# Neos-codes/microbeast

Hardware: AMD Instinct MI355X
Metric: env frames/sec (whole node) on 16x16 microRTS (higher is better)
Workload: dtype bf16

## Files before the change

### microbeast_amd/_native.py

```python
from __future__ import annotations

import ctypes
import importlib.util
import os
import sys
import threading
from pathlib import Path

import torch

_LIB = Path(__file__).resolve().parent / "_lib"
_lock = threading.Lock()
_kern = None
_rt = None

c_void_p, c_int, c_int64, c_float = ctypes.c_void_p, ctypes.c_int, ctypes.c_int64, ctypes.c_float

_SIGS = {
    "mbk_multi_copy": [c_void_p, c_int, c_void_p],
    "mbk_comm_standin": [c_void_p, c_void_p, c_int64, c_int, c_int, c_void_p],
    "mbk_row_gather": [c_void_p, c_void_p, c_void_p, c_int, c_int64, c_void_p],
    "mbk_memset": [c_void_p, c_int, c_int64, c_void_p],
    "mbk_masked_cell_fwd": [c_void_p, c_int, c_void_p, c_void_p, c_void_p, c_int, c_int64,
                            c_void_p, c_void_p, c_void_p],
# ... 10 lines not shown
    "mbk_imgwgrad_parts": [],
    "mbk_cells_nchunk": [c_int],
    "mbk_cells_compact": [c_void_p, c_int, c_int, c_int, c_void_p, c_void_p, c_void_p, c_void_p,
                          c_void_p, c_void_p, c_void_p, c_void_p, c_void_p, c_void_p],
    "mbk_rows_colsum": [c_void_p, c_int, c_int, c_void_p, c_int, c_void_p, c_void_p],
    "mbk_masked_cell_rows_fwd": [c_void_p, c_int, c_void_p, c_void_p, c_int, c_void_p, c_void_p,
                                 c_void_p, c_int, c_void_p, c_void_p, c_void_p],
    "mbk_masked_cell_rows_bwd": [c_void_p, c_int, c_void_p, c_void_p, c_int, c_int, c_void_p,
                                 c_void_p, c_void_p, c_void_p, c_void_p, c_void_p],
    "mbk_pwgrad": [c_void_p, c_void_p],
    "mbk_pwgrad_all": [c_void_p, c_void_p],
    "mbk_pwgrad_all_parts": [c_int, c_int, c_int],
    "mbk_pwgrad_parts": [c_int, c_int, c_int, c_int],
    "mbk_reduce_map": [c_void_p, c_int, c_int64, c_void_p, c_int64, c_void_p, c_void_p],
    "mbk_reduce_inv": [c_void_p, c_int, c_int64, c_void_p, c_int64, c_void_p, c_void_p, c_int64,
                       c_void_p],
    "mbk_ppool_fwd": [c_void_p, c_int, c_int, c_int, c_int, c_void_p, c_void_p, c_void_p],
    "mbk_ppool_bwd": [c_void_p, c_int64, c_int, c_void_p, c_int64, c_int, c_void_p, c_void_p,
                      c_int, c_int, c_int, c_int, c_void_p, c_void_p],
    "mbk_rng_advance": [c_void_p, c_void_p],
    "mbk_vtrace": [c_void_p, c_void_p, c_void_p, c_void_p, c_void_p, c_void_p, c_int, c_int,
                   c_float, c_float, c_float, c_float, c_float, c_float, c_float, c_void_p,
                   c_void_p, c_void_p, c_void_p, c_void_p, c_void_p, c_void_p],
    "mbk_vtrace_upgo": [c_void_p, c_void_p, c_void_p, c_void_p, c_void_p, c_void_p, c_int, c_int,
                        c_float, c_float, c_float, c_float, c_float, c_float, c_float, c_float,
                        c_float, c_float, c_void_p, c_void_p, c_void_p, c_void_p, c_void_p,
                        c_void_p, c_void_p, c_void_p],
    "mbk_gae": [c_void_p, c_void_p, c_void_p, c_int, c_int, c_float, c_float, c_float, c_int,
                c_void_p, c_void_p, c_void_p, c_void_p, c_void_p],
    "mbk_vtrace_adv": [c_void_p, c_void_p, c_void_p, c_void_p, c_void_p, c_int, c_int, c_float,
                       c_float, c_float, c_float, c_float, c_int, c_void_p, c_void_p, c_void_p,
                       c_void_p, c_void_p, c_void_p],
    "mbk_ppo_loss": [c_void_p, c_void_p, c_void_p, c_void_p, c_void_p, c_void_p, c_void_p,
                     c_void_p, c_int, c_int, c_float, c_float, c_float, c_float, c_float, c_float,
                     c_void_p, c_void_p, c_void_p, c_void_p, c_void_p],
    "mbk_adv_stats_rows": [c_void_p, c_int, c_int, c_int, c_int, c_void_p, c_void_p, c_void_p],
    "mbk_ppo_loss_rows": [c_void_p, c_void_p, c_void_p, c_void_p, c_void_p, c_void_p, c_void_p,
                          c_void_p, c_int, c_int, c_int, c_float, c_float, c_float, c_float,
                          c_float, c_float, c_int, c_void_p, c_void_p, c_void_p, c_void_p,
                          c_void_p, c_void_p],
    "mbk_grad_clip_scale": [c_void_p, c_int64, c_float, c_float, c_void_p, c_void_p, c_void_p],
    "mbk_adam": [c_void_p, c_void_p, c_void_p, c_void_p, c_void_p, c_int64, c_float, c_float,
                 c_float, c_float, c_float, c_int64, c_void_p, c_float, c_void_p],
    "mbk_to_bf16": [c_void_p, c_int64, c_void_p, c_void_p],
    "mbk_from_bf16": [c_void_p, c_int64, c_void_p, c_void_p],
    "mbk_conv_fwd": [c_void_p, c_int, c_int, c_int, c_void_p, c_void_p, c_void_p, c_void_p,
                     c_void_p, c_void_p, c_void_p, c_int, c_int, c_int, c_int, c_int, c_void_p],
    "mbk_conv_fwd_fp8": [c_void_p, c_int, c_int, c_int, c_void_p, c_void_p, c_void_p, c_void_p,
                         c_void_p, c_int, c_int, c_int, c_int, c_int, c_void_p],
    "mbk_conv_fwd_imgs": [c_int, c_int, c_int, c_int, c_int, c_int, c_int],
    "mbk_conv_wgrad_imgs": [c_int, c_int, c_int, c_int, c_int, c_int],
    "mbk_res_bwd16_imgs": [c_int, c_int],
    "mbk_res_blk32_fwd_imgs": [c_int, c_int],
    "mbk_res_bwd32_imgs": [c_int, c_int],
    "mbk_res_fwd16_stage_ok": [c_int, c_int],
    "mbk_conv_pack_fp8": [c_void_p, c_int, c_void_p],
    "mbk_pool_bwd_idx": [c_void_p, c_void_p, c_int, c_int, c_int, c_int, c_void_p, c_void_p],
    "mbk_conv_wgrad": [c_void_p, c_int, c_int, c_int, c_void_p, c_void_p, c_void_p, c_void_p,
                       c_int, c_int, c_int, c_int, c_int, c_int, c_void_p],
    "mbk_conv_wgrad_parts": [c_int, c_int, c_int, c_int, c_int, c_int, c_int],
    "mbk_conv_wgrad0_sparse_parts": [c_int],
    "mbk_conv_wgrad0_sparse": [c_void_p, c_void_p, c_void_p, ctypes.c_uint, c_void_p, c_int, c_int,
                               c_void_p],
    "mbk_pool_conv_bwd_parts": [c_int, c_int, c_int, c_int, c_int],
    "mbk_pool_conv_bwd": [c_void_p, c_void_p, c_void_p, c_void_p, c_void_p, c_void_p, c_int,
                          c_int, c_int, c_int, c_int, c_int, c_void_p],
    "mbk_conv_set_grid_cap": [c_int],
    "mbk_set_learner_occupancy": [c_int, c_int],
    "mbk_set_work_queues": [c_int],
    "mbk_set_work_queue_site": [c_int, c_int],
    "mbk_conv0_row_set": [c_int],
    "mbk_fc_wgrad_parts": [c_int, c_int, c_int],
    "mbk_fc_wgrad": [c_void_p, c_void_p, c_int, c_int, c_int, c_void_p, c_int, c_void_p, c_int,
                     c_void_p],
    "mbk_fc_fwd": [c_void_p, c_int, c_void_p, c_void_p, c_void_p, c_void_p, c_int, c_int, c_int,
                   c_void_p, c_void_p, c_void_p],
    "mbk_gemm_nt": [c_void_p, c_void_p, c_void_p, c_void_p, c_int, c_int, c_int, c_int, c_int,
                    c_int, c_int, c_int, c_int, c_void_p],
    "mbk_wgrad_partial_floats": [c_int, c_int, c_int],
    "mbk_wgrad_reduce_batch": [c_void_p, c_int, c_void_p],
    "mbk_pool_bwd": [c_void_p, c_void_p, c_int, c_int, c_int, c_int, c_void_p, c_void_p],
    "mbk_conv_pack": [c_void_p, c_int, c_void_p],
    "mbk_head_compact": [c_void_p, c_int, c_int, c_void_p, c_void_p, c_void_p, c_void_p,
                         c_void_p, c_void_p, c_void_p, c_void_p, c_void_p, c_void_p, c_void_p,
                         c_void_p, c_void_p, c_int, c_void_p, c_void_p, c_void_p, c_void_p],
    "mbk_head_fwd": [c_void_p, c_void_p, c_void_p, c_void_p, c_void_p, c_void_p, c_int,
                     c_void_p, c_void_p, c_void_p, c_void_p, c_void_p, c_void_p, c_int, c_int,
                     c_void_p, c_void_p, c_int, c_void_p],
    "mbk_fc_wgrad_wide_parts": [c_int, c_int, c_int],
    "mbk_fc_wgrad_wide": [c_void_p, c_void_p, c_int, c_int, c_int, c_int, c_void_p, c_int,
                          c_void_p, c_void_p, c_void_p],
    "mbk_head_score": [c_void_p, c_void_p, c_void_p, c_void_p, c_void_p, c_void_p, c_void_p,
                       c_void_p, c_void_p, c_void_p, c_void_p, c_int, c_void_p, c_void_p,
                       c_void_p, c_void_p],
    "mbk_head_pair_rowsum": [c_void_p, c_void_p, c_int, c_int, c_void_p, c_void_p, c_void_p,
                             c_void_p, c_void_p],
    "mbk_head_bwd": [c_void_p, c_void_p, c_void_p, c_void_p, c_void_p, c_void_p, c_void_p,
                     c_void_p, c_void_p, c_void_p, c_void_p, c_void_p, c_void_p, c_void_p,
                     c_void_p, c_int, c_int, c_void_p, c_void_p, c_void_p, c_void_p,
                     c_void_p, c_void_p, c_void_p],
    "mbk_head_dx_gather": [c_void_p, c_void_p, c_void_p, c_int, c_int, c_void_p, c_void_p],
    "mbk_head_dx_value_parts": [c_int],
    "mbk_head_dx_value": [c_void_p, c_void_p, c_void_p, c_int, c_int, c_void_p, c_void_p,
                          c_void_p, c_int, c_void_p, c_void_p, c_int, c_void_p],
    "mbk_head_pack": [c_void_p, c_void_p, c_int, c_void_p, c_void_p, c_void_p, c_void_p],
    "mbk_decode_obs_mask": [c_void_p, c_void_p, c_int, c_int, c_int, c_void_p, c_void_p, c_void_p],
    "mbk_decode_obs_mask_bucket": [c_void_p, c_void_p, c_int, c_int, c_int, c_void_p, c_void_p,
                                   c_void_p, c_void_p, c_void_p, c_void_p, c_void_p],
    "mbk_head_units": [c_void_p, c_int, c_int, c_void_p, c_void_p, c_void_p, c_void_p, c_void_p,
                       c_void_p],
    "mbk_row_sum_rng": [c_void_p, c_int64, c_int, c_void_p, c_void_p, c_void_p],
    "mbk_row_sum_pack": [c_void_p, c_int64, c_int, c_void_p, c_void_p, c_void_p, c_void_p,
                         c_void_p, c_int, c_void_p],
    "mbk_head_fwd_counts": [c_void_p, c_void_p, c_void_p, c_void_p, c_void_p, c_void_p,
                            c_void_p, c_void_p, c_int, c_int, c_int, c_void_p, c_int, c_void_p],
    "mbk_trunk_tail": [c_void_p, c_void_p, c_void_p, c_int, c_int, c_int, c_void_p, c_void_p],
    "mbk_trunk_tail_fp8": [c_void_p, c_void_p, c_void_p, c_void_p, c_int, c_int, c_int, c_void_p,
                           c_void_p],
    "mbk_trunk_tail_fc": [c_void_p, c_void_p, c_void_p, c_int, c_int, c_int, c_void_p, c_void_p,
                          c_void_p, c_void_p, c_void_p, c_int, c_void_p, c_void_p, c_void_p],
    "mbk_pack_env_actions": [c_void_p, c_int64, c_void_p, c_void_p],
    "mbk_res_bwd16_parts": [c_int, c_int, c_int],
    "mbk_res_bwd32_parts": [c_int, c_int, c_int],
    "mbk_res_bwd32": [c_void_p, c_void_p, c_void_p, c_void_p, c_void_p, c_void_p, c_void_p, c_int,
                      c_int, c_int, c_int, c_void_p],
    "mbk_res_fwd16": [c_void_p, c_void_p, c_void_p, c_void_p, c_void_p, c_void_p, c_void_p, c_int,
                      c_int, c_int, c_void_p],
    "mbk_res_fwd16_stage": [c_void_p, c_void_p, c_void_p, c_void_p, c_void_p, c_void_p, c_void_p,
                            c_void_p, c_void_p, c_void_p, c_void_p, c_int, c_int, c_int, c_void_p],
    "mbk_res_blk32_fwd": [c_void_p, c_void_p, c_void_p, c_void_p, c_void_p, c_int, c_int, c_int,
                          c_void_p],
    "mbk_pool_conv_fwd4": [c_void_p, c_void_p, c_void_p, c_void_p, c_void_p, c_int, c_void_p],
    "mbk_res_blk32_fwd_wave": [c_void_p, c_void_p, c_void_p, c_void_p, c_void_p, c_int, c_int,
                               c_int, c_void_p],
    "mbk_res_bwd32_team_parts": [c_int, c_int, c_int],
    "mbk_res_bwd32_team": [c_void_p, c_void_p, c_void_p, c_void_p, c_void_p, c_void_p, c_void_p,
                           c_int, c_int, c_int, c_int, c_void_p],
    "mbk_res_bwd16": [c_void_p, c_void_p, c_void_p, c_void_p, c_void_p, c_void_p, c_void_p, c_int,
                      c_int, c_int, c_int, c_void_p],
    "mbk_bits_pad": [c_void_p, c_int, c_int, c_int, c_int, c_int, c_void_p, c_void_p],
    "mbk_colsum_parts": [c_int64],
    "mbk_colsum": [c_void_p, c_int, c_int, c_int, c_int, c_void_p, c_void_p, c_int, c_void_p,
                   c_void_p],
    "mbk_map_gather": [c_int, c_void_p, c_void_p, c_void_p, c_void_p, c_void_p, c_void_p],
    "mbk_value_bwd_parts": [c_int],
    "mbk_value_bwd": [c_void_p, c_void_p, c_void_p, c_int, c_int, c_void_p, c_void_p, c_void_p,
                      c_int, c_int, c_void_p],
    "mbk_fc_wgrad_ex": [c_void_p, c_void_p, c_int, c_int, c_int, c_void_p, c_int, c_void_p, c_int,
                        c_int, c_void_p],
    "mbk_act_step": [c_void_p, c_void_p, c_void_p],
    "mbk_act_trunk": [c_void_p, c_void_p, c_void_p],
    "mbk_act_head": [c_void_p, c_void_p, c_void_p],
    "mbk_act_set_stamps": [c_void_p],
    "mbk_rows_to_codes": [c_void_p, c_int, c_int, c_int, c_void_p, c_void_p, c_void_p],
    "mbk_codes_to_rows": [c_void_p, c_int, c_int, c_void_p, c_int, c_void_p],
    "mbk_gemm_nt_mask": [c_void_p, c_void_p, c_void_p, c_void_p, c_int, c_int, c_int, c_int, c_int,
                         c_int, c_int, c_int, c_void_p, c_void_p],
}
_RESTYPE = {"mbk_wgrad_partial_floats": c_int64}


def _ensure_built() -> None:
    kl = _LIB / "libmbk_kernels.so"
    rts = list(_LIB.glob("_mbrt*.so"))
    if kl.exists() and rts and os.environ.get("MBK_REBUILD", "0") != "1":
        return
    from .csrc import build as _b

    _b.build()


def kernels():
    global _kern
    if _kern is not None:
        return _kern
    with _lock:
        if _kern is None:
            _ensure_built()
            lib = ctypes.CDLL(str(_LIB / "libmbk_kernels.so"), mode=ctypes.RTLD_GLOBAL)
            for name, args in _SIGS.items():
                fn = getattr(lib, name)
                fn.argtypes = args
                fn.restype = _RESTYPE.get(name, c_int)
            _kern = _Checked(lib)
    return _kern


class _Checked:

    def __init__(self, lib):
        self._lib = lib

    def __getattr__(self, name):
        if name not in _SIGS:
            raise AttributeError(f"{name}: no ctypes signature declared in _native._SIGS")
        return getattr(self._lib, name)


def runtime():
    global _rt
    if _rt is not None:
        return _rt
    with _lock:
        if _rt is None:
            _ensure_built()
            kernels_path = _LIB / "libmbk_kernels.so"
            ctypes.CDLL(str(kernels_path), mode=ctypes.RTLD_GLOBAL)
            cands = sorted(_LIB.glob("_mbrt*.so"))
            if not cands:
                raise ImportError("microbeast_amd native runtime (_mbrt) not built")
            spec = importlib.util.spec_from_file_location("microbeast_amd._lib._mbrt", cands[0])
            mod = importlib.util.module_from_spec(spec)
            spec.loader.exec_module(mod)
            sys.modules["microbeast_amd._lib._mbrt"] = mod
            _rt = mod
    return _rt


def check(rc: int, what: str) -> None:
    if rc != 0:
        raise RuntimeError(f"{what} failed with hipError {rc}")


def stream_ptr(stream: torch.cuda.Stream | None = None) -> int:
    s = stream if stream is not None else torch.cuda.current_stream()
    return int(s.cuda_stream)


def ptr(t: torch.Tensor | None) -> int | None:
    return None if t is None else t.data_ptr()


def loaded_libraries() -> list[str]:
    out = []
    try:
        with open("/proc/self/maps") as f:
            for line in f:
                if str(_LIB) in line:
                    p = line.split()[-1]
                    if p not in out:
                        out.append(p)
    except OSError:
        pass
    return out
```

### microbeast_amd/csrc/include/mbk_api.h

```cpp
#pragma once
#include <hip/hip_runtime_api.h>
#include <stdint.h>

#ifdef __cplusplus
extern "C" {
#endif

#define MBK_MAX_COPY_SEGS 16
typedef struct {
  const void* src;
  void* dst;
  uint64_t bytes;
} MbkCopySeg;

int mbk_multi_copy(const MbkCopySeg* segs, int n, hipStream_t stream);

typedef struct {
  const float* w;
  void* fwd;
  void* bwd;
  int cin, cin_real, cout;
} MbkPackJob;

int mbk_conv_pack(const MbkPackJob* jobs, int n, hipStream_t stream);

typedef struct {
  const float* w;
  void* q;
  float* scale;
  int cin, cin_real, cout;
} MbkPackJob8;

int mbk_conv_pack_fp8(const MbkPackJob8* jobs, int n, hipStream_t stream);

typedef struct {
  const void* w0;
  const float* b0;
  const void* w[14];
  const float* b[14];
  const void* w5;
  const float* b5;
  const float* wc;
  const float* bc;
  const void* Wp;
  const float* bp;
  uint64_t* rng;
  void* feat;
  int* bucket_cnt;
  int* bucket;
  uint64_t* cellx;
  int* pending;
  int E, H, W;
} MbkActModel;

typedef struct {
  const uint16_t* codes;
  const int32_t* res;
  const uint32_t* code_list;
  uint32_t* obs;
  uint32_t* mask;
  uint32_t* obs2;
  uint32_t* mask2;
  uint8_t* action;
  float* logp;
  float* value;
  uint16_t* act16;
  uint32_t* act_list;
  int list_stride;
  const float* reward_src;
  const uint8_t* done_src;
  float* reward_dst;
  uint8_t* done_dst;
  uint64_t step;
  uint32_t* abits;
  uint32_t* abits2;
  int32_t greedy;
} MbkActStep;

int mbk_act_step(const MbkActModel* m, const MbkActStep* s, hipStream_t stream);
int mbk_rows_to_codes(const uint32_t* rows, int stride, int E, int S, void* codes, int32_t* res,
                      hipStream_t stream);
int mbk_codes_to_rows(const void* act16, int E, int S, uint32_t* rows, int stride,
                      hipStream_t stream);
int mbk_act_trunk(const MbkActModel* m, const MbkActStep* s, hipStream_t stream);
int mbk_act_head(const MbkActModel* m, const MbkActStep* s, hipStream_t stream);

int mbk_gae(const float* v_old, const float* reward, const uint8_t* done, int T, int B,
            float gamma, float lambda, float reward_clip, int norm_adv, float* adv, float* ret,
            float* partials, float* stats, hipStream_t stream);
int mbk_vtrace_adv(const float* logp_pi, const float* logp_mu, const float* v,
                   const float* reward, const uint8_t* done, int T, int B, float gamma,
                   float lambda, float rho_bar, float c_bar, float reward_clip, int norm_adv,
                   float* adv, float* ret, float* partials, float* stats, float* is_stats,
                   hipStream_t stream);
int mbk_ppo_loss(const float* logp_new, const float* logp_old, const float* values,
                 const float* v_old, const float* adv, const float* ret, const float* entropy,
                 const float* stats, int T, int B, float clip_lo, float clip_hi, float clip,
                 float value_clip, float baseline_cost, float entropy_cost, float* g_logp,
                 float* g_value, float* partials, float* losses, hipStream_t stream);
int mbk_adv_stats_rows(const float* adv, int T, int B, int K, int norm_adv, float* partials,
                       float* stats, hipStream_t stream);
int mbk_ppo_loss_rows(const float* logp_new, const float* logp_old, const float* values,
                      const float* v_old, const float* adv, const float* ret,
                      const float* entropy, const float* stats, int t0, int Tm, int B,
                      float clip_lo, float clip_hi, float clip, float value_clip,
                      float baseline_cost, float entropy_cost, int step, float* g_logp,
                      float* g_value, float* partials, float* losses, float* epoch_mean,
                      hipStream_t stream);

int mbk_vtrace_upgo(const float* logp_new, const float* logp_old, const float* values,
                    const float* reward, const uint8_t* done, const float* entropy, int T, int B,
                    float gamma, float lambda, float rho_bar, float c_bar, float pg_rho_bar,
                    float upgo_rho_bar, float baseline_cost, float entropy_cost, float upgo_cost,
                    float reward_clip, float* vs_out, float* adv_out, float* upgo_out,
                    float* g_logp, float* g_value, float* partials, float* losses,
                    hipStream_t stream);

#ifdef __cplusplus
}
#endif
```

### microbeast_amd/csrc/kernels/conv.hip

```cpp
#include "../include/mbk_api.h"
#include "common.h"
#include "launch.h"
#include "tile.h"

#include <algorithm>
#include <map>
#include <mutex>

using namespace mbk;

namespace {

constexpr int kThreads = 256;

template <int CIN>
struct Geo {
  static constexpr int NCH = CIN == 16 ? 5 : 9;
  static constexpr int PIXB = CIN * 2 + 16;
  static constexpr int PIXB8 = CIN + 8;
};

struct ConvFwdArgs {
  const void* x;
  const bf16* w;
  const float* bias;
  const bf16* add;
  const bf16* mask_src;
  bf16* y;
  bf16* y_full;
  uint8_t* pool_idx;
  int N, H, W, imgs, relu_in, pool;
  const float* wscale;
  int* queue = nullptr;
};

constexpr int kPF = 8;

__device__ __forceinline__ uint4 expand_bits8(uint32_t bits) {
  uint32_t w4[4];
#pragma unroll
  for (int j = 0; j < 4; ++j)
    w4[j] = (((bits >> (2 * j)) & 1u) ? 0x3F80u : 0u) |
            (((bits >> (2 * j + 1)) & 1u) ? 0x3F800000u : 0u);
  return make_uint4(w4[0], w4[1], w4[2], w4[3]);
}

__device__ __forceinline__ uint2 expand_bits8_fp8(uint32_t bits) {
  uint32_t w2[2] = {0u, 0u};
#pragma unroll
  for (int j = 0; j < 8; ++j)
    if ((bits >> j) & 1u) w2[j >> 2] |= 0x38u << (8 * (j & 3));
  return make_uint2(w2[0], w2[1]);
}

__device__ __forceinline__ uint32_t cvt_fp8x4(float a, float b, float c, float d) {
  auto sat = [](float v) { return fminf(fmaxf(v, -448.f), 448.f); };
  int w = __builtin_amdgcn_cvt_pk_fp8_f32(sat(a), sat(b), 0, false);
  w = __builtin_amdgcn_cvt_pk_fp8_f32(sat(c), sat(d), w, true);
  return (uint32_t)w;
}

__device__ __forceinline__ uint2 bf16x8_to_fp8(uint4 v) {
  const uint32_t w[4] = {v.x, v.y, v.z, v.w};
  float f[8];
#pragma unroll
  for (int j = 0; j < 4; ++j) {
    f[2 * j] = __uint_as_float(w[j] << 16);
    f[2 * j + 1] = __uint_as_float(w[j] & 0xFFFF0000u);
  }
  return make_uint2(cvt_fp8x4(f[0], f[1], f[2], f[3]), cvt_fp8x4(f[4], f[5], f[6], f[7]));
}

template <int CIN, bool BITS, bool F8>
__device__ __forceinline__ int fwd_lds_off(int e, int H, int W) {
  constexpr int PIXB = F8 ? Geo<CIN>::PIXB8 : Geo<CIN>::PIXB;
  const int Hp = H + 2, Wp = W + 2, HW = H * W;
  if (BITS) {
    const int im = e / HW, r = e - im * HW, y = r / W, x = r - y * W;
    return ((im * Hp + y + 1) * Wp + x + 1) * PIXB;
  } else {
    constexpr int CH16 = CIN / 8;
    const int q = e % CH16, p = e / CH16;
    const int im = p / HW, r = p - im * HW, y = r / W, x = r - y * W;
    return ((im * Hp + y + 1) * Wp + x + 1) * PIXB + q * (F8 ? 8 : 16);
  }
}


template <int CIN, int COUT, bool BITS, bool F8>
__global__ __launch_bounds__(kThreads) void conv_fwd_kernel(ConvFwdArgs a) {
  extern __shared__ __attribute__((aligned(16))) char smem[];
  constexpr int NCH = Geo<CIN>::NCH;
  constexpr int PIXB = F8 ? Geo<CIN>::PIXB8 : Geo<CIN>::PIXB;
  constexpr int NB = COUT / 16;
  constexpr int EPP = BITS ? 1 : CIN / 8;
  constexpr int OSTR = COUT + 4;
  const int H = a.H, W = a.W, HW = H * W, Hp = H + 2, Wp = W + 2;
  const PixSplit split{HW, W, 1.f / (float)HW, 1.f / (float)W};
  const int tid = threadIdx.x, lane = tid & 63, wave = tid >> 6;
  const int g = lane >> 4, li = lane & 15;
  char* tile = smem;
  const int tile_bytes = ((a.imgs * Hp * Wp * PIXB) + 15) & ~15;
  bf16* otile = (bf16*)(smem + tile_bytes);
  const int ngroups = (a.N + a.imgs - 1) / a.imgs;
  const int per_grp = a.imgs * HW * EPP;

  for (int e = tid; e < tile_bytes / 16; e += kThreads) ((uint4*)tile)[e] = make_uint4(0, 0, 0, 0);
  int loff[kPF];
#pragma unroll
  for (int k = 0; k < kPF; ++k) {
    const int e = tid + k * kThreads;
    loff[k] = e < per_grp ? fwd_lds_off<CIN, BITS, F8>(e, H, W) : 0;
  }
  Frag8 bw[NCH][NB];
  long bw8[NCH][NB];
#pragma unroll
  for (int nb = 0; nb < NB; ++nb) {
    if constexpr (F8) {
      const long* wp = (const long*)((const uint8_t*)a.w + (size_t)(nb * 16 + li) * NCH * 32 + g * 8);
#pragma unroll
      for (int c = 0; c < NCH; ++c) bw8[c][nb] = wp[c * 4];
    } else {
      const uint4* wp = (const uint4*)(a.w + (size_t)(nb * 16 + li) * NCH * 32 + g * 8);
#pragma unroll
      for (int c = 0; c < NCH; ++c) bw[c][nb].u = wp[c * 4];
    }
  }
  float bias_v[NB][4], wsc[NB][4];
#pragma unroll
  for (int nb = 0; nb < NB; ++nb)
#pragma unroll
    for (int i = 0; i < 4; ++i) {
      bias_v[nb][i] = a.bias ? a.bias[nb * 16 + 4 * g + i] : 0.f;
      wsc[nb][i] = F8 ? a.wscale[nb * 16 + 4 * g + i] : 1.f;
    }

  uint4 pv[kPF];
  uint32_t pw[kPF];
  auto prefetch = [&](int grp) {
    const size_t base = (size_t)grp * per_grp;
    const int lim = min(per_grp, (a.N - grp * a.imgs) * HW * EPP);
#pragma unroll
    for (int k = 0; k < kPF; ++k) {
      const int e = tid + k * kThreads;
      if (BITS) pw[k] = e < lim ? ((const uint32_t*)a.x)[base + e] : 0u;
      else pv[k] = e < lim ? ((const uint4*)a.x)[base + e] : make_uint4(0, 0, 0, 0);
    }
  };
  auto put = [&](int off, uint4 v) {
    if (a.relu_in) {
      v.x = relu2(v.x); v.y = relu2(v.y);
      v.z = relu2(v.z); v.w = relu2(v.w);
    }
    if constexpr (F8) *(uint2*)(tile + off) = bf16x8_to_fp8(v);
    else *(uint4*)(tile + off) = v;
// ... 1045 lines not shown
  red[pl][col] = s;
  __syncthreads();
  if (pl != 0 || e >= row) return;
  s = red[0][col] + red[1][col] + red[2][col] + red[3][col];
  if (stage) {
    stage[(size_t)split * row + e] = s;
    return;
  }
  if (e < cout * ktot) {
    const int co = e / ktot, r = e - co * ktot, t = r / cin, ci = r - t * cin;
    if (ci >= cin_real) return;
    float* d = dw + ((size_t)co * cin_real + ci) * 9 + t;
    *d = s;
  } else if (db) {
    const int co = e - cout * ktot;
    db[co] = s;
  }
}

struct MbkReduceJob {
  const float* partial;
  float* dw;
  float* db;
  int nparts, cin, cin_real, cout;
};
constexpr int kMaxReduceJobs = 32;
struct ReduceBatch {
  MbkReduceJob j[kMaxReduceJobs];
};

__global__ __launch_bounds__(256) void wgrad_reduce_batch_kernel(ReduceBatch b, int level) {
  __shared__ float red[4][64];
  const MbkReduceJob J = b.j[blockIdx.z];
  const int row = mbk::wgrad_row_floats(J.cin, J.cout);
  if ((int)blockIdx.x * 64 >= row) return;
  const bool two = J.nparts > 2 * kReducePps;
  const int splits = two ? mbk::wgrad_reduce_splits(J.nparts) : 1;
  float* stage = two ? (float*)J.partial + (size_t)J.nparts * row : nullptr;
  if (level == 0) {
    if ((int)blockIdx.y >= splits) return;
    wgrad_reduce_cols(J.partial, J.nparts, two ? kReducePps : J.nparts, blockIdx.y, blockIdx.x,
                      stage, J.cin, J.cin_real, J.cout, J.dw, J.db, red);
  } else {
    if (!two || blockIdx.y != 0) return;
    wgrad_reduce_cols(stage, splits, splits, 0, blockIdx.x, nullptr, J.cin, J.cin_real, J.cout,
                      J.dw, J.db, red);
  }
}

__global__ __launch_bounds__(256) void pool_bwd_kernel(const bf16* __restrict__ cfull,
                                                       const bf16* __restrict__ dp, int N, int H,
                                                       int W, int C, bf16* __restrict__ dc) {
  const int Ho = (H + 1) >> 1, Wo = (W + 1) >> 1;
  const size_t tot = (size_t)N * H * W * C;
  for (size_t e = (size_t)blockIdx.x * blockDim.x + threadIdx.x; e < tot;
       e += (size_t)gridDim.x * blockDim.x) {
    const int c = e % C;
    const size_t p = e / C;
    const int x = p % W, y = (p / W) % H;
    const size_t n = p / ((size_t)H * W);
    float g = 0.f;
    const int oy_lo = y / 2, oy_hi = min(Ho - 1, (y + 1) / 2);
    const int ox_lo = x / 2, ox_hi = min(Wo - 1, (x + 1) / 2);
    for (int oy = max(0, oy_lo - 1); oy <= oy_hi; ++oy) {
      if (y < 2 * oy - 1 || y > 2 * oy + 1) continue;
      for (int ox = max(0, ox_lo - 1); ox <= ox_hi; ++ox) {
        if (x < 2 * ox - 1 || x > 2 * ox + 1) continue;
        float mx = -INFINITY;
        int ay = -1, ax = -1;
        for (int ky = 0; ky < 3; ++ky) {
          const int yy = 2 * oy - 1 + ky;
          if (yy < 0 || yy >= H) continue;
          for (int kx = 0; kx < 3; ++kx) {
            const int xx = 2 * ox - 1 + kx;
            if (xx < 0 || xx >= W) continue;
            const float v = bf2f(cfull[((n * H + yy) * W + xx) * C + c]);
            if (v > mx || ay < 0) { mx = v; ay = yy; ax = xx; }
          }
        }
        if (ay == y && ax == x) g += bf2f(dp[((n * Ho + oy) * Wo + ox) * C + c]);
      }
    }
    dc[e] = f2bf(g);
  }
}

template <int C>
__global__ __launch_bounds__(256) void pool_bwd_idx_kernel(const uint8_t* __restrict__ pidx,
                                                           const bf16* __restrict__ dp, int N,
                                                           int H, int W,
                                                           bf16* __restrict__ dc) {
  constexpr int C8 = C / 8;
  const int Ho = (H + 1) >> 1, Wo = (W + 1) >> 1;
  const uint32_t tot = (uint32_t)N * Ho * Wo * C8;
  for (uint32_t e = blockIdx.x * blockDim.x + threadIdx.x; e < tot; e += gridDim.x * blockDim.x) {
    const int c8 = e % C8;
    uint32_t q = e / C8;
    const int k = q % Wo;
    q /= Wo;
    const int j = q % Ho;
    const uint32_t n = q / Ho;
    uint32_t ids[2][2][2];
    uint32_t dv[2][2][4];
#pragma unroll
    for (int dj = 0; dj < 2; ++dj)
#pragma unroll
      for (int dk = 0; dk < 2; ++dk) {
        const int oy = j + dj, ox = k + dk;
        if (oy < Ho && ox < Wo) {
          const uint32_t o = ((n * Ho + oy) * Wo + ox) * C + c8 * 8;
          const uint2 iv = *(const uint2*)(pidx + o);
          const uint4 d = *(const uint4*)(dp + o);
          ids[dj][dk][0] = iv.x; ids[dj][dk][1] = iv.y;
          dv[dj][dk][0] = d.x; dv[dj][dk][1] = d.y; dv[dj][dk][2] = d.z; dv[dj][dk][3] = d.w;
        } else {
          ids[dj][dk][0] = ids[dj][dk][1] = 0xFFFFFFFFu;
          dv[dj][dk][0] = dv[dj][dk][1] = dv[dj][dk][2] = dv[dj][dk][3] = 0u;
        }
      }
#pragma unroll
    for (int a = 0; a < 2; ++a)
#pragma unroll
      for (int b = 0; b < 2; ++b) {
        const int y = 2 * j + a, x = 2 * k + b;
        if (y >= H || x >= W) continue;
        float g[8] = {0, 0, 0, 0, 0, 0, 0, 0};
#pragma unroll
        for (int dj = 0; dj < 2; ++dj)
#pragma unroll
          for (int dk = 0; dk < 2; ++dk) {
            const int ky = a + 1 - 2 * dj, kx = b + 1 - 2 * dk;
            if (ky < 0 || kx < 0) continue;
            const uint32_t me = (uint32_t)(ky * 3 + kx);
#pragma unroll
            for (int t = 0; t < 8; ++t) {
              const uint32_t id = (ids[dj][dk][t >> 2] >> (8 * (t & 3))) & 0xFFu;
              const uint32_t hb = (dv[dj][dk][t >> 1] >> (16 * (t & 1))) & 0xFFFFu;
              if (id == me) g[t] += __uint_as_float(hb << 16);
            }
          }
        uint32_t o[4];
#pragma unroll
        for (int t = 0; t < 4; ++t) {
          const uint32_t lo = __bfloat16_as_ushort(f2bf(g[2 * t]));
          const uint32_t hi = __bfloat16_as_ushort(f2bf(g[2 * t + 1]));
          o[t] = lo | (hi << 16);
        }
        *(uint4*)(dc + ((size_t)(n * H + y) * W + x) * C + c8 * 8) =
            make_uint4(o[0], o[1], o[2], o[3]);
      }
  }
}

struct PackJob {
  const float* w;
  bf16* fwd;
  bf16* bwd;
  int cin, cin_real, cout;
};
struct PackJobs {
  PackJob j[16];
  int n;
};

__device__ __forceinline__ int nch_of(int c) { return c == 16 ? 5 : 9; }

__global__ __launch_bounds__(256) void conv_pack_kernel(PackJobs jobs) {
  const PackJob& J = jobs.j[blockIdx.y];
  if (blockIdx.y >= jobs.n) return;
  const int nf = J.cout * nch_of(J.cin) * 32;
  const int nb = J.bwd ? J.cin * nch_of(J.cout) * 32 : 0;
  for (int e = blockIdx.x * blockDim.x + threadIdx.x; e < nf + nb; e += gridDim.x * blockDim.x) {
    if (e < nf) {
      const int co = e / (nch_of(J.cin) * 32), r = e % (nch_of(J.cin) * 32);
      const int c = r / 32, k = r % 32;
      int tap, ci;
      if (J.cin == 16) { tap = 2 * c + k / 16; ci = k % 16; }
      else { tap = c; ci = k; }
      float v = 0.f;
      if (tap < 9 && ci < J.cin_real) v = J.w[((size_t)co * J.cin_real + ci) * 9 + tap];
      J.fwd[e] = f2bf(v);
    } else {
      const int f = e - nf;
      const int ci = f / (nch_of(J.cout) * 32), r = f % (nch_of(J.cout) * 32);
      const int c = r / 32, k = r % 32;
      int tap, co;
      if (J.cout == 16) { tap = 2 * c + k / 16; co = k % 16; }
      else { tap = c; co = k; }
      float v = 0.f;
      if (tap < 9 && ci < J.cin_real) v = J.w[((size_t)co * J.cin_real + ci) * 9 + (8 - tap)];
      J.bwd[f] = f2bf(v);
    }
  }
}

struct PackJob8 {
  const float* w;
  uint8_t* q;
  float* scale;
  int cin, cin_real, cout;
};
struct PackJobs8 {
  PackJob8 j[16];
  int n;
};

__global__ __launch_bounds__(256) void conv_pack_fp8_kernel(PackJobs8 jobs) {
  if ((int)blockIdx.y >= jobs.n) return;
  const PackJob8& J = jobs.j[blockIdx.y];
  const int co = blockIdx.x;
  if (co >= J.cout) return;
  __shared__ float red[256];
  const int nk = J.cin_real * 9;
  const float* wr = J.w + (size_t)co * nk;
  float m = 0.f;
  for (int e = threadIdx.x; e < nk; e += blockDim.x) m = fmaxf(m, fabsf(wr[e]));
  red[threadIdx.x] = m;
  __syncthreads();
  for (int st = 128; st > 0; st >>= 1) {
    if ((int)threadIdx.x < st) red[threadIdx.x] = fmaxf(red[threadIdx.x], red[threadIdx.x + st]);
    __syncthreads();
  }
  const float amax = red[0];
  int k = 0;
  if (amax > 0.f) {
    k = (int)floorf(log2f(224.f / amax));
    k = max(-30, min(30, k));
  }
  const float sc = ldexpf(1.f, k);
  const int nch = J.cin == 16 ? 5 : 9;
  for (int e = threadIdx.x; e < nch * 32; e += blockDim.x) {
    const int c = e / 32, kk = e % 32;
    int tap, ci;
    if (J.cin == 16) { tap = 2 * c + kk / 16; ci = kk % 16; }
    else { tap = c; ci = kk; }
    float v = 0.f;
    if (tap < 9 && ci < J.cin_real) v = wr[ci * 9 + tap] * sc;
    v = fminf(fmaxf(v, -448.f), 448.f);
    const int b = __builtin_amdgcn_cvt_pk_fp8_f32(v, 0.f, 0, false);
    J.q[(size_t)co * nch * 32 + e] = (uint8_t)(b & 0xFF);
  }
  if (threadIdx.x == 0) J.scale[co] = ldexpf(1.f, -k);
}

inline size_t fwd_smem(int cin, int imgs, int H, int W, int cout, bool pool, bool fp8 = false) {
  const int pixb = fp8 ? cin + 8 : cin * 2 + 16;
  size_t t = (((size_t)imgs * (H + 2) * (W + 2) * pixb) + 15) & ~(size_t)15;
  if (pool) t += (size_t)imgs * H * W * (cout + 4) * 2;
  return t;
}

constexpr int kFwdPix = 512;
constexpr size_t kFwdLds = 48 * 1024;
int fwd_imgs(int cin, int cout, int H, int W, bool bits, bool pool, bool fp8) {
  if (cin < 8 || H < 1 || W < 1) return 0;
  const int hw = H * W, epp = bits ? 1 : cin / 8;
  int imgs = std::max(1, kFwdPix / hw);
  while (imgs > 1 && (fwd_smem(cin, imgs, H, W, cout, pool, fp8) > kFwdLds ||
                      imgs * hw * epp > kPF * kThreads))
    imgs /= 2;
  return imgs;
}

int wgrad_imgs(int cin, int cout, int H, int W, bool bits, int unpool_imgs) {
  if (cin < 8 || cout < 8 || H < 1 || W < 1) return 0;
  const int hw = H * W, xepp = bits ? 1 : cin / 8, pf = kPFW * kThreads;
  int imgs = std::max(1, std::min(pf / (hw * xepp), pf / (hw * (cout / 8))));
  if (unpool_imgs > 0) imgs = std::min(imgs, unpool_imgs);
  const size_t lim = (cin > cout ? 72 : 64) * 1024;
  while (imgs > 1 && wg_tile_bytes(cin, cout, imgs, H, W, wg_band_w(H, W)) - 128 > lim) imgs /= 2;
  return imgs;
}

inline size_t wgrad_smem(int cin, int cout, int imgs, int H, int W) {
  size_t t = wg_tile_bytes(cin, cout, imgs, H, W, wg_band_w(H, W));
  t += 4096;
  t += 64;
  size_t red = (size_t)cout * 9 * cin * 4;
  return t > red ? t : red;
}

int g_grid_cap = 0;
int g_conv0_row = 1;

int capped_resident_blocks(const void* kfn, int threads, size_t sm, int (*occ)(int)) {
  const int r = resident_blocks(kfn, threads, sm, occ);
  return g_grid_cap > 0 && r > g_grid_cap ? g_grid_cap : r;
}

int fwd_grid(int ngroups, const void* kfn, size_t sm) {
  const long r = (long)capped_resident_blocks(kfn, kThreads, sm, mbk_occ_f);
  return (int)std::max(1L, std::min((long)ngroups, r));
}

}

static int conv_fwd_launch(const void* x, int in_bits, int cin, int cout, const void* w,
                           const float* wscale, const float* bias, const void* add,
                           const void* mask_src, void* y, void* y_full, void* pool_idx, int N,
                           int H, int W, int relu_in, int pool, bool fp8, hipStream_t stream) {
  if (N <= 0) return 0;
  if (fp8 && !wscale) return (int)hipErrorInvalidValue;
  const int imgs = fwd_imgs(cin, cout, H, W, in_bits != 0, pool != 0, fp8);
  if (!index_math_ok(imgs, H, W)) return (int)hipErrorInvalidValue;
  ConvFwdArgs a{x, (const bf16*)w, bias, (const bf16*)add, (const bf16*)mask_src, (bf16*)y,
                (bf16*)y_full, (uint8_t*)pool_idx, N, H, W, imgs, relu_in, pool, wscale};
  const size_t sm = fwd_smem(cin, imgs, H, W, cout, pool != 0, fp8);
  if (sm > 160 * 1024) return (int)hipErrorInvalidValue;
  const int ngroups = (N + imgs - 1) / imgs;
#define LAUNCH(CI, CO, B)                                                                   \
  do {                                                                                      \
    auto kfn = fp8 ? conv_fwd_kernel<CI, CO, B, true> : conv_fwd_kernel<CI, CO, B, false>;  \
    const int grid = fwd_grid(ngroups, (const void*)kfn, sm);   \
    hipLaunchKernelGGL(kfn, dim3(grid), dim3(kThreads), sm, stream, a);                     \
  } while (0)
  if (in_bits && cout == 16 && W > 16 && W <= 32 && !fp8 && g_conv0_row && !add && !mask_src &&
      !relu_in && kLutBytes + (size_t)kRowImgs * H * W * 16 * 2 <= 160 * 1024) {
    const size_t sm0 = kLutBytes + (pool ? (size_t)kRowImgs * H * W * 16 * 2 : 0);
    const auto kfn = conv0_row_kernel<0, 16, true>;
    const int grid = fwd_grid((N + kRowImgs - 1) / kRowImgs, (const void*)kfn, sm0);
    hipLaunchKernelGGL(kfn, dim3(grid), dim3(kThreads), sm0, stream, a);
    return (int)hipGetLastError();
  }
  if (in_bits && (cout == 16 || cout == 32) && W == 16 && !fp8 && g_conv0_row && !add &&
      !mask_src && !relu_in) {
    const size_t sm0 =
        kLutBytes + (pool ? (size_t)kRowImgs * H * 16 * conv0_ostr(cout, false) * 2 : 0);
    if (sm0 > 160 * 1024) return (int)hipErrorInvalidValue;
    const bool hb = H == 16;
    const auto kfn = cout == 16 ? (hb ? conv0_row16_kernel : conv0_row_kernel<0, 16>)
                                : (hb ? conv0_row_kernel<16, 32> : conv0_row_kernel<0, 32>);
    const int grid = fwd_grid((N + kRowImgs - 1) / kRowImgs, (const void*)kfn, sm0);
    if (hb) a.queue = mbk_work_queue(stream, kQueueConv0);
    hipLaunchKernelGGL(kfn, dim3(grid), dim3(kThreads), sm0, stream, a);
    return (int)hipGetLastError();
  }
  if (in_bits) {
    if (cout == 16) LAUNCH(32, 16, true);
    else if (cout == 32) LAUNCH(32, 32, true);
    else return (int)hipErrorInvalidValue;
  } else if (cin == 16 && cout == 16) LAUNCH(16, 16, false);
  else if (cin == 16 && cout == 32) LAUNCH(16, 32, false);
  else if (cin == 32 && cout == 16) LAUNCH(32, 16, false);
  else if (cin == 32 && cout == 32) LAUNCH(32, 32, false);
  else return (int)hipErrorInvalidValue;
#undef LAUNCH
// ... 277 lines not shown
```

### microbeast_amd/csrc/kernels/gridnet.hip

```cpp
#include "common.h"

#include <algorithm>
#include <climits>

namespace {

constexpr int kThreads = 256;

__device__ __forceinline__ float bf_lo(uint32_t u) { return __uint_as_float(u << 16); }
__device__ __forceinline__ float bf_hi(uint32_t u) { return __uint_as_float(u & 0xFFFF0000u); }
__device__ __forceinline__ uint32_t bf_bits(float v) {
  return (uint32_t)__bfloat16_as_ushort(__float2bfloat16(v));
}
__device__ __forceinline__ uint32_t pack2(float a, float b) { return bf_bits(a) | (bf_bits(b) << 16); }
__device__ __forceinline__ float to_f(float v) { return v; }
__device__ __forceinline__ float to_f(bf16 v) { return __bfloat162float(v); }

int grid_for(long work) {
  long g = (work + kThreads - 1) / kThreads;
  return (int)(g < 1 ? 1 : g > 65535 * 4 ? 65535 * 4 : g);
}

template <typename IDX>
__global__ __launch_bounds__(kThreads) void bits_pad_kernel(const uint32_t* __restrict__ bits,
                                                            int n, int h, int w, int ph, int pw,
                                                            uint32_t* __restrict__ out) {
  const IDX total = (IDX)n * ph * pw;
  for (IDX e = (IDX)blockIdx.x * kThreads + threadIdx.x; e < total; e += (IDX)gridDim.x * kThreads) {
    const int x = (int)(e % pw), t = (int)(e / pw);
    const int y = t % ph, b = t / ph;
    out[e] = (y < h && x < w) ? bits[(size_t)b * h * w + y * w + x] : 0u;
  }
}

template <typename T>
__global__ __launch_bounds__(kThreads) void colsum_part_kernel(const T* __restrict__ x, int R,
                                                               int C, int ld, int rpp,
                                                               float* __restrict__ partial) {
  __shared__ float red[4][64];
  const int lane = threadIdx.x & 63, wave = threadIdx.x >> 6;
  const int col = blockIdx.y * 64 + lane;
  const int r0 = blockIdx.x * rpp, r1 = min(R, r0 + rpp);
  float s = 0.f;
  if (col < C)
    for (int r = r0 + wave; r < r1; r += 4) s += to_f(x[(size_t)r * ld + col]);
  red[wave][lane] = s;
  __syncthreads();
  if (wave == 0 && col < C)
    partial[(size_t)blockIdx.x * C + col] = (red[0][lane] + red[1][lane]) + (red[2][lane] + red[3][lane]);
}

__global__ __launch_bounds__(kThreads) void colsum_part_vec_kernel(const bf16* __restrict__ x,
                                                                   int R, int C, int ld, int rpp,
                                                                   float* __restrict__ partial) {
  __shared__ float red[kThreads][8];
  const int CG = (C + 7) >> 3, slots = kThreads / CG;
  const int cg = threadIdx.x % CG, rs = threadIdx.x / CG;
  const int r0 = blockIdx.x * rpp, r1 = min(R, r0 + rpp);
  float acc[8];
#pragma unroll
  for (int j = 0; j < 8; ++j) acc[j] = 0.f;
  if (rs < slots)
    for (int r = r0 + rs; r < r1; r += slots) {
      const uint4 u = *(const uint4*)(x + (size_t)r * ld + 8 * cg);
      const uint32_t uu[4] = {u.x, u.y, u.z, u.w};
#pragma unroll
      for (int j = 0; j < 8; ++j) acc[j] += (j & 1) ? bf_hi(uu[j >> 1]) : bf_lo(uu[j >> 1]);
    }
#pragma unroll
  for (int j = 0; j < 8; ++j) red[threadIdx.x][j] = acc[j];
  __syncthreads();
  if (threadIdx.x < CG) {
    float s[8];
#pragma unroll
    for (int j = 0; j < 8; ++j) s[j] = 0.f;
    for (int q = 0; q < slots; ++q)
#pragma unroll
      for (int j = 0; j < 8; ++j) s[j] += red[q * CG + threadIdx.x][j];
#pragma unroll
    for (int j = 0; j < 8; ++j) {
      const int c = 8 * threadIdx.x + j;
      if (c < C) partial[(size_t)blockIdx.x * C + c] = s[j];
    }
  }
}

__global__ __launch_bounds__(kThreads) void colsum_fin_kernel(const float* __restrict__ partial,
                                                              int P, int C, float* out0, int c0,
                                                              float* out1) {
  __shared__ float red[kThreads];
  const int c = blockIdx.x;
  float s = 0.f;
  for (int p = threadIdx.x; p < P; p += kThreads) s += partial[(size_t)p * C + c];
  red[threadIdx.x] = s;
  __syncthreads();
  for (int o = kThreads / 2; o > 0; o >>= 1) {
    if ((int)threadIdx.x < o) red[threadIdx.x] += red[threadIdx.x + o];
    __syncthreads();
  }
  if (threadIdx.x == 0) {
    if (c < c0) out0[c] = red[0];
    else out1[c - c0] = red[0];
  }
}

constexpr int kMaxSeg = 24;
struct MapSeg {
  const float* src;
  void* dst;
  const int* map;
  int n, dst_bf16;
};
struct MapSegs {
  MapSeg s[kMaxSeg];
};

__global__ __launch_bounds__(kThreads) void map_gather_kernel(MapSegs a) {
  const MapSeg sg = a.s[blockIdx.y];
  for (int i = blockIdx.x * kThreads + threadIdx.x; i < sg.n; i += gridDim.x * kThreads) {
    const int m = sg.map[i];
    const float v = m >= 0 ? sg.src[m] : 0.f;
    if (sg.dst_bf16) ((bf16*)sg.dst)[i] = __float2bfloat16(v);
    else ((float*)sg.dst)[i] = v;
  }
}

__global__ __launch_bounds__(kThreads) void value_bwd_kernel(const float* __restrict__ dv,
                                                             const bf16* __restrict__ h,
                                                             const float* __restrict__ w2, int R,
                                                             int K, int rpp, bf16* __restrict__ dh,
                                                             float* __restrict__ partial,
                                                             const void* __restrict__ gadd,
                                                             int gadd_rows, int gadd_f32) {
  __shared__ float red[kThreads][9];
  const int G = K >> 3, rows = kThreads / G;
  const int cg = threadIdx.x % G, rs = threadIdx.x / G;
  float w[8], sw[8], sb = 0.f;
#pragma unroll
  for (int j = 0; j < 8; ++j) { w[j] = w2[8 * cg + j]; sw[j] = 0.f; }
  const int r0 = blockIdx.x * rpp, r1 = min(R, r0 + rpp);
  if (rs < rows)
    for (int r = r0 + rs; r < r1; r += rows) {
      const float d = dv[r];
      const uint4 u = *(const uint4*)(h + (size_t)r * K + 8 * cg);
      const uint32_t uu[4] = {u.x, u.y, u.z, u.w};
      float ga[8];
#pragma unroll
      for (int j = 0; j < 8; ++j) ga[j] = 0.f;
      if (r < gadd_rows) {
        if (gadd_f32) {
          const float4* gp = (const float4*)((const float*)gadd + (size_t)r * K + 8 * cg);
          const float4 a = gp[0], b = gp[1];
          ga[0] = a.x, ga[1] = a.y, ga[2] = a.z, ga[3] = a.w;
          ga[4] = b.x, ga[5] = b.y, ga[6] = b.z, ga[7] = b.w;
        } else {
          const uint4 gv = *(const uint4*)((const bf16*)gadd + (size_t)r * K + 8 * cg);
          const uint32_t gg[4] = {gv.x, gv.y, gv.z, gv.w};
#pragma unroll
          for (int j = 0; j < 8; ++j) ga[j] = (j & 1) ? bf_hi(gg[j >> 1]) : bf_lo(gg[j >> 1]);
        }
      }
      float o[8];
#pragma unroll
      for (int j = 0; j < 8; ++j) {
        const float hj = (j & 1) ? bf_hi(uu[j >> 1]) : bf_lo(uu[j >> 1]);
        o[j] = hj > 0.f ? d * w[j] + ga[j] : 0.f;
        sw[j] += d * hj;
      }
      sb += d;
      *(uint4*)(dh + (size_t)r * K + 8 * cg) =
          make_uint4(pack2(o[0], o[1]), pack2(o[2], o[3]), pack2(o[4], o[5]), pack2(o[6], o[7]));
    }
#pragma unroll
  for (int j = 0; j < 8; ++j) red[threadIdx.x][j] = sw[j];
  red[threadIdx.x][8] = sb;
  __syncthreads();
  if (threadIdx.x < G) {
    float acc[9];
#pragma unroll
    for (int j = 0; j < 9; ++j) acc[j] = 0.f;
    for (int s = 0; s < rows; ++s)
#pragma unroll
      for (int j = 0; j < 9; ++j) acc[j] += red[s * G + threadIdx.x][j];
    float* out = partial + (size_t)blockIdx.x * (K + 1);
#pragma unroll
    for (int j = 0; j < 8; ++j) out[8 * threadIdx.x + j] = acc[j];
    if (threadIdx.x == 0) out[K] = acc[8];
  }
}

bool fits(long v) { return v >= 0 && v < INT_MAX; }
#define MBK_LAUNCH_IDX(kern, total, ...)                                                  \
  do {                                                                                   \
    if (fits(total))                                                                     \
      hipLaunchKernelGGL(kern<int>, dim3(grid_for(total)), dim3(kThreads), 0, __VA_ARGS__); \
    else                                                                                 \
      hipLaunchKernelGGL(kern<int64_t>, dim3(grid_for(total)), dim3(kThreads), 0,          \
                         __VA_ARGS__);                                                   \
  } while (0)

}

extern "C" int mbk_bits_pad(const void* bits, int n, int h, int w, int ph, int pw, void* out,
                            hipStream_t stream) {
  if (n <= 0) return 0;
  if (ph < h || pw < w) return (int)hipErrorInvalidValue;
  const long total = (long)n * ph * pw;
  MBK_LAUNCH_IDX(bits_pad_kernel, total, stream, (const uint32_t*)bits, n, h, w, ph, pw,
                 (uint32_t*)out);
  return (int)hipGetLastError();
}

int colsum_parts(long R) { return (int)std::max(1L, std::min(2048L, (R + 1023) / 1024)); }

extern "C" int mbk_colsum(const void* x, int x_f32, int R, int C, int ld, float* partial,
                          float* out0, int c0, float* out1, hipStream_t stream) {
  if (C <= 0) return 0;
  if (R < 0 || ld < C) return (int)hipErrorInvalidValue;
  const int P = colsum_parts(R);
  const int rpp = std::max(1, (R + P - 1) / P);
  const dim3 g1(P, (C + 63) / 64);
  if (!x_f32 && ld % 8 == 0 && C <= 256 && ((uintptr_t)x & 15) == 0)
    hipLaunchKernelGGL(colsum_part_vec_kernel, dim3(P), dim3(kThreads), 0, stream, (const bf16*)x,
                       R, C, ld, rpp, partial);
  else if (x_f32)
    hipLaunchKernelGGL(colsum_part_kernel<float>, g1, dim3(kThreads), 0, stream, (const float*)x,
                       R, C, ld, rpp, partial);
  else
    hipLaunchKernelGGL(colsum_part_kernel<bf16>, g1, dim3(kThreads), 0, stream, (const bf16*)x, R,
                       C, ld, rpp, partial);
  hipLaunchKernelGGL(colsum_fin_kernel, dim3(C), dim3(kThreads), 0, stream, (const float*)partial,
                     P, C, out0, c0, out1);
  return (int)hipGetLastError();
}

extern "C" int mbk_colsum_parts(long R) { return colsum_parts(R); }

extern "C" int mbk_map_gather(int nseg, const void* const* src, void* const* dst,
                              const void* const* map, const int* n, const int* dst_bf16,
                              hipStream_t stream) {
  if (nseg <= 0) return 0;
  if (nseg > kMaxSeg) return (int)hipErrorInvalidValue;
  MapSegs a{};
  int mx = 0;
  for (int s = 0; s < nseg; ++s) {
    a.s[s] = MapSeg{(const float*)src[s], dst[s], (const int*)map[s], n[s], dst_bf16[s]};
    mx = std::max(mx, n[s]);
  }
  if (mx == 0) return 0;
  hipLaunchKernelGGL(map_gather_kernel, dim3(std::min(grid_for(mx), 1024), nseg), dim3(kThreads),
                     0, stream, a);
  return (int)hipGetLastError();
}

int value_parts(int R) { return std::max(1, std::min(256, (R + 1023) / 1024)); }
extern "C" int mbk_value_bwd_parts(int R) { return value_parts(R); }

extern "C" int mbk_value_bwd(const float* dv, const void* h, const float* w2, int R, int K,
                             void* dh, float* partial, const void* gadd, int gadd_rows,
                             int gadd_f32, hipStream_t stream) {
  if (R <= 0) return 0;
  if (K % 8 || K > 8 * kThreads || gadd_rows > R) return (int)hipErrorInvalidValue;
  const int P = value_parts(R);
  const int rpp = (R + P - 1) / P;
  hipLaunchKernelGGL(value_bwd_kernel, dim3(P), dim3(kThreads), 0, stream, dv, (const bf16*)h, w2,
                     R, K, rpp, (bf16*)dh, partial, gadd, gadd ? gadd_rows : 0, gadd_f32);
  return (int)hipGetLastError();
}
```

### microbeast_amd/csrc/kernels/head.hip

```cpp
#include <cstdio>
#include <vector>

#include "../include/mbk_api.h"
#include "../include/microrts_rules.h"
#include "common.h"
#include "launch.h"
#include "tile.h"

#ifndef MBK_HA_MB
#define MBK_HA_MB 4
#endif

using namespace mbk;

namespace {

constexpr int KD = 256;
constexpr int NP = 80;
constexpr int NPT = 96;

__device__ __forceinline__ bool active3(const uint32_t* m) { return (m[0] | m[1] | m[2]) != 0u; }

__device__ __forceinline__ int abits_words(int S) { return (S + 31) >> 5; }

__global__ __launch_bounds__(256) void head_count_kernel(const uint32_t* __restrict__ mask,
                                                         int F, int S, int FB,
                                                         int* __restrict__ cnt,
                                                         uint32_t* __restrict__ abits) {
  const int b = blockIdx.x, nfb = gridDim.x;
  const int lane = threadIdx.x & 63;
  const int c = blockIdx.y * 256 + threadIdx.x, c0 = c - lane;
  if (c0 >= S) return;
  const bool in = c < S;
  const int SW = abits_words(S), w0 = c0 >> 5;
  const bool two = c0 + 32 < S;
  const int f0 = b * FB, f1 = min(F, f0 + FB);
  int n = 0;
#pragma unroll 8
  for (int f = f0; f < f1; ++f) {
    const bool a = in && active3(mask + ((size_t)f * S + c) * 3);
    n += a;
    const uint64_t bal = __ballot(a);
    if (lane == 0) abits[(size_t)f * SW + w0] = (uint32_t)bal;
    if (lane == 1 && two) abits[(size_t)f * SW + w0 + 1] = (uint32_t)(bal >> 32);
  }
  if (in) cnt[c * nfb + b] = n;
}

constexpr int CHUNK = 512;
constexpr int MAX_S = 1024;

__global__ __launch_bounds__(256) void head_cell_scan_kernel(const int* __restrict__ cnt, int nfb,
                                                             int* __restrict__ off,
                                                             int* __restrict__ tot) {
  __shared__ int ws[4];
  const int c = blockIdx.x, tid = threadIdx.x, lane = tid & 63, wave = tid >> 6;
  int carry = 0;
  for (int b0 = 0; b0 < nfb; b0 += 256) {
    const int b = b0 + tid;
    const int x = b < nfb ? cnt[c * nfb + b] : 0;
    int incl = x;
#pragma unroll
    for (int o = 1; o < 64; o <<= 1) {
      const int y = __shfl_up(incl, o, 64);
      if (lane >= o) incl += y;
    }
    if (lane == 63) ws[wave] = incl;
    __syncthreads();
    int wbase = 0;
    for (int w = 0; w < wave; ++w) wbase += ws[w];
    const int total = ws[0] + ws[1] + ws[2] + ws[3];
    if (b < nfb) off[c * nfb + b] = carry + wbase + incl - x;
    carry += total;
    __syncthreads();
  }
  if (tid == 0) tot[c] = carry;
}

__global__ __launch_bounds__(1024) void head_scan_kernel(const int* __restrict__ cell_tot, int S,
                                                         int* __restrict__ grp_start,
                                                         int* __restrict__ grp_count,
                                                         int* __restrict__ unit_cell,
                                                         int* __restrict__ unit_row,
                                                         int* __restrict__ chunk_cell,
                                                         int* __restrict__ chunk_row,
                                                         int* __restrict__ chunk_start,
                                                         int* __restrict__ totals ) {
  __shared__ int ust[MAX_S], cst[MAX_S], gst[MAX_S];
  __shared__ int sv[1024], su[1024], sq[1024];
  const int tid = threadIdx.x, lane = tid & 63, wave = tid >> 6, nw = blockDim.x >> 6;
  int v = 0, u = 0, q = 0;
  if (tid < S) {
    v = cell_tot[tid];
    u = (v + 15) / 16;
    q = (v + CHUNK - 1) / CHUNK;
  }
  sv[tid] = v; su[tid] = u; sq[tid] = q;
  __syncthreads();
  for (int o = 1; o < 1024; o <<= 1) {
    const int a = tid >= o ? sv[tid - o] : 0, b = tid >= o ? su[tid - o] : 0,
              d = tid >= o ? sq[tid - o] : 0;
    __syncthreads();
    sv[tid] += a; su[tid] += b; sq[tid] += d;
    __syncthreads();
  }
  if (tid < S) {
    const int gs = sv[tid] - v;
    grp_start[tid] = gs;
    grp_count[tid] = v;
    chunk_start[tid] = sq[tid] - q;
    gst[tid] = gs;
    ust[tid] = su[tid] - u;
    cst[tid] = sq[tid] - q;
  }
  if (tid == 1023) {
    totals[0] = sv[1023];
    totals[1] = su[1023];
    totals[2] = sq[1023];
  }
  __syncthreads();
  for (int c = wave; c < S; c += nw) {
    const int gs = gst[c], n = sv[c] - gs;
    for (int r = lane * 16; r < n; r += 64 * 16) {
      const int k = ust[c] + r / 16;
      unit_cell[k] = c;
      unit_row[k] = gs + r;
    }
    for (int r = lane * CHUNK; r < n; r += 64 * CHUNK) {
      const int k = cst[c] + r / CHUNK;
      chunk_cell[k] = c;
      chunk_row[k] = gs + r;
    }
  }
}

__global__ __launch_bounds__(256) void head_count_bits_kernel(const uint32_t* __restrict__ abits,
                                                              int F, int S, int FB,
                                                              int* __restrict__ cnt) {
  const int b = blockIdx.x, nfb = gridDim.x;
  const int c = blockIdx.y * 256 + threadIdx.x;
  if (c >= S) return;
  const int SW = abits_words(S), w = c >> 5, bit = c & 31;
  const int f0 = b * FB, f1 = min(F, f0 + FB);
  int n = 0;
#pragma unroll 8
  for (int f = f0; f < f1; ++f) n += (abits[(size_t)f * SW + w] >> bit) & 1u;
  cnt[c * nfb + b] = n;
}

__global__ __launch_bounds__(256) void head_scatter_kernel(
    const uint32_t* __restrict__ abits, int F, int S, int FB, const int* __restrict__ off,
    const int* __restrict__ grp_start,
    int* __restrict__ pairs, int* __restrict__ pidx, uint8_t* __restrict__ action_zero,
    float* __restrict__ cell_lp, float* __restrict__ cell_ent) {
  const int b = blockIdx.x, nfb = gridDim.x;
  const int c = blockIdx.y * 256 + threadIdx.x;
  if (c >= S) return;
  const int f0 = b * FB, f1 = min(F, f0 + FB);
  const int SW = abits_words(S), w = c >> 5, bit = c & 31;
// ... 1013 lines not shown
    float s = 0.f;
    for (int q = 0; q < nch; ++q)
      if (hb_run_end(c0 + q, c0 + nch, nchunks, bwd_grid))
        s += dWp[(size_t)(c0 + q) * kCell * KD + e];
    dW[(size_t)c * kCell * KD + e] = s;
  } else if (e < kCell * KD + kCell) {
    const int n = e - kCell * KD;
    float s = 0.f;
    for (int q = 0; q < nch; ++q)
      if (hb_run_end(c0 + q, c0 + nch, nchunks, bwd_grid)) s += dbp[(size_t)(c0 + q) * kCell + n];
    db[c * kCell + n] = s;
  }
}

__device__ __forceinline__ bool abit(const uint32_t* ab, int c, int S) {
  return c < S && ((ab[c >> 5] >> (c & 31)) & 1u);
}

__global__ __launch_bounds__(256) void head_dx_gather_kernel(const bf16* __restrict__ dXp,
                                                             const int* __restrict__ pidx,
                                                             const uint32_t* __restrict__ abits,
                                                             int F, int S,
                                                             float* __restrict__ dX) {
  const int lane = threadIdx.x & 63;
  const int f = blockIdx.x * 4 + (threadIdx.x >> 6);
  if (f >= F) return;
  float4 acc = make_float4(0.f, 0.f, 0.f, 0.f);
  const int* pr = pidx + (size_t)f * S;
  const uint32_t* ab = abits + (size_t)f * abits_words(S);
  for (int c0 = 0; c0 < S; c0 += 64) {
    const int p = abit(ab, c0 + lane, S) ? pr[c0 + lane] : -1;
    uint64_t m = __ballot(p >= 0);
    while (m) {
      const int b = __builtin_ctzll(m);
      m &= m - 1;
      const int pp = __shfl(p, b);
      const uint2 v = ((const uint2*)(dXp + (size_t)pp * KD))[lane];
      acc.x += __uint_as_float(v.x << 16); acc.y += __uint_as_float(v.x & 0xFFFF0000u);
      acc.z += __uint_as_float(v.y << 16); acc.w += __uint_as_float(v.y & 0xFFFF0000u);
    }
  }
  ((float4*)(dX + (size_t)f * KD))[lane] = acc;
}

__global__ __launch_bounds__(256) void head_dx_value_kernel(const bf16* __restrict__ dXp,
                                                            const int* __restrict__ pidx,
                                                            const uint32_t* __restrict__ abits,
                                                            int F,
                                                            int S, const float* __restrict__ dv,
                                                            const bf16* __restrict__ h,
                                                            const float* __restrict__ wc, int R,
                                                            bf16* __restrict__ dh,
                                                            float* __restrict__ partial) {
  __shared__ float red[4][KD + 4];
  const int lane = threadIdx.x & 63, wave = __builtin_amdgcn_readfirstlane(threadIdx.x >> 6);
  const float4 w = ((const float4*)wc)[lane];
  float sw[4] = {0.f, 0.f, 0.f, 0.f}, sb = 0.f;
  constexpr int kMaxCh = MAX_S / 64;
  const int nch = (S + 63) / 64;
  const int stride = gridDim.x * 4;
  float dn = 0.f;
  uint2 hn = make_uint2(0, 0);
  int pn[kMaxCh];
  uint32_t wn[kMaxCh];
  auto fetch_bits = [&](int r) {
    const uint32_t* ab = abits + (size_t)r * abits_words(S);
#pragma unroll
    for (int q = 0; q < kMaxCh; ++q)
      wn[q] = (r < F && q < nch && q * 64 + lane < S) ? ab[(q * 64 + lane) >> 5] : 0u;
  };
  auto fetch = [&](int r) {
    dn = dv[r];
    hn = ((const uint2*)(h + (size_t)r * KD))[lane];
    const int* pr = pidx + (size_t)r * S;
#pragma unroll
    for (int q = 0; q < kMaxCh; ++q)
      pn[q] = ((wn[q] >> (lane & 31)) & 1u) ? pr[q * 64 + lane] : -1;
  };
  const int rfirst = blockIdx.x * 4 + wave;
  if (rfirst < R) {
    fetch_bits(rfirst);
    fetch(rfirst);
    if (rfirst + stride < R) fetch_bits(rfirst + stride);
  }
  for (int r = rfirst; r < R; r += stride) {
    const float d = dn;
    const uint2 hv = hn;
    int pc[kMaxCh];
#pragma unroll
    for (int q = 0; q < kMaxCh; ++q) pc[q] = pn[q];
    if (r + stride < R) {
      fetch(r + stride);
      if (r + 2 * stride < R) fetch_bits(r + 2 * stride);
    }
    float4 acc = make_float4(0.f, 0.f, 0.f, 0.f);
#pragma unroll
    for (int q = 0; q < kMaxCh; ++q) {
      if (q >= nch) break;
      const int p = pc[q];
      uint64_t m = __ballot(p >= 0);
      while (m) {
        int pp[4];
#pragma unroll
        for (int j = 0; j < 4; ++j) {
          pp[j] = -1;
          if (m) {
            const int b = __builtin_ctzll(m);
            m &= m - 1;
            pp[j] = __shfl(p, b);
          }
        }
        uint2 v[4];
#pragma unroll
        for (int j = 0; j < 4; ++j)
          v[j] = pp[j] >= 0 ? ((const uint2*)(dXp + (size_t)pp[j] * KD))[lane]
                            : make_uint2(0u, 0u);
#pragma unroll
        for (int j = 0; j < 4; ++j) {
          if (pp[j] < 0) break;
          acc.x += __uint_as_float(v[j].x << 16); acc.y += __uint_as_float(v[j].x & 0xFFFF0000u);
          acc.z += __uint_as_float(v[j].y << 16); acc.w += __uint_as_float(v[j].y & 0xFFFF0000u);
        }
      }
    }
    const float hj[4] = {__uint_as_float(hv.x << 16), __uint_as_float(hv.x & 0xFFFF0000u),
                         __uint_as_float(hv.y << 16), __uint_as_float(hv.y & 0xFFFF0000u)};
    const float wj[4] = {w.x, w.y, w.z, w.w}, gj[4] = {acc.x, acc.y, acc.z, acc.w};
    float o[4];
#pragma unroll
    for (int i = 0; i < 4; ++i) {
      o[i] = hj[i] > 0.f ? d * wj[i] + gj[i] : 0.f;
      sw[i] += d * hj[i];
    }
    sb += d;
    const uint32_t o0 = (uint32_t)__bfloat16_as_ushort(f2bf(o[0])) |
                        ((uint32_t)__bfloat16_as_ushort(f2bf(o[1])) << 16);
    const uint32_t o1 = (uint32_t)__bfloat16_as_ushort(f2bf(o[2])) |
                        ((uint32_t)__bfloat16_as_ushort(f2bf(o[3])) << 16);
    ((uint2*)(dh + (size_t)r * KD))[lane] = make_uint2(o0, o1);
  }
#pragma unroll
  for (int i = 0; i < 4; ++i) red[wave][4 * lane + i] = sw[i];
  if (lane == 0) red[wave][KD] = sb;
  __syncthreads();
  for (int e = threadIdx.x; e < KD + 1; e += 256)
    partial[(size_t)blockIdx.x * (KD + 1) + e] = red[0][e] + red[1][e] + red[2][e] + red[3][e];
}

__global__ __launch_bounds__(256) void head_pack_kernel(const float* __restrict__ W,
                                                        const float* __restrict__ b, int S,
                                                        bf16* __restrict__ Wp,
                                                        float* __restrict__ bp,
                                                        bf16* __restrict__ WpT) {
  const size_t nWp = (size_t)S * NP * KD;
  const size_t nWt = WpT ? (size_t)S * KD * NPT : 0;
  const size_t nb = (size_t)S * NP;
  for (size_t e = (size_t)blockIdx.x * blockDim.x + threadIdx.x; e < nWp + nWt + nb;
       e += (size_t)gridDim.x * blockDim.x) {
    if (e < nWp) {
      const size_t c = e / (NP * KD), r = e % (NP * KD), n = r / KD, k = r % KD;
      Wp[e] = f2bf(n < (size_t)kCell ? W[(c * kCell + n) * KD + k] : 0.f);
    } else if (e < nWp + nWt) {
      const size_t q = e - nWp, c = q / (KD * NPT), r = q % (KD * NPT), d = r / NPT, n = r % NPT;
      WpT[q] = f2bf(n < (size_t)kCell ? W[(c * kCell + n) * KD + d] : 0.f);
    } else {
      const size_t q = e - nWp - nWt, c = q / NP, n = q % NP;
      bp[q] = n < (size_t)kCell ? b[c * kCell + n] : 0.f;
    }
  }
}

}

extern "C" int mbk_head_fb(int F) {
  int fb = F / 64;
  if (fb < 8) fb = 8;
  if (fb > 256) fb = 256;
  return fb;
}

extern "C" int mbk_head_compact(const uint32_t* mask, int F, int S, int* cnt, int* off,
                                int* grp_start, int* grp_count, int* unit_cell, int* unit_row,
                                int* chunk_cell, int* chunk_row, int* chunk_start,
                                int* totals, int* pairs, int* pidx, uint32_t* abits,
                                int abits_given, uint8_t* action_zero, float* cell_lp,
                                float* cell_ent, hipStream_t stream) {
  if (S > MAX_S) return (int)hipErrorInvalidValue;
  const int FB = mbk_head_fb(F);
  const int nfb = (F + FB - 1) / FB;
  dim3 g1(nfb, (S + 255) / 256);
  if (!abits) return (int)hipErrorInvalidValue;
  if (abits_given)
    hipLaunchKernelGGL(head_count_bits_kernel, g1, dim3(256), 0, stream, abits, F, S, FB, cnt);
  else
    hipLaunchKernelGGL(head_count_kernel, g1, dim3(256), 0, stream, mask, F, S, FB, cnt, abits);
  hipLaunchKernelGGL(head_cell_scan_kernel, dim3(S), dim3(256), 0, stream, cnt, nfb, off,
                     grp_count);
  hipLaunchKernelGGL(head_scan_kernel, dim3(1), dim3(1024), 0, stream, grp_count, S, grp_start,
                     grp_count, unit_cell, unit_row, chunk_cell, chunk_row, chunk_start, totals);
  hipLaunchKernelGGL(head_scatter_kernel, g1, dim3(256), 0, stream, abits, F, S, FB, off,
                     grp_start, pairs, pidx, action_zero, cell_lp, cell_ent);
  return (int)hipGetLastError();
}

extern "C" int mbk_head_units(int* bucket_cnt, int S, int E, int* grp_start, int* grp_count,
                              int* unit_cell, int* unit_row, int* totals, hipStream_t stream) {
  if (S > MAX_S) return (int)hipErrorInvalidValue;
  hipLaunchKernelGGL(head_units_kernel, dim3(1), dim3(1024), 0, stream, bucket_cnt, S, E,
                     grp_start, grp_count, unit_cell, unit_row, totals);
  return (int)hipGetLastError();
}

extern "C" int mbk_head_fwd(const void* X, const void* Wp, const float* bp, const uint32_t* mask,
                            uint8_t* action, const uint64_t* rng, int sample, const int* pairs,
                            const int* unit_cell, const int* unit_row, const int* grp_start,
                            const int* grp_count, const int* totals, int S, int grid,
                            float* cell_lp, float* cell_ent, int pair_out, hipStream_t stream) {
  if (sample < 0 || sample > 2) return (int)hipErrorInvalidValue;
  if (sample == 2)
    hipLaunchKernelGGL(head_fwd_kernel<true>, dim3(grid), dim3(256), 0, stream, (const bf16*)X,
                       (const bf16*)Wp, bp, mask, action, rng, sample, pairs, unit_cell, unit_row,
                       grp_start, grp_count, totals, S, cell_lp, cell_ent, pair_out,
                       (const int*)nullptr, 0);
  else
    hipLaunchKernelGGL(head_fwd_kernel<false>, dim3(grid), dim3(256), 0, stream, (const bf16*)X,
                       (const bf16*)Wp, bp, mask, action, rng, sample, pairs, unit_cell, unit_row,
                       grp_start, grp_count, totals, S, cell_lp, cell_ent, pair_out,
                       (const int*)nullptr, 0);
  return (int)hipGetLastError();
}

extern "C" int mbk_head_fwd_counts(const void* X, const void* Wp, const float* bp,
                                   const uint32_t* mask, uint8_t* action, const uint64_t* rng,
                                   const int* bucket, const int* cnt, int E, int S, int grid,
                                   float* cell_lp, int greedy, hipStream_t stream) {
  if (S < 1 || S > kMaxUnitCells - 1 || !cnt) return (int)hipErrorInvalidValue;
  if (greedy)
    hipLaunchKernelGGL(head_fwd_kernel<true>, dim3(grid), dim3(256), 0, stream, (const bf16*)X,
                       (const bf16*)Wp, bp, mask, action, rng, 2, bucket, (const int*)nullptr,
                       (const int*)nullptr, (const int*)nullptr, (const int*)nullptr,
                       (const int*)nullptr, S, cell_lp, (float*)nullptr, 0, cnt, E);
  else
    hipLaunchKernelGGL(head_fwd_kernel<false>, dim3(grid), dim3(256), 0, stream, (const bf16*)X,
                       (const bf16*)Wp, bp, mask, action, rng, 1, bucket, (const int*)nullptr,
                       (const int*)nullptr, (const int*)nullptr, (const int*)nullptr,
                       (const int*)nullptr, S, cell_lp, (float*)nullptr, 0, cnt, E);
  return (int)hipGetLastError();
}

extern "C" int mbk_head_pair_rowsum(const int* pidx, const uint32_t* abits, int F, int S,
                                    const float* plp, const float* pent, float* logp, float* ent,
                                    hipStream_t stream) {
  if (F <= 0) return 0;
  hipLaunchKernelGGL(head_pair_rowsum_kernel, dim3((F + 255) / 256), dim3(256), 0, stream, pidx,
                     abits, F, S, plp, pent, logp, ent);
  return (int)hipGetLastError();
}

extern "C" int mbk_head_bwd(const void* X, const void* Wp, const void* WpT, const float* bp,
                            const uint32_t* mask, const uint8_t* action, const int* pairs,
                            const int* grp_start, const int* grp_count, const int* chunk_cell,
                            const int* chunk_row, const int* chunk_start, const int* totals,
                            const float* g_logp, const float* g_ent, int S, int grid, void* dXp,
                            float* dWp, float* dbp, float* dW, float* db, const float* stats,
                            hipStream_t stream) {
  int bwd_grid = 1;
  {
    const int cus = mbk::cu_count();
    static uint64_t* hb_stamps = nullptr;
    static bool init = false;
    if (!init) {
      init = true;
      hipFuncSetAttribute((const void*)head_bwd2_kernel<false>,
                          hipFuncAttributeMaxDynamicSharedMemorySize, HB_LDS);
      hipFuncSetAttribute((const void*)head_bwd2_kernel<true>,
                          hipFuncAttributeMaxDynamicSharedMemorySize, HB_LDS);
      if (getenv("MBK_HB_STAMPS")) {
        hipMalloc(&hb_stamps, (size_t)cus * 64 * 8);
        hipMemset(hb_stamps, 0, (size_t)cus * 64 * 8);
      }
    }
    const int g2 = std::max(1, std::min(grid, cus));
    bwd_grid = g2;
    hipLaunchKernelGGL(stats ? head_bwd2_kernel<true> : head_bwd2_kernel<false>, dim3(g2),
                       dim3(64 * HB_NW), HB_LDS, stream, (const bf16*)X, (const bf16*)Wp, bp,
                       mask, action, pairs, grp_start, grp_count, chunk_cell, chunk_row, totals,
                       g_logp, g_ent, S, (bf16*)dXp, dWp, dbp, hb_stamps, stats);
    if (hb_stamps) {
      std::vector<uint64_t> h((size_t)g2 * 64);
      hipMemcpyAsync(h.data(), hb_stamps, h.size() * 8, hipMemcpyDeviceToHost, stream);
      hipStreamSynchronize(stream);
      double acc[8] = {0};
      int n = 0;
      for (int b = 0; b < g2; ++b)
        for (int t = 1; t < 8; ++t) {
          const uint64_t* r = &h[((size_t)b * 8 + t) * 8];
          if (!r[0] || !r[7]) continue;
          for (int k = 0; k < 7; ++k) acc[k] += (double)(r[k + 1] - r[k]) * 0.01;
          ++n;
        }
      fprintf(stderr, "head_bwd2 phases (us, %d tiles): store+W %.2f | loads+Z %.2f | dZ %.2f | "
              "B2 %.2f | dX %.2f | dW %.2f | end %.2f\n", n, acc[0] / n, acc[1] / n, acc[2] / n,
              acc[3] / n, acc[4] / n, acc[5] / n, acc[6] / n);
      hipMemsetAsync(hb_stamps, 0, h.size() * 8, stream);
    }
  }
  dim3 g2((kCell * KD + kCell + 255) / 256, S);
  hipLaunchKernelGGL(head_dw_reduce_kernel, g2, dim3(256), 0, stream, dWp, dbp, chunk_start,
                     grp_count, totals, bwd_grid, S, dW, db);
  return (int)hipGetLastError();
}

extern "C" int mbk_head_score(const void* X, const void* Wp, const float* bp,
                              const uint32_t* mask, const uint8_t* action, const int* pairs,
                              const int* grp_start, const int* grp_count, const int* chunk_cell,
                              const int* chunk_row, const int* totals, int S, float* plp,
                              float* pent, float* stats, hipStream_t stream) {
  const int cus = mbk::cu_count();
  static bool init = false;
  if (!init) {
    init = true;
    hipFuncSetAttribute((const void*)head_score_kernel,
                        hipFuncAttributeMaxDynamicSharedMemorySize, HS_LDS);
  }
  hipLaunchKernelGGL(head_score_kernel, dim3(cus), dim3(64 * HS_NW), HS_LDS, stream,
                     (const bf16*)X, (const bf16*)Wp, bp, mask, action, pairs, grp_start,
                     grp_count, chunk_cell, chunk_row, totals, S, plp, pent, stats);
  return (int)hipGetLastError();
}

extern "C" int mbk_head_dx_gather(const void* dXp, const int* pidx, const uint32_t* abits, int F,
                                  int S, float* dX, hipStream_t stream) {
  hipLaunchKernelGGL(head_dx_gather_kernel, dim3((F + 3) / 4), dim3(256), 0, stream,
                     (const bf16*)dXp, pidx, abits, F, S, dX);
  return (int)hipGetLastError();
}

extern "C" int mbk_head_dx_value_parts(int R) {
  const int cus = mbk::cu_count();
  const int need = (R + 3) / 4;
  return need < 1 ? 1 : (need < cus * 4 ? need : cus * 4);
}

extern "C" int mbk_head_dx_value(const void* dXp, const int* pidx, const uint32_t* abits, int F,
                                 int S, const float* dv, const void* h, const float* wc, int R,
                                 void* dh, float* partial, int parts, hipStream_t stream) {
  if (R <= 0) return 0;
  if (F > R || parts < 1) return (int)hipErrorInvalidValue;
  hipLaunchKernelGGL(head_dx_value_kernel, dim3(parts), dim3(256), 0, stream, (const bf16*)dXp,
                     pidx, abits, F, S, dv, (const bf16*)h, wc, R, (bf16*)dh, partial);
  return (int)hipGetLastError();
}

extern "C" int mbk_head_pack(const float* W, const float* b, int S, void* Wp, float* bp, void* WpT,
                             hipStream_t stream) {
  size_t tot = (size_t)S * (NP * KD + (WpT ? KD * NPT : 0) + NP);
  size_t blocks = (tot + 255) / 256;
  if (blocks > 4096) blocks = 4096;
  hipLaunchKernelGGL(head_pack_kernel, dim3((unsigned)blocks), dim3(256), 0, stream, W, b, S,
                     (bf16*)Wp, bp, (bf16*)WpT);
  return (int)hipGetLastError();
}

extern "C" int mbk_act_head(const MbkActModel* m, const MbkActStep* s, hipStream_t stream) {
  if (!m || !s || m->E <= 0) return (int)hipErrorInvalidValue;
  const int S = m->H * m->W;
  if (S < 1 || S > kMaxUnitCells - 1 || (S & 3)) return (int)hipErrorInvalidValue;
  if (!m->feat || !m->Wp || !m->bp || !m->rng || !m->bucket || !m->bucket_cnt || !m->cellx ||
      !m->pending || !s->mask || !s->action || (!s->act16 && !s->act_list) ||
      !s->logp)
    return (int)hipErrorInvalidValue;
  if ((uintptr_t)m->cellx & 7) return (int)hipErrorInvalidValue;
  HeadActArgs a{};
  a.X = (const bf16*)m->feat;
  a.Wp = (const bf16*)m->Wp;
  a.bp = m->bp;
  a.mask = s->mask;
  a.action = s->action;
  a.rng = m->rng;
  a.bucket = m->bucket;
  a.cnt = m->bucket_cnt + (s->step & 1) * S;
  a.cellx = m->cellx;
  a.act16 = s->act16;
  a.act_list = s->act_list;
  a.list_stride = s->list_stride;
  a.logp = s->logp;
  a.pending = m->pending;
  a.step = s->step;
  a.S = S;
  a.E = m->E;
  const int cus = mbk::cu_count();
  hipLaunchKernelGGL(s->greedy ? head_act_greedy_kernel : head_act_kernel,
                     dim3(std::max(1, cus * 6 / HA_NW)), dim3(64 * HA_NW), 0, stream, a);
  return (int)hipGetLastError();
}

extern "C" int mbk_act_trunk(const MbkActModel* m, const MbkActStep* s, hipStream_t stream);

extern "C" int mbk_act_step(const MbkActModel* m, const MbkActStep* s, hipStream_t stream) {
  const int rc = mbk_act_trunk(m, s, stream);
  if (rc) return rc;
  return mbk_act_head(m, s, stream);
}
```

### microbeast_amd/csrc/runtime/bindings.cpp

```cpp
#include <cstring>
#include <pybind11/pybind11.h>
#include <pybind11/stl.h>

#include <memory>

#include <hip/hip_runtime_api.h>

#include "engine.h"
#include "shm_ring.h"
#include "vec_env.h"

namespace py = pybind11;
using namespace mb;

namespace {

template <typename T>
T* P(uintptr_t a) { return reinterpret_cast<T*>(a); }

struct PyVecEnv {
  std::unique_ptr<VecEnv> env;
  EpisodeLog log;
  PyVecEnv(int size, int n, int max_steps, uint64_t seed, std::vector<int> bots,
           std::vector<float> rw, int base)
// ... 45 lines not shown
                               P<float>(ep_ret), P<int32_t>(ep_step), &e.log);
           },
           py::arg("actions"), py::arg("obs"), py::arg("mask"), py::arg("reward"),
           py::arg("done"), py::arg("ep_return") = 0, py::arg("ep_step") = 0)
      .def("dense_obs", [](PyVecEnv& e, uintptr_t out) { e.env->dense_obs(P<float>(out)); })
      .def("dense_mask", [](PyVecEnv& e, uintptr_t out) { e.env->dense_mask(P<uint8_t>(out)); })
      .def("drain_episodes", [](PyVecEnv& e) { return records_to_list(e.log.drain()); })
      .def("set_bot", [](PyVecEnv& e, int i, int bot) { e.env->sim(i).set_bot(bot); })
      .def("bot", [](PyVecEnv& e, int i) { return e.env->sim(i).bot(); })
      .def("preroll",
           [](PyVecEnv& e, int max_pre, uint64_t seed, int n_threads) {
             py::gil_scoped_release g;
             return e.env->preroll(max_pre, seed, n_threads);
           },
           py::arg("max_pre"), py::arg("seed"), py::arg("n_threads") = 1)
      .def("set_external_opponent",
           [](PyVecEnv& e, bool on) {
             for (int i = 0; i < e.env->num_envs(); ++i) e.env->sim(i).set_external_opponent(on);
           })
      .def("obs_p1",
           [](PyVecEnv& e, uintptr_t out) {
             const size_t S = (size_t)e.env->size() * e.env->size();
             for (int i = 0; i < e.env->num_envs(); ++i)
               e.env->sim(i).write_obs_p1(P<uint32_t>(out) + i * S);
           })
      .def("mask_p1",
           [](PyVecEnv& e, uintptr_t out) {
             const size_t S = (size_t)e.env->size() * e.env->size();
             for (int i = 0; i < e.env->num_envs(); ++i)
               e.env->sim(i).write_mask_p1(P<uint32_t>(out) + i * S * kMaskWords);
           })
      .def("set_opponent_actions",
           [](PyVecEnv& e, uintptr_t act) {
             const size_t S = (size_t)e.env->size() * e.env->size();
             for (int i = 0; i < e.env->num_envs(); ++i)
               e.env->sim(i).set_opponent_actions(P<uint8_t>(act) + i * S * kActComps);
           })
      .def("ticks", [](PyVecEnv& e, int i) { return e.env->sim(i).ticks(); })
      .def("set_validate", [](PyVecEnv& e, bool on) { e.env->set_validate(on); })
      .def("obs_codes",
           [](PyVecEnv& e, uintptr_t codes, uintptr_t res) {
             const size_t S = (size_t)e.env->size() * e.env->size();
             for (int i = 0; i < e.env->num_envs(); ++i) {
               e.env->sim(i).write_obs_codes(P<uint16_t>(codes) + i * S);
               P<int32_t>(res)[i] = e.env->sim(i).resources(0);
             }
           })
      .def("set_external_opponent_range",
           [](PyVecEnv& e, int e0, int e1, bool on) { e.env->set_external_opponent(e0, e1, on); })
      .def("obs_codes_p1",
           [](PyVecEnv& e, uintptr_t codes, uintptr_t res) {
             const size_t S = (size_t)e.env->size() * e.env->size();
             for (int i = 0; i < e.env->num_envs(); ++i) {
               e.env->sim(i).write_obs_codes_as(1, P<uint16_t>(codes) + i * S);
               P<int32_t>(res)[i] = e.env->sim(i).resources(1);
             }
           })
      .def("step_codes_sp",
           [](PyVecEnv& e, uintptr_t act16, uintptr_t opp16, uintptr_t codes, uintptr_t res,
              uintptr_t codes_p1, uintptr_t res_p1, uintptr_t rew, uintptr_t done, int opponent) {
             py::gil_scoped_release g;
             e.env->step_range_codes_sp(0, e.env->num_envs(), P<uint16_t>(act16),
                                        P<uint16_t>(opp16), P<uint16_t>(codes), P<int32_t>(res),
                                        P<uint16_t>(codes_p1), P<int32_t>(res_p1), P<float>(rew),
                                        P<uint8_t>(done), &e.log, opponent);
           })
      .def("step_codes",
           [](PyVecEnv& e, uintptr_t act16, uintptr_t codes, uintptr_t res, uintptr_t rew,
              uintptr_t done) {
             py::gil_scoped_release g;
             e.env->step_range_codes(0, e.env->num_envs(), P<uint16_t>(act16), P<uint16_t>(codes),
                                     P<int32_t>(res), P<float>(rew), P<uint8_t>(done), &e.log);
           })
      .def("code_lists",
           [](PyVecEnv& e, uintptr_t lists, int stride, int player) {
             e.env->write_code_lists(P<uint32_t>(lists), stride, player);
           },
           py::arg("lists"), py::arg("stride"), py::arg("player") = 0)
      .def("step_lists_sp",
           [](PyVecEnv& e, uintptr_t acts, uintptr_t opp_acts, uintptr_t lists,
              uintptr_t lists_p1, int stride, uintptr_t rew, uintptr_t done, int opponent) {
             py::gil_scoped_release g;
             return e.env->step_range_lists_sp(0, e.env->num_envs(), P<uint32_t>(acts),
                                               P<uint32_t>(opp_acts), P<uint32_t>(lists),
                                               P<uint32_t>(lists_p1), stride, P<float>(rew),
                                               P<uint8_t>(done), &e.log, opponent);
           });

  py::class_<IndexRing>(m, "IndexRing")
      .def(py::init([](uintptr_t addr, size_t cap, bool init) {
             return new IndexRing(P<void>(addr), cap, init);
           }),
           py::arg("addr"), py::arg("capacity"), py::arg("init"))
      .def_static("bytes_needed", &IndexRing::bytes_needed)
      .def("try_push", &IndexRing::try_push)
      .def("try_pop",
           [](IndexRing& r) -> py::object {
             int64_t v;
             if (r.try_pop(&v)) return py::int_(v);
             return py::none();
           })
      .def("push",
           [](IndexRing& r, int64_t v, double timeout) {
             py::gil_scoped_release g;
             return r.push(v, timeout);
           },
           py::arg("value"), py::arg("timeout") = -1.0)
      .def("pop",
           [](IndexRing& r, double timeout) -> py::object {
             int64_t v;
             bool ok;
             {
               py::gil_scoped_release g;
               ok = r.pop(&v, timeout);
             }
             if (ok) return py::int_(v);
             return py::none();
           },
           py::arg("timeout") = -1.0)
      .def("size", &IndexRing::size)
      .def("capacity", &IndexRing::capacity)
      .def("close", &IndexRing::close)
      .def("closed", &IndexRing::closed);

  m.def("seqlock_write_begin",
        [](uintptr_t ver) { return seqlock_write_begin(P<std::atomic<uint64_t>>(ver)); });
  m.def("seqlock_write_end", [](uintptr_t ver) { seqlock_write_end(P<std::atomic<uint64_t>>(ver)); });
  m.def("seqlock_write",
        [](uintptr_t ver, uintptr_t src, uintptr_t dst, size_t n) {
          py::gil_scoped_release g;
          seqlock_write(P<std::atomic<uint64_t>>(ver), P<const void>(src), P<void>(dst), n);
        },
        py::arg("ver"), py::arg("src"), py::arg("dst"), py::arg("nbytes"));
  m.def("seqlock_read",
        [](uintptr_t ver, uintptr_t src, uintptr_t dst, size_t n, int tries) {
          py::gil_scoped_release g;
          return seqlock_read(P<const std::atomic<uint64_t>>(ver), P<const void>(src), P<void>(dst),
                              n, tries);
        },
        py::arg("ver"), py::arg("src"), py::arg("dst"), py::arg("nbytes"),
        py::arg("max_tries") = 1000);

  m.def("host_register", [](uintptr_t addr, size_t nbytes) -> int {
    return (int)hipHostRegister(P<void>(addr), nbytes, hipHostRegisterDefault);
  });
  m.def("host_unregister", [](uintptr_t addr) -> int {
    return (int)hipHostUnregister(P<void>(addr));
  });
  m.def("memcpy2d_async", [](uintptr_t dst, size_t dpitch, uintptr_t src, size_t spitch,
                             size_t width, size_t height, uintptr_t stream) -> int {
    return (int)hipMemcpy2DAsync(P<void>(dst), dpitch, P<const void>(src), spitch, width, height,
                                 hipMemcpyDefault, (hipStream_t)stream);
  });

  py::class_<GpuEngine>(m, "GpuEngine")
      .def(py::init([](py::dict c, py::dict b) {
        EngineConfig cfg;
        cfg.size = c["size"].cast<int>();
        cfg.n_groups = c["n_groups"].cast<int>();
        cfg.envs_per_group = c["envs_per_group"].cast<int>();
        cfg.unroll = c["unroll"].cast<int>();
        cfg.n_slots = c["n_slots"].cast<int>();
        cfg.n_threads = c["n_threads"].cast<int>();
        cfg.max_steps = c["max_steps"].cast<int>();
        cfg.seed = c["seed"].cast<uint64_t>();
        cfg.bots = c["bots"].cast<std::vector<int>>();
        cfg.reward_weight = c["reward_weight"].cast<std::vector<float>>();
        cfg.env_index_base = c["env_index_base"].cast<int>();
        cfg.device = c["device"].cast<int>();
        if (c.contains("selfplay_groups")) cfg.selfplay_groups = c["selfplay_groups"].cast<int>();
        if (c.contains("n_lanes")) cfg.n_lanes = c["n_lanes"].cast<int>();
        if (c.contains("preroll")) cfg.preroll = c["preroll"].cast<int>();
        EngineBuffers buf;
        buf.obs = b["obs"].cast<uintptr_t>();
        buf.mask = b["mask"].cast<uintptr_t>();
        buf.action = b["action"].cast<uintptr_t>();
        buf.logp = b["logp"].cast<uintptr_t>();
        buf.value = b["value"].cast<uintptr_t>();
        buf.reward = b["reward"].cast<uintptr_t>();
        buf.done = b["done"].cast<uintptr_t>();
        auto opt = [&](const char* k) {
          return b.contains(k) ? b[k].cast<uintptr_t>() : (uintptr_t)0;
        };
        buf.ep_return = opt("ep_return");
        buf.ep_step = opt("ep_step");
        buf.last_action0 = opt("last_action0");
        buf.logits = opt("policy_logits");
        buf.abits = opt("abits");
        auto get = [](py::dict d, const char* k) {
          return d.contains(k) ? d[k].cast<uintptr_t>() : (uintptr_t)0;
        };
        for (auto item : b["lanes"].cast<py::list>()) {
          py::dict d = item.cast<py::dict>();
          LaneIO io;
          io.in_obs = get(d, "in_obs");
          io.in_mask = get(d, "in_mask");
          io.out_action = get(d, "out_action");
          io.out_logp = get(d, "out_logp");
          io.out_value = get(d, "out_value");
          io.in_codes = get(d, "in_codes");
          io.in_res = get(d, "in_res");
          io.out_act16 = get(d, "out_act16");
          io.in_codes_p1 = get(d, "in_codes_p1");
          io.in_res_p1 = get(d, "in_res_p1");
          io.out_act16_p1 = get(d, "out_act16_p1");
          io.out_logits = get(d, "out_logits");
          buf.lanes.push_back(io);
        }
        return new GpuEngine(cfg, buf);
      }))
      .def("start",
           [](GpuEngine& e, std::vector<std::vector<uintptr_t>> graphs) {
             std::vector<LaneGraphs> lg;
             for (const auto& t : graphs) {
               if (t.size() != 4)
                 throw std::runtime_error("start: need 4 graph handles per lane");
               lg.push_back(LaneGraphs{t[0], t[1], t[2], t[3]});
             }
             e.start(lg);
           })
      .def("stop", [](GpuEngine& e) { py::gil_scoped_release g; e.stop(); })
      .def("get_full",
           [](GpuEngine& e, int n, double timeout) {
             py::gil_scoped_release g;
             return e.get_full(n, timeout);
           },
           py::arg("n"), py::arg("timeout") = -1.0)
      .def("stream_wait_full", &GpuEngine::stream_wait_full)
      .def("release", &GpuEngine::release)
      .def("publish", &GpuEngine::publish, py::arg("src"), py::arg("dsts"), py::arg("nbytes"),
           py::arg("stream"), py::arg("version") = -1)
      .def("slot_version", &GpuEngine::slot_version)
      .def("set_policy_version", &GpuEngine::set_policy_version)
      .def("publish_opponent", &GpuEngine::publish_opponent)
      .def("set_initial_opponent", &GpuEngine::set_initial_opponent)
      .def("drain_episodes", [](GpuEngine& e) { return records_to_list(e.drain_episodes()); })
      .def("stream", &GpuEngine::stream, py::arg("lane") = 0)
      .def("failed", &GpuEngine::failed)
      .def("host_codes", &GpuEngine::host_codes)
      .def("host_res", &GpuEngine::host_res)
      .def("host_act16", &GpuEngine::host_act16)
      .def("set_act_models",
           [](GpuEngine& e, std::vector<py::bytes> blocks, std::vector<py::bytes> opp_blocks) {
             auto unpack = [](const std::vector<py::bytes>& bs) {
               std::vector<MbkActModel> ms;
               for (const py::bytes& b : bs) {
                 const std::string raw = b;
                 if (raw.size() != sizeof(MbkActModel))
                   throw std::runtime_error("set_act_models: block size " +
                                            std::to_string(raw.size()) +
                                            " != sizeof(MbkActModel) " +
                                            std::to_string(sizeof(MbkActModel)));
                 MbkActModel m;
                 std::memcpy(&m, raw.data(), sizeof(m));
                 ms.push_back(m);
               }
               return ms;
             };
             e.set_act_models(unpack(blocks), unpack(opp_blocks));
           },
           py::arg("blocks"),
           py::arg("opp_blocks") = std::vector<py::bytes>{})
      .def("act_mode", &GpuEngine::act_mode)
      .def("set_sparse_io", &GpuEngine::set_sparse_io)
      .def("set_greedy", &GpuEngine::set_greedy)
      .def("greedy", &GpuEngine::greedy)
      .def("sparse_io", &GpuEngine::sparse_io)
      .def_static("act_model_size", [] { return (int)sizeof(MbkActModel); })
      .def("inject_fault", &GpuEngine::inject_fault)
      .def("code_rows", [](GpuEngine& e) {
        return py::make_tuple((uintptr_t)e.host_code_list(), e.list_stride());
      })
      .def("error", &GpuEngine::error)
      .def("stats", [](GpuEngine& e) {
        EngineStats s = e.stats();
        py::dict d;
        d["frames"] = s.frames;
        d["gpu_steps"] = s.gpu_steps;
        d["slots_full"] = s.slots_full;
        d["full_depth"] = s.full_depth;
        d["driver_idle_s"] = s.driver_idle_s;
        d["gpu_phase_s"] = s.gpu_phase_s;
        d["step_h2d_s"] = s.step_h2d_s;
        d["step_graph_s"] = s.step_graph_s;
        d["step_out_s"] = s.step_out_s;
        d["timed_steps"] = s.timed_steps;
        d["env_phase_s"] = s.env_phase_s;
        d["enqueue_s"] = s.enqueue_s;
        d["graph_launch_s"] = s.graph_launch_s;
        d["act_steps"] = s.act_steps;
        d["act_active_cells"] = s.act_active_cells;
        d["slot_wait_s"] = s.slot_wait_s;
        d["env_s"] = s.env_s;
        d["publishes"] = s.publishes;
        d["opp_publishes"] = s.opp_publishes;
        d["opp_version"] = s.opp_version;
        d["preroll_steps"] = s.preroll_steps;
        return d;
      });
}
```

### microbeast_amd/csrc/runtime/engine.cpp

```cpp
#include "engine.h"


#include <chrono>
#include <cstdlib>

#include <pthread.h>
#include <sched.h>
#include <cstring>
#include <stdexcept>
#include <string>

#include "../include/mbk_api.h"

namespace mb {

#define ENG_CHECK(expr)                                                              \
  do {                                                                               \
    hipError_t _e = (expr);                                                          \
    if (_e != hipSuccess) {                                                          \
      fail(std::string(#expr) + " failed: " + hipGetErrorString(_e));                \
      return false;                                                                  \
    }                                                                                \
  } while (0)

#define CTOR_CHECK(expr)                                                             \
  do {                                                                               \
    hipError_t _e = (expr);                                                          \
    if (_e != hipSuccess)                                                            \
      throw std::runtime_error(std::string(#expr) + " failed: " + hipGetErrorString(_e)); \
  } while (0)

GpuEngine::GpuEngine(const EngineConfig& cfg, const EngineBuffers& buf) : cfg_(cfg), buf_(buf) {
  if (cfg_.n_groups < 1 || cfg_.envs_per_group < 1 || cfg_.unroll < 1)
    throw std::runtime_error("GpuEngine: bad config");
  if (cfg_.n_slots < cfg_.n_groups + 1)
    throw std::runtime_error("GpuEngine: need n_slots >= n_groups + 1");
  S_ = cfg_.size * cfg_.size;
  const size_t E = cfg_.envs_per_group, T1 = cfg_.unroll + 1;
  slot_stride_obs_ = T1 * E * S_ * 4;
  slot_stride_mask_ = T1 * E * S_ * 4 * kMaskWords;
  slot_stride_act_ = T1 * E * S_ * kActComps;
  slot_stride_scalar_ = T1 * E;
  const int total = cfg_.n_groups * cfg_.envs_per_group;
  env_.reset(new VecEnv(cfg_.size, total, cfg_.max_steps, cfg_.seed, cfg_.bots,
                        cfg_.reward_weight.empty() ? nullptr : cfg_.reward_weight.data(),
                        cfg_.env_index_base));
  CTOR_CHECK(hipSetDevice(cfg_.device));
  if (cfg_.n_lanes < 1 || (int)buf_.lanes.size() != cfg_.n_lanes)
    throw std::runtime_error("GpuEngine: need one LaneIO per lane");
  int prio_least = 0, prio_greatest = 0;
  CTOR_CHECK(hipDeviceGetStreamPriorityRange(&prio_least, &prio_greatest));
  lanes_.resize(cfg_.n_lanes);
  for (int l = 0; l < cfg_.n_lanes; ++l) {
    Lane& L = lanes_[l];
    L.io = buf_.lanes[l];
    if (!L.io.in_codes || !L.io.in_res || !L.io.out_act16)
      throw std::runtime_error("GpuEngine: in_codes / in_res / out_act16 buffers required");
    CTOR_CHECK(hipStreamCreateWithPriority(&L.stream, hipStreamNonBlocking, prio_greatest));
  }
  CTOR_CHECK(hipHostMalloc((void**)&h_codes_, (size_t)total * S_ * 2, hipHostMallocDefault));
  CTOR_CHECK(hipHostMalloc((void**)&h_res_, (size_t)total * 4, hipHostMallocDefault));
  CTOR_CHECK(hipHostMalloc((void**)&h_act16_, (size_t)total * S_ * 2, hipHostMallocDefault));
  CTOR_CHECK(hipHostMalloc((void**)&h_reward_, (size_t)total * 4, hipHostMallocDefault));
  CTOR_CHECK(hipHostMalloc((void**)&h_done_, (size_t)total, hipHostMallocDefault));
  std::memset(h_reward_, 0, (size_t)total * 4);
  std::memset(h_done_, 0, (size_t)total);
  if (buf_.ep_return || buf_.ep_step) {
    CTOR_CHECK(hipHostMalloc((void**)&h_ep_return_, (size_t)total * 4, hipHostMallocDefault));
    CTOR_CHECK(hipHostMalloc((void**)&h_ep_step_, (size_t)total * 4, hipHostMallocDefault));
    std::memset(h_ep_return_, 0, (size_t)total * 4);
    std::memset(h_ep_step_, 0, (size_t)total * 4);
  }
  if (cfg_.selfplay_groups < 0 || cfg_.selfplay_groups > cfg_.n_groups)
    throw std::runtime_error("GpuEngine: bad selfplay_groups");
  const int sp0 = cfg_.n_groups - cfg_.selfplay_groups;
  if (cfg_.selfplay_groups > 0) {
    for (const Lane& L : lanes_)
      if (!L.io.in_codes_p1 || !L.io.in_res_p1 || !L.io.out_act16_p1)
        throw std::runtime_error(
            "GpuEngine: self-play needs in_codes_p1 / in_res_p1 / out_act16_p1");
    CTOR_CHECK(hipHostMalloc((void**)&h_codes_p1_, (size_t)total * S_ * 2, hipHostMallocDefault));
    CTOR_CHECK(hipHostMalloc((void**)&h_res_p1_, (size_t)total * 4, hipHostMallocDefault));
    CTOR_CHECK(hipHostMalloc((void**)&h_act16_p1_, (size_t)total * S_ * 2, hipHostMallocDefault));
    std::memset(h_act16_p1_, 0, (size_t)total * S_ * 2);
    env_->set_external_opponent(sp0 * cfg_.envs_per_group, total, true);
  }
  if (cfg_.preroll > 1) {
    env_->reset_codes(nullptr, nullptr);
    preroll_steps_ = env_->preroll(cfg_.preroll, cfg_.seed, std::max(1, cfg_.n_threads));
    env_->set_validate(false);
    env_->write_codes(h_codes_, h_res_);
  } else {
    env_->set_validate(false);
    env_->reset_codes(h_codes_, h_res_);
  }
  if (cfg_.selfplay_groups > 0) env_->reset_codes_p1(h_codes_p1_, h_res_p1_);
  {
    const char* st = std::getenv("MBK_STEP_TIMING");
    step_timing_ = st && st[0] == '1';
  }
  for (int g = 0; g < cfg_.n_groups; ++g) {
    groups_.emplace_back(new Group());
    CTOR_CHECK(hipEventCreateWithFlags(&groups_[g]->ev, hipEventDisableTiming));
    if (step_timing_)
      for (auto& e : groups_[g]->tev) CTOR_CHECK(hipEventCreate(&e));
    groups_[g]->selfplay = g >= sp0;
    groups_[g]->lane = g % cfg_.n_lanes;
    groups_[g]->phase.store(READY);
  }
  full_ev_.resize(cfg_.n_slots);
  release_ev_.resize(cfg_.n_slots);
  release_pending_.assign(cfg_.n_slots, 0);
  slot_version_.assign(cfg_.n_slots, 0);
  for (int s = 0; s < cfg_.n_slots; ++s) {
    CTOR_CHECK(hipEventCreateWithFlags(&full_ev_[s], hipEventDisableTiming));
    CTOR_CHECK(hipEventCreateWithFlags(&release_ev_[s], hipEventDisableTiming));
    free_slots_.push_back(s);
  }
  for (PubChan& c : pub_) {
    CTOR_CHECK(hipEventCreateWithFlags(&c.ready, hipEventDisableTiming));
    c.pending.assign(cfg_.n_lanes, false);
    c.dst.assign(cfg_.n_lanes, 0);
    c.consumed.assign(cfg_.n_lanes, nullptr);
    for (auto& ev : c.consumed) CTOR_CHECK(hipEventCreateWithFlags(&ev, hipEventDisableTiming));
  }
  chunk_ = std::max(1, std::min(16, cfg_.envs_per_group / std::max(1, 2 * cfg_.n_threads)));
}

GpuEngine::~GpuEngine() {
  stop();
  for (Lane& L : lanes_)
    if (L.stream) hipStreamSynchronize(L.stream);
  for (auto& g : groups_) {
    if (g->ev) hipEventDestroy(g->ev);
    for (auto e : g->tev)
      if (e) hipEventDestroy(e);
  }
  for (auto e : full_ev_) hipEventDestroy(e);
  for (auto e : release_ev_) hipEventDestroy(e);
  for (PubChan& c : pub_) {
    if (c.ready) hipEventDestroy(c.ready);
    for (auto ev : c.consumed)
      if (ev) hipEventDestroy(ev);
    if (c.staging) hipFree(c.staging);
  }
  if (h_codes_p1_) hipHostFree(h_codes_p1_);
  if (h_res_p1_) hipHostFree(h_res_p1_);
  if (h_act16_p1_) hipHostFree(h_act16_p1_);
  if (h_codes_) hipHostFree(h_codes_);
  if (h_res_) hipHostFree(h_res_);
  if (h_act16_) hipHostFree(h_act16_);
  if (h_reward_) hipHostFree(h_reward_);
  if (h_ep_return_) hipHostFree(h_ep_return_);
  if (h_ep_step_) hipHostFree(h_ep_step_);
  if (h_done_) hipHostFree(h_done_);
  if (h_code_list_) hipHostFree(h_code_list_);
  if (h_act_list_) hipHostFree(h_act_list_);
  if (h_code_list_p1_) hipHostFree(h_code_list_p1_);
  if (h_act_list_p1_) hipHostFree(h_act_list_p1_);
  for (Lane& L : lanes_) {
    if (L.opp_scratch) hipFree(L.opp_scratch);
    if (L.stream) hipStreamDestroy(L.stream);
  }
}

void GpuEngine::fail(const std::string& msg) {
  {
    std::lock_guard<std::mutex> g(err_m_);
    if (err_.empty()) err_ = msg;
  }
  failed_.store(true);
  running_.store(false);
  work_cv_.notify_all();
  full_cv_.notify_all();
}

std::string GpuEngine::error() const {
  std::lock_guard<std::mutex> g(err_m_);
  return err_;
}

void GpuEngine::start(const std::vector<LaneGraphs>& graphs) {
  if (running_.load()) return;
  if ((int)graphs.size() != cfg_.n_lanes)
    throw std::runtime_error("GpuEngine::start: need one LaneGraphs per lane");
  for (int l = 0; l < cfg_.n_lanes; ++l) {
    const LaneGraphs& g = graphs[l];
    if (!g.policy) throw std::runtime_error("GpuEngine::start: missing policy graph");
    if (cfg_.selfplay_groups > 0 && !g.opp)
      throw std::runtime_error("GpuEngine::start: self-play groups need the opponent graph");
    Lane& L = lanes_[l];
    L.graph = (hipGraphExec_t)g.policy;
    L.opp_graph = (hipGraphExec_t)g.opp;
    L.pack_graph[0] = (hipGraphExec_t)g.pack;
    L.pack_graph[1] = (hipGraphExec_t)g.opp_pack;
  }
  started_ = true;
  running_.store(true);
  for (int w = 0; w < cfg_.n_threads; ++w) workers_.emplace_back(&GpuEngine::worker_loop, this, w);
  driver_ = std::thread(&GpuEngine::driver_loop, this);
}

void GpuEngine::alloc_rows() {
  if (h_code_list_) return;
  const size_t total = (size_t)cfg_.n_groups * cfg_.envs_per_group;
  list_stride_ = (S_ + 1 + 3) & ~3;
  const size_t bytes = total * list_stride_ * 4;
  if (hipHostMalloc((void**)&h_code_list_, bytes, hipHostMallocDefault) != hipSuccess ||
      hipHostMalloc((void**)&h_act_list_, bytes, hipHostMallocDefault) != hipSuccess)
    throw std::runtime_error("GpuEngine: hipHostMalloc of the sparse rows failed");
  std::memset(h_act_list_, 0, bytes);
  env_->write_code_lists(h_code_list_, list_stride_);
  if (cfg_.selfplay_groups > 0) {
    if (hipHostMalloc((void**)&h_code_list_p1_, bytes, hipHostMallocDefault) != hipSuccess ||
        hipHostMalloc((void**)&h_act_list_p1_, bytes, hipHostMallocDefault) != hipSuccess)
      throw std::runtime_error("GpuEngine: hipHostMalloc of the opponent rows failed");
    std::memset(h_act_list_p1_, 0, bytes);
    std::memset(h_code_list_p1_, 0, bytes);
    env_->write_code_lists(h_code_list_p1_, list_stride_, 1);
  }
}

void GpuEngine::set_greedy(bool on) {
  if (started_ || running_.load()) throw std::runtime_error("set_greedy: engine already started");
  greedy_ = on;
}

void GpuEngine::set_sparse_io(bool on) {
  if (running_.load()) throw std::runtime_error("set_sparse_io: engine running");
  if (!on) { sparse_ = false; return; }
  if (act_mode()) return;
  if (buf_.ep_return || buf_.ep_step)
    throw std::runtime_error("set_sparse_io: not with the reference buffer keys");
  alloc_rows();
  sparse_ = true;
}

void GpuEngine::set_act_models(const std::vector<MbkActModel>& models,
                               const std::vector<MbkActModel>& opp_models) {
  if (running_.load()) throw std::runtime_error("set_act_models: engine running");
  if (!models.empty() && (int)models.size() != cfg_.n_lanes)
    throw std::runtime_error("set_act_models: need one model per lane");
  if (!models.empty() && (buf_.ep_return || buf_.ep_step || buf_.last_action0 || buf_.logits))
    throw std::runtime_error("set_act_models: not with reference buffer keys");
  const bool sp_needed = !models.empty() && cfg_.selfplay_groups > 0;
  if (sp_needed && (int)opp_models.size() != cfg_.n_lanes)
    throw std::runtime_error("set_act_models: self-play needs one opponent block per lane");
  if (!sp_needed && !opp_models.empty())
    throw std::runtime_error("set_act_models: opponent blocks without self-play groups");
  for (const std::vector<MbkActModel>* v : {&models, &opp_models})
    for (const MbkActModel& m : *v)
      if (m.E != cfg_.envs_per_group || m.H != cfg_.size || m.W != cfg_.size)
        throw std::runtime_error("set_act_models: model block shape mismatch");
  act_models_ = models;
  opp_act_models_ = opp_models;
  sparse_ = !models.empty();
  if (sparse_) alloc_rows();
  if (sp_needed) {
    const size_t E = cfg_.envs_per_group, sc = E * S_ * (4 + 12 + 8) + 2 * E * 4 + 256;
    for (Lane& L : lanes_)
      if (!L.opp_scratch && hipMalloc((void**)&L.opp_scratch, sc) != hipSuccess)
        throw std::runtime_error("set_act_models: hipMalloc of the opponent scratch failed");
  }
}

void GpuEngine::stop() {
  running_.store(false);
  work_cv_.notify_all();
  full_cv_.notify_all();
  if (driver_.joinable()) driver_.join();
  for (auto& t : workers_) if (t.joinable()) t.join();
  workers_.clear();
  for (Lane& L : lanes_)
    if (L.stream) hipStreamSynchronize(L.stream);
}

void GpuEngine::dispatch_env(int g) {
  Group& G = *groups_[g];
  const auto now = std::chrono::steady_clock::now();
  gpu_phase_ns_.fetch_add(
      std::chrono::duration_cast<std::chrono::nanoseconds>(now - G.t_phase).count(),
      std::memory_order_relaxed);
  G.t_phase = now;
  if (G.timed) {
    float ms[3] = {0.f, 0.f, 0.f};
    bool ok = true;
    for (int i = 0; i < 3; ++i)
      ok = ok && hipEventElapsedTime(&ms[i], G.tev[i], G.tev[i + 1]) == hipSuccess;
    if (ok) {
      step_h2d_ns_.fetch_add((int64_t)(ms[0] * 1e6), std::memory_order_relaxed);
      step_graph_ns_.fetch_add((int64_t)(ms[1] * 1e6), std::memory_order_relaxed);
      step_out_ns_.fetch_add((int64_t)(ms[2] * 1e6), std::memory_order_relaxed);
      timed_steps_.fetch_add(1, std::memory_order_relaxed);
    }
    G.timed = false;
  }
  G.idle.store(0, std::memory_order_relaxed);
  G.phase.store(ENV_BUSY, std::memory_order_release);
  G.remaining.store(cfg_.envs_per_group, std::memory_order_release);
  G.next_env.store(0, std::memory_order_release);
  {
    std::lock_guard<std::mutex> l(work_m_);
    work_epoch_.fetch_add(1);
  }
  work_cv_.notify_all();
}

void GpuEngine::worker_loop(int wid) {
  const int E = cfg_.envs_per_group, NG = cfg_.n_groups;
  while (running_.load(std::memory_order_relaxed)) {
    const uint64_t epoch = work_epoch_.load();
    bool did = false;
    for (int k = 0; k < NG; ++k) {
      const int g = (wid + k) % NG;
      Group& G = *groups_[g];
      if (G.phase.load(std::memory_order_acquire) != ENV_BUSY) continue;
      for (;;) {
        int e = G.next_env.fetch_add(chunk_);
        if (e >= E) break;
        int e1 = std::min(e + chunk_, E);
        const int a0 = g * E;
        auto t0 = std::chrono::steady_clock::now();
        try {
          if (inject_fault_.exchange(0) != 0)
            throw std::runtime_error("injected env-worker fault (--fault_inject_every)");
          if (sparse_ && G.selfplay)
            G.idle.fetch_add(env_->step_range_lists_sp(a0 + e, a0 + e1, h_act_list_,
                                                       h_act_list_p1_, h_code_list_,
                                                       h_code_list_p1_, list_stride_, h_reward_,
                                                       h_done_, &log_, G.opp_version),
                             std::memory_order_relaxed);
          else if (sparse_)
            G.idle.fetch_add(env_->step_range_lists(a0 + e, a0 + e1, h_act_list_, h_code_list_,
                                                    list_stride_, h_reward_, h_done_, &log_),
                             std::memory_order_relaxed);
          else if (G.selfplay)
            env_->step_range_codes_sp(a0 + e, a0 + e1, h_act16_, h_act16_p1_, h_codes_, h_res_,
                                      h_codes_p1_, h_res_p1_, h_reward_, h_done_, &log_,
                                      G.opp_version, h_ep_return_, h_ep_step_);
          else
            env_->step_range_codes(a0 + e, a0 + e1, h_act16_, h_codes_, h_res_, h_reward_,
                                   h_done_, &log_, h_ep_return_, h_ep_step_);
        } catch (const std::exception& ex) {
          fail("env worker " + std::to_string(wid) + ": " + ex.what());
          return;
        }
        env_ns_.fetch_add(std::chrono::duration_cast<std::chrono::nanoseconds>(
                              std::chrono::steady_clock::now() - t0).count(),
                          std::memory_order_relaxed);
        frames_.fetch_add(e1 - e, std::memory_order_relaxed);
        did = true;
        if (G.remaining.fetch_sub(e1 - e) == e1 - e) {
          G.t_ready_ns.store(std::chrono::duration_cast<std::chrono::nanoseconds>(
                                 std::chrono::steady_clock::now().time_since_epoch()).count(),
                             std::memory_order_relaxed);
          G.phase.store(READY, std::memory_order_release);
        }
      }
    }
    if (!did) {
      std::unique_lock<std::mutex> l(work_m_);
      work_cv_.wait_for(l, std::chrono::milliseconds(2),
                        [&] { return work_epoch_.load() != epoch || !running_.load(); });
    }
  }
}

bool GpuEngine::enqueue_gpu(int g) {
  const auto t_enq = std::chrono::steady_clock::now();
  struct Timer {
    std::atomic<int64_t>& acc;
    std::chrono::steady_clock::time_point t0;
    ~Timer() {
      acc.fetch_add(std::chrono::duration_cast<std::chrono::nanoseconds>(
                        std::chrono::steady_clock::now() - t0).count(),
                    std::memory_order_relaxed);
    }
  } timer{enqueue_ns_, t_enq};
  Group& G = *groups_[g];
  Lane& L = lanes_[G.lane];
  hipStream_t st = L.stream;
  const LaneIO& io = L.io;
  const size_t E = cfg_.envs_per_group, T = cfg_.unroll;
  {
    std::lock_guard<std::mutex> l(pub_m_);
    const int ln = G.lane;
    for (int c = 0; c < 2; ++c) {
      PubChan& P = pub_[c];
      if (!P.pending[ln]) continue;
      if (hipEventQuery(P.ready) == hipErrorNotReady) continue;
      ENG_CHECK(hipStreamWaitEvent(st, P.ready, 0));
      ENG_CHECK(hipMemcpyAsync((void*)P.dst[ln], P.staging, P.n, hipMemcpyDeviceToDevice,
                               st));
      ENG_CHECK(hipEventRecord(P.consumed[ln], st));
      if (L.pack_graph[c]) ENG_CHECK(hipGraphLaunch(L.pack_graph[c], st));
      P.pending[ln] = false;
      if (c == 1) L.opp_version = P.version;
      else if (P.version >= 0) L.policy_version = P.version;
      bool all = true;
      for (bool pl : P.pending) all = all && !pl;
      if (all) {
        if (c == 0) publishes_.fetch_add(1);
        else {
          opp_version_pub_.store(P.version);
          opp_publishes_.fetch_add(1);
        }
      }
    }
  }
  if (G.t == 0) {
    auto waiting = [&] {
      for (int w : slot_wait_q_) if (w == g) return true;
      return false;
    };
    if (!slot_wait_q_.empty() && slot_wait_q_.front() != g) {
      if (!waiting()) slot_wait_q_.push_back(g);
      return false;
    }
    int slot = -1;
    bool pending = false;
    {
      std::lock_guard<std::mutex> l(slot_m_);
      for (auto it = free_slots_.begin(); it != free_slots_.end(); ++it) {
        const int s = *it;
        if (release_pending_[s]) {
          const hipError_t q = hipEventQuery(release_ev_[s]);
          if (q == hipErrorNotReady) continue;
          if (q == hipSuccess) release_pending_[s] = 0;
        }
        slot = s;
        pending = release_pending_[s] != 0;
        free_slots_.erase(it);
        break;
      }
    }
    if (slot < 0) {
      if (!waiting()) slot_wait_q_.push_back(g);
      return false;
    }
    if (!slot_wait_q_.empty() && slot_wait_q_.front() == g) slot_wait_q_.pop_front();
    if (pending) ENG_CHECK(hipStreamWaitEvent(st, release_ev_[slot], 0));
    G.cur = slot;
    slot_version_[slot] = L.policy_version;
  }
  const size_t e0 = (size_t)g * E;
  G.timed = step_timing_;
  const size_t t = G.t;
  auto obs_at = [&](int slot, size_t i) {
    return (char*)buf_.obs + slot * slot_stride_obs_ + i * E * S_ * 4;
  };
  auto mask_at = [&](int slot, size_t i) {
    return (char*)buf_.mask + slot * slot_stride_mask_ + i * E * S_ * 4 * kMaskWords;
  };
  auto act_at = [&](int slot, size_t i) {
    return (char*)buf_.action + slot * slot_stride_act_ + i * E * S_ * kActComps;
  };
  auto f32_at = [&](uintptr_t base, int slot, size_t i) {
    return (char*)base + (slot * slot_stride_scalar_ + i * E) * 4;
  };
  auto u8_at = [&](uintptr_t base, int slot, size_t i) {
    return (char*)base + (slot * slot_stride_scalar_ + i * E);
  };
  const bool close_prev = (t == 0 && G.prev >= 0);
  const int rs = t > 0 ? G.cur : G.prev;
  const size_t ri = t > 0 ? t - 1 : T - 1;
  if (act_mode()) {
    const MbkActModel& M = act_models_[G.lane];
    if (G.timed) ENG_CHECK(hipEventRecord(G.tev[0], st));
    if (G.timed) ENG_CHECK(hipEventRecord(G.tev[1], st));
    MbkActStep a{};
    a.code_list = h_code_list_ + e0 * list_stride_;
    a.act_list = h_act_list_ + e0 * list_stride_;
    a.list_stride = list_stride_;
    a.obs = (uint32_t*)obs_at(G.cur, t);
    a.mask = (uint32_t*)mask_at(G.cur, t);
    if (close_prev) {
      a.obs2 = (uint32_t*)obs_at(G.prev, T);
      a.mask2 = (uint32_t*)mask_at(G.prev, T);
    }
    a.action = (uint8_t*)act_at(G.cur, t);
    if (buf_.abits) {
      const size_t sw = (size_t)(S_ + 31) / 32;
      auto ab_at = [&](int slot, size_t i) {
        return (uint32_t*)buf_.abits + (slot * slot_stride_scalar_ + i * E) * sw;
      };
      a.abits = ab_at(G.cur, t);
      if (close_prev) a.abits2 = ab_at(G.prev, T);
    }
    a.logp = (float*)f32_at(buf_.logp, G.cur, t);
    a.value = (float*)f32_at(buf_.value, G.cur, t);
    if (!G.first) {
      a.reward_src = h_reward_ + e0;
      a.done_src = h_done_ + e0;
      a.reward_dst = (float*)f32_at(buf_.reward, rs, ri);
      a.done_dst = (uint8_t*)u8_at(buf_.done, rs, ri);
    }
    a.step = L.act_step++;
    a.greedy = greedy_ ? 1 : 0;
    act_active_cells_.fetch_add(G.idle.load(std::memory_order_relaxed), std::memory_order_relaxed);
    act_steps_.fetch_add(1, std::memory_order_relaxed);
    {
      const auto t0 = std::chrono::steady_clock::now();
      ENG_CHECK((hipError_t)mbk_act_step(&M, &a, st));
      if (G.selfplay) {
        const size_t ES = E * S_;
        uint8_t* sc = L.opp_scratch;
        MbkActStep o{};
        o.code_list = h_code_list_p1_ + e0 * list_stride_;
        o.act_list = h_act_list_p1_ + e0 * list_stride_;
        o.list_stride = list_stride_;
        o.obs = (uint32_t*)sc;
        o.mask = (uint32_t*)(sc + ES * 4);
        o.action = sc + ES * 16;
        o.logp = (float*)(sc + ES * 24);
        o.value = (float*)(sc + ES * 24 + E * 4);
        o.step = L.opp_act_step++;
        ENG_CHECK((hipError_t)mbk_act_step(&opp_act_models_[G.lane], &o, st));
        G.opp_version = L.opp_version;
      }
      launch_ns_.fetch_add(std::chrono::duration_cast<std::chrono::nanoseconds>(
                               std::chrono::steady_clock::now() - t0).count(),
                           std::memory_order_relaxed);
    }
    if (G.timed) ENG_CHECK(hipEventRecord(G.tev[2], st));
    if (close_prev) {
      ENG_CHECK(hipEventRecord(full_ev_[G.prev], st));
      {
        std::lock_guard<std::mutex> l(slot_m_);
        full_slots_.push_back(G.prev);
      }
      slots_full_.fetch_add(1);
      full_cv_.notify_all();
      G.prev = -1;
    }
    if (G.timed) ENG_CHECK(hipEventRecord(G.tev[3], st));
    ENG_CHECK(hipEventRecord(G.ev, st));
  } else {
    const uintptr_t in_codes = io.in_codes, in_res = io.in_res, out_act16 = io.out_act16;
    if (G.timed) ENG_CHECK(hipEventRecord(G.tev[0], st));
    if (sparse_) {
      ENG_CHECK((hipError_t)mbk_rows_to_codes(h_code_list_ + e0 * list_stride_, list_stride_,
                                              (int)E, S_, (void*)in_codes, (int32_t*)in_res,
                                              st));
    } else {
      ENG_CHECK(hipMemcpyAsync((void*)in_codes, h_codes_ + e0 * S_, E * S_ * 2,
                               hipMemcpyHostToDevice, st));
      ENG_CHECK(hipMemcpyAsync((void*)in_res, h_res_ + e0, E * 4, hipMemcpyHostToDevice, st));
    }
    if (G.timed) ENG_CHECK(hipEventRecord(G.tev[1], st));
    {
      const auto t0 = std::chrono::steady_clock::now();
      ENG_CHECK(hipGraphLaunch(L.graph, st));
      launch_ns_.fetch_add(std::chrono::duration_cast<std::chrono::nanoseconds>(
                               std::chrono::steady_clock::now() - t0).count(),
                           std::memory_order_relaxed);
    }
    if (G.selfplay) {
// ... 23 lines not shown
      seg[n++] = {(const void*)(h_reward_ + e0), f32_at(buf_.reward, rs, ri), E * 4};
      seg[n++] = {(const void*)(h_done_ + e0), u8_at(buf_.done, rs, ri), E};
      if (buf_.ep_return)
        seg[n++] = {(const void*)(h_ep_return_ + e0), f32_at(buf_.ep_return, rs, ri), E * 4};
      if (buf_.ep_step)
        seg[n++] = {(const void*)(h_ep_step_ + e0), f32_at(buf_.ep_step, rs, ri), E * 4};
    }
    if (buf_.logits && io.out_logits)
      seg[n++] = {(const void*)io.out_logits,
                  (char*)buf_.logits + (G.cur * slot_stride_scalar_ + t * E) * (size_t)S_ * 78 * 4,
                  E * (size_t)S_ * 78 * 4};
    if (close_prev && buf_.last_action0)
      seg[n++] = {(const void*)act_at(G.prev, T - 1),
                  (char*)buf_.last_action0 + (size_t)G.cur * E * S_ * kActComps,
                  E * S_ * kActComps};
    if (close_prev) {
      seg[n++] = {(const void*)io.in_obs, obs_at(G.prev, T), E * S_ * 4};
      seg[n++] = {(const void*)io.in_mask, mask_at(G.prev, T), E * S_ * 4 * kMaskWords};
    }
    ENG_CHECK((hipError_t)mbk_multi_copy(seg, n, st));
    if (close_prev) {
      ENG_CHECK(hipEventRecord(full_ev_[G.prev], st));
      {
        std::lock_guard<std::mutex> l(slot_m_);
        full_slots_.push_back(G.prev);
      }
      slots_full_.fetch_add(1);
      full_cv_.notify_all();
      G.prev = -1;
    }
    if (sparse_) {
      ENG_CHECK((hipError_t)mbk_codes_to_rows((const void*)out_act16, (int)E, S_,
                                              h_act_list_ + e0 * list_stride_, list_stride_,
                                              st));
      if (G.selfplay)
        ENG_CHECK((hipError_t)mbk_codes_to_rows((const void*)io.out_act16_p1, (int)E, S_,
                                                h_act_list_p1_ + e0 * list_stride_,
                                                list_stride_, st));
    } else {
      ENG_CHECK(hipMemcpyAsync(h_act16_ + e0 * S_, (const void*)out_act16, E * S_ * 2,
                               hipMemcpyDeviceToHost, st));
      if (G.selfplay)
        ENG_CHECK(hipMemcpyAsync(h_act16_p1_ + e0 * S_, (const void*)io.out_act16_p1,
                                 E * S_ * 2, hipMemcpyDeviceToHost, st));
    }
    if (G.timed) ENG_CHECK(hipEventRecord(G.tev[3], st));
    ENG_CHECK(hipEventRecord(G.ev, st));
  }
  gpu_steps_.fetch_add(1);
  G.t += 1;
  if (G.t == (int)T) {
    G.t = 0;
    G.prev = G.cur;
    G.cur = -1;
  }
  G.first = false;
  {
    const auto now = std::chrono::steady_clock::now();
    const int64_t rdy = G.t_ready_ns.exchange(0, std::memory_order_relaxed);
    if (rdy > 0)
      env_phase_ns_.fetch_add(
          rdy - std::chrono::duration_cast<std::chrono::nanoseconds>(
                    G.t_phase.time_since_epoch()).count(),
          std::memory_order_relaxed);
    G.t_phase = now;
  }
  G.phase.store(ON_GPU, std::memory_order_release);
  return true;
}

void GpuEngine::driver_loop() {
  hipSetDevice(cfg_.device);
  const int NG = cfg_.n_groups;
  int idle_spins = 0;
  auto idle_t0 = std::chrono::steady_clock::now();
  bool idle = false;
  double stall_s = 0.0;
  while (running_.load(std::memory_order_relaxed)) {
    bool progressed = false, stalled = false;
    for (int g = 0; g < NG && running_.load(std::memory_order_relaxed); ++g) {
      Group& G = *groups_[g];
      int ph = G.phase.load(std::memory_order_acquire);
      if (ph == READY) {
        if (enqueue_gpu(g)) progressed = true;
        else if (failed_.load()) return;
        else stalled = true;
      } else if (ph == ON_GPU) {
        hipError_t q = hipEventQuery(G.ev);
        if (q == hipSuccess) {
          dispatch_env(g);
          progressed = true;
        } else if (q != hipErrorNotReady) {
          fail(std::string("hipEventQuery: ") + hipGetErrorString(q));
          return;
        }
      }
    }
    if (progressed) {
      if (idle) {
        double dt = std::chrono::duration<double>(std::chrono::steady_clock::now() - idle_t0).count();
        std::lock_guard<std::mutex> l(stats_m_);
        driver_idle_s_ += dt;
        if (stall_s > 0) slot_wait_s_ += dt;
      }
      idle = false;
      idle_spins = 0;
      stall_s = 0.0;
    } else {
      if (!idle) { idle = true; idle_t0 = std::chrono::steady_clock::now(); }
      if (stalled) stall_s = 1.0;
      if (++idle_spins < 256) {
        __builtin_ia32_pause();
      } else if (idle_spins < 2048) {
        std::this_thread::yield();
      } else {
        std::this_thread::sleep_for(std::chrono::microseconds(20));
      }
    }
  }
}

std::vector<int> GpuEngine::get_full(int n, double timeout_s) {
  std::unique_lock<std::mutex> l(slot_m_);
  auto pred = [&] { return (int)full_slots_.size() >= n || !running_.load() || failed_.load(); };
  if (timeout_s < 0) full_cv_.wait(l, pred);
  else full_cv_.wait_for(l, std::chrono::duration<double>(timeout_s), pred);
  std::vector<int> out;
  if ((int)full_slots_.size() < n) return out;
  for (int i = 0; i < n; ++i) { out.push_back(full_slots_.front()); full_slots_.pop_front(); }
  return out;
}

void GpuEngine::stream_wait_full(uintptr_t stream, int slot) {
  hipError_t e = hipStreamWaitEvent((hipStream_t)stream, full_ev_[slot], 0);
  if (e != hipSuccess) throw std::runtime_error(std::string("stream_wait_full: ") + hipGetErrorString(e));
}

void GpuEngine::release(const std::vector<int>& slots, uintptr_t stream) {
  for (int s : slots) {
    hipError_t e = hipEventRecord(release_ev_[s], (hipStream_t)stream);
    if (e != hipSuccess) throw std::runtime_error(std::string("release: ") + hipGetErrorString(e));
  }
  std::lock_guard<std::mutex> l(slot_m_);
  for (int s : slots) {
    release_pending_[s] = 1;
    free_slots_.push_back(s);
  }
}

bool GpuEngine::publish_chan(int chan, uintptr_t src, const std::vector<uintptr_t>& dsts,
                             size_t nbytes, uintptr_t stream, int version) {
  std::lock_guard<std::mutex> l(pub_m_);
  PubChan& P = pub_[chan];
  if ((int)dsts.size() != cfg_.n_lanes)
    throw std::runtime_error("publish: need one destination per lane");
  for (bool pl : P.pending)
    if (pl) return false;
  hipStream_t s = (hipStream_t)stream;
  if (nbytes > P.staging_n) {
    if (P.staging) {
      for (Lane& L : lanes_) hipStreamSynchronize(L.stream);
      hipFree(P.staging);
    }
    if (hipMalloc((void**)&P.staging, nbytes) != hipSuccess)
      throw std::runtime_error("publish: hipMalloc staging failed");
    P.staging_n = nbytes;
  }
  for (hipEvent_t ev : P.consumed) hipStreamWaitEvent(s, ev, 0);
  hipMemcpyAsync(P.staging, (const void*)src, nbytes, hipMemcpyDeviceToDevice, s);
  hipEventRecord(P.ready, s);
  P.dst = dsts;
  P.n = nbytes;
  P.version = version;
  P.pending.assign(cfg_.n_lanes, true);
  return true;
}

EngineStats GpuEngine::stats() const {
  EngineStats s;
  s.frames = frames_.load();
  s.gpu_steps = gpu_steps_.load();
  s.slots_full = slots_full_.load();
  s.env_s = env_ns_.load() * 1e-9;
  s.gpu_phase_s = gpu_phase_ns_.load() * 1e-9;
  s.step_h2d_s = step_h2d_ns_.load() * 1e-9;
  s.step_graph_s = step_graph_ns_.load() * 1e-9;
  s.step_out_s = step_out_ns_.load() * 1e-9;
  s.timed_steps = timed_steps_.load();
  s.preroll_steps = preroll_steps_;
  s.env_phase_s = env_phase_ns_.load() * 1e-9;
  s.enqueue_s = enqueue_ns_.load() * 1e-9;
  s.graph_launch_s = launch_ns_.load() * 1e-9;
  s.publishes = publishes_.load();
  s.opp_publishes = opp_publishes_.load();
  s.opp_version = opp_version_pub_.load();
  s.act_steps = act_steps_.load();
  s.act_active_cells = act_active_cells_.load();
  {
    std::lock_guard<std::mutex> q(slot_m_);
    s.full_depth = (int)full_slots_.size();
  }
  std::lock_guard<std::mutex> l(stats_m_);
  s.driver_idle_s = driver_idle_s_;
  s.slot_wait_s = slot_wait_s_;
  return s;
}

}
```

### microbeast_amd/csrc/runtime/engine.h

```cpp
#pragma once
#include <hip/hip_runtime_api.h>

#include <atomic>
#include <chrono>
#include <condition_variable>
#include <cstdint>
#include <cstdlib>
#include <deque>
#include <memory>
#include <mutex>
#include <thread>
#include <vector>

#include "vec_env.h"
#include "../include/mbk_api.h"

namespace mb {

struct EngineConfig {
  int size = 16;
  int n_groups = 2;
  int envs_per_group = 256;
  int unroll = 64;
  int n_slots = 8;
  int n_threads = 8;
  int max_steps = 2000;
  uint64_t seed = 1;
  std::vector<int> bots;
  std::vector<float> reward_weight;
  int env_index_base = 0;
  int device = 0;
  int selfplay_groups = 0;
  int n_lanes = 1;
  int preroll = 0;
};

struct LaneIO {
  uintptr_t in_obs = 0, in_mask = 0, out_action = 0, out_logp = 0, out_value = 0;
  uintptr_t in_codes = 0, in_res = 0, out_act16 = 0;
  uintptr_t in_codes_p1 = 0, in_res_p1 = 0, out_act16_p1 = 0;
  uintptr_t out_logits = 0;
};

struct LaneGraphs {
  uintptr_t policy = 0, opp = 0, pack = 0, opp_pack = 0;
};

struct EngineBuffers {
  uintptr_t obs = 0;
  uintptr_t mask = 0;
  uintptr_t action = 0;
  uintptr_t logp = 0;
  uintptr_t value = 0;
  uintptr_t reward = 0;
  uintptr_t done = 0;
  uintptr_t ep_return = 0;
  uintptr_t ep_step = 0;
  uintptr_t last_action0 = 0;
  uintptr_t logits = 0;
  uintptr_t abits = 0;
  std::vector<LaneIO> lanes;
};

struct EngineStats {
  int64_t frames = 0;
  int64_t gpu_steps = 0;
  int64_t slots_full = 0;
  int full_depth = 0;
  double driver_idle_s = 0.0;
  double slot_wait_s = 0.0;
  double env_s = 0.0;
  double gpu_phase_s = 0.0;
  double env_phase_s = 0.0;
  double enqueue_s = 0.0;
  double graph_launch_s = 0.0;
  double step_h2d_s = 0.0, step_graph_s = 0.0, step_out_s = 0.0;
  int64_t timed_steps = 0;
  int64_t publishes = 0;
  int64_t opp_publishes = 0;
  int opp_version = -1;
  int64_t act_steps = 0, act_active_cells = 0;
  int64_t preroll_steps = 0;
};

class GpuEngine {
 public:
  GpuEngine(const EngineConfig& cfg, const EngineBuffers& buf);
  ~GpuEngine();
  void start(const std::vector<LaneGraphs>& graphs);
  void stop();
  std::vector<int> get_full(int n, double timeout_s);
  void stream_wait_full(uintptr_t stream, int slot);
  void release(const std::vector<int>& slots, uintptr_t stream);
  bool publish(uintptr_t src, const std::vector<uintptr_t>& dsts, size_t nbytes,
               uintptr_t stream, int version = -1) {
    return publish_chan(0, src, dsts, nbytes, stream, version);
  }
  int slot_version(int slot) const { return slot_version_.at(slot); }
  void set_policy_version(int version) {
    for (auto& L : lanes_) L.policy_version = version;
  }
  void set_initial_opponent(int version) {
    for (auto& L : lanes_) L.opp_version = version;
    opp_version_pub_.store(version);
  }
  bool publish_opponent(uintptr_t src, const std::vector<uintptr_t>& dsts, size_t nbytes,
                        uintptr_t stream, int version) {
    return publish_chan(1, src, dsts, nbytes, stream, version);
  }
  std::vector<EpisodeRecord> drain_episodes() { return log_.drain(); }
  EngineStats stats() const;
  uintptr_t stream(int lane = 0) const { return (uintptr_t)lanes_.at(lane).stream; }
  uintptr_t host_codes() const { return (uintptr_t)h_codes_; }
  uintptr_t host_res() const { return (uintptr_t)h_res_; }
  uintptr_t host_act16() const { return (uintptr_t)h_act16_; }
  uintptr_t host_code_list() const { return (uintptr_t)h_code_list_; }
  uintptr_t host_act_list() const { return (uintptr_t)h_act_list_; }
  int list_stride() const { return list_stride_; }
  void set_act_models(const std::vector<MbkActModel>& models,
                      const std::vector<MbkActModel>& opp_models = {});
  bool act_mode() const { return !act_models_.empty(); }
  void set_sparse_io(bool on);
  bool sparse_io() const { return sparse_; }
  void set_greedy(bool on);
  bool greedy() const { return greedy_; }
  const EngineConfig& config() const { return cfg_; }
  VecEnv& env() { return *env_; }
  bool failed() const { return failed_.load(); }
  void inject_fault() { inject_fault_.store(1); }
  std::string error() const;

 private:
  enum Phase : int { ENV_BUSY = 0, READY = 1, ON_GPU = 2 };
  struct Group {
    std::atomic<int> phase{ENV_BUSY};
    std::atomic<int> next_env{0};
    std::atomic<int> remaining{0};
    std::atomic<int> idle{0};
    int cur = -1, prev = -1, t = 0;
    bool first = true;
    bool selfplay = false;
    int opp_version = -1;
    int lane = 0;
    hipEvent_t ev = nullptr;
    hipEvent_t tev[4] = {nullptr, nullptr, nullptr, nullptr};
    bool timed = false;
    std::chrono::steady_clock::time_point t_phase;
    std::atomic<int64_t> t_ready_ns{0};
  };
  struct PubChan {
    std::vector<bool> pending;
    std::vector<uintptr_t> dst;
    size_t n = 0;
    int version = -1;
    hipEvent_t ready = nullptr;
    std::vector<hipEvent_t> consumed;
    uint8_t* staging = nullptr;
    size_t staging_n = 0;
  };
  struct Lane {
    hipStream_t stream = nullptr;
    hipGraphExec_t graph = nullptr, opp_graph = nullptr;
    hipGraphExec_t pack_graph[2] = {nullptr, nullptr};
    LaneIO io;
    int opp_version = -1;
    int policy_version = 0;
    uint64_t act_step = 0;
    uint8_t* opp_scratch = nullptr;
    uint64_t opp_act_step = 0;
  };

  EngineConfig cfg_;
  EngineBuffers buf_;
  int S_;
  size_t slot_stride_obs_, slot_stride_mask_, slot_stride_act_, slot_stride_scalar_;
  std::unique_ptr<VecEnv> env_;
  EpisodeLog log_;
  std::vector<Lane> lanes_;
  std::vector<std::unique_ptr<Group>> groups_;
  uint16_t* h_codes_ = nullptr;
  int32_t* h_res_ = nullptr;
  float* h_reward_ = nullptr;
  uint8_t* h_done_ = nullptr;
  uint16_t* h_act16_ = nullptr;
  uint16_t* h_codes_p1_ = nullptr;
  int32_t* h_res_p1_ = nullptr;
  uint16_t* h_act16_p1_ = nullptr;
  float* h_ep_return_ = nullptr;
  int32_t* h_ep_step_ = nullptr;

  mutable std::mutex slot_m_;
  std::condition_variable full_cv_;
  std::deque<int> free_slots_, full_slots_;
  std::vector<hipEvent_t> full_ev_, release_ev_;
  int64_t preroll_steps_ = 0;
  std::vector<uint8_t> release_pending_;
  std::vector<int> slot_version_;
  std::deque<int> slot_wait_q_;

  std::mutex pub_m_;
  PubChan pub_[2];
  bool publish_chan(int chan, uintptr_t src, const std::vector<uintptr_t>& dsts, size_t nbytes,
                    uintptr_t stream, int version);

  std::vector<std::thread> workers_;
  std::thread driver_;
  std::mutex work_m_;
  std::condition_variable work_cv_;
  std::atomic<uint64_t> work_epoch_{0};
  std::atomic<bool> running_{false};
  bool started_ = false;
  bool greedy_ = false;
  std::atomic<bool> failed_{false};
  std::atomic<int> inject_fault_{0};
  mutable std::mutex err_m_;
  std::string err_;

  std::atomic<int64_t> frames_{0}, gpu_steps_{0}, slots_full_{0}, publishes_{0}, opp_publishes_{0};
  std::atomic<int> opp_version_pub_{-1};
  std::atomic<int64_t> env_ns_{0};
  std::atomic<int64_t> gpu_phase_ns_{0}, env_phase_ns_{0}, enqueue_ns_{0}, launch_ns_{0};
  bool step_timing_ = false;
  std::atomic<int64_t> step_h2d_ns_{0}, step_graph_ns_{0}, step_out_ns_{0}, timed_steps_{0};
  std::atomic<int64_t> act_steps_{0}, act_active_cells_{0};
  double driver_idle_s_ = 0.0, slot_wait_s_ = 0.0;
  mutable std::mutex stats_m_;

  void worker_loop(int wid);
  void driver_loop();
  bool enqueue_gpu(int g);
  void dispatch_env(int g);
  void fail(const std::string& msg);
  void alloc_rows();
  int chunk_;
  std::vector<MbkActModel> act_models_;
  std::vector<MbkActModel> opp_act_models_;
  bool sparse_ = false;
  int list_stride_ = 0;
  uint32_t* h_code_list_ = nullptr;
  uint32_t* h_act_list_ = nullptr;
  uint32_t* h_code_list_p1_ = nullptr;
  uint32_t* h_act_list_p1_ = nullptr;
};

}
```

### microbeast_amd/runtime/gpu_actors.py

```python
from __future__ import annotations

import os

import torch

from .. import _native as N
from ..ops import act as act_ops
from ..ops.pixconv import pbc_to_cell_major
from ..ops import cell_head
from ..ops.copy import zeros
from ..ops.optim import FlatParams

BOT_IDS = {"coac": 0, "random_biased": 1, "light_rush": 2, "worker_rush": 3, "passive": 4,
           "random": 5}
DEFAULT_BOTS = ("coac", "coac", "coac", "random_biased", "light_rush", "worker_rush")


def available_cpus() -> int:
    try:
        n = len(os.sched_getaffinity(0))
    except AttributeError:
        n = os.cpu_count() or 1
    try:
        with open("/sys/fs/cgroup/cpu.max") as f:
            q, p = f.read().split()
            if q != "max":
                n = min(n, max(1, int(int(q) / int(p))))
    except (OSError, ValueError):
        pass
    return n


class EngineFailure(RuntimeError):
    """The native engine stopped (an env worker raised, or a HIP call failed); the learner
    process is intact and may rebuild the actor side (train.py)."""


def graph_policy_step(io: dict, m, rng: torch.Tensor, E: int, size: int, device,
                      greedy: bool = False) -> None:
    k = N.kernels()
    st = N.stream_ptr()
    hip = hasattr(m, "_head") and m._use_hip(io["in_obs"])
    packed = False
    if hip:
        head = m._head(device)
        head.ensure_buckets(E)
        N.check(k.mbk_decode_obs_mask_bucket(
            io["in_codes"].data_ptr(), io["in_res"].data_ptr(), E, size, size,
            io["in_obs"].data_ptr(), io["in_mask"].data_ptr(), head.bucket_cnt.data_ptr(),
            head.bucket.data_ptr(), head.cell_lp.data_ptr(), io["out_action"].data_ptr(),
            st), "decode_obs_mask_bucket")
        _, _, value = m.act(io["in_obs"], io["in_mask"], rng, action_out=io["out_action"],
                            logp_out=io["out_logp"], bucketed=True,
                            logits_out=io.get("out_logits"), value_out=io["out_value"],
                            act16_out=io["out_act16"], greedy=greedy)
        packed = True
    else:
        N.check(k.mbk_decode_obs_mask(io["in_codes"].data_ptr(), io["in_res"].data_ptr(),
                                      E, size, size, io["in_obs"].data_ptr(),
                                      io["in_mask"].data_ptr(), st), "decode_obs_mask")
        if hasattr(m, "policy_value_pbc") and m._use_hip(io["in_obs"]):
            if "out_logits" in io:
                logits, value = m.policy_value_pbc(io["in_obs"])
                io["out_logits"].copy_(pbc_to_cell_major(logits).reshape(io["out_logits"].shape))
                cell_head.sample_pbc(logits, io["in_mask"], rng, action_out=io["out_action"],
                                     cell_logp=io["cell_logp"], logp_out=io["out_logp"],
                                     greedy=greedy)
            else:
                _, _, value = m.act(io["in_obs"], io["in_mask"], rng, action_out=io["out_action"],
                                    cell_logp=io["cell_logp"], logp_out=io["out_logp"],
                                    greedy=greedy)
        else:
            logits, value = m.policy_value(io["in_obs"])
            if "out_logits" in io:
                io["out_logits"].copy_(logits.reshape(io["out_logits"].shape))
            cell_head.sample_gpu(logits, io["in_mask"], rng, action_out=io["out_action"],
                                 cell_logp=io["cell_logp"], logp_out=io["out_logp"],
                                 greedy=greedy)
    if value.data_ptr() != io["out_value"].data_ptr():
        io["out_value"].copy_(value.view(-1))
    if not packed:
        N.check(k.mbk_pack_env_actions(io["out_action"].data_ptr(), E * size * size,
                                       io["out_act16"].data_ptr(), N.stream_ptr()),
                "pack_env_actions")


def make_io(E: int, S: int, device, logits: bool = False) -> dict:
    return {
        "in_codes": zeros(E, S, dtype=torch.int16, device=device),
        "in_res": zeros(E, dtype=torch.int32, device=device),
        "out_act16": zeros(E, S, dtype=torch.int16, device=device),
        "in_obs": zeros(E, S, dtype=torch.int32, device=device),
        "in_mask": zeros(E, S, 3, dtype=torch.int32, device=device),
        "out_action": zeros(E, S, 7, dtype=torch.uint8, device=device),
        "out_logp": zeros(E, dtype=torch.float32, device=device),
        "out_value": zeros(E, dtype=torch.float32, device=device),
        "cell_logp": zeros(E * S, dtype=torch.float32, device=device),
    } | ({"out_logits": zeros(E, S * 78, dtype=torch.float32, device=device)} if logits else {})


class GpuActorRuntime:
    def __init__(self, make_model, size: int, n_groups: int, envs_per_group: int, unroll: int,
                 batch_slots: int, device: torch.device, n_threads: int | None = None,
                 n_slots: int | None = None, max_steps: int = 2000, seed: int = 1,
                 bots=DEFAULT_BOTS, reward_weight=(10.0, 1.0, 1.0, 0.2, 1.0, 4.0),
                 env_index_base: int = 0, selfplay_groups: int = 0, fp8_policy: bool = False,
                 n_lanes: int | None = None,
                 reference_keys: bool = False, policy_logits: bool = False,
                 preroll: int = 0, fused_act: bool | None = None, greedy: bool = False):
        rt = N.runtime()
        self.device = device
        self.size, self.S = size, size * size
        self.G, self.E, self.T = n_groups, envs_per_group, unroll
        self.batch_slots = batch_slots
        self.n_slots = n_slots or (2 * n_groups + batch_slots + 1)
        S, E, T1, NS = self.S, self.E, self.T + 1, self.n_slots
        dev = device
        self.rb = {
            "obs": zeros(NS, T1, E, S, dtype=torch.int32, device=dev),
            "mask": zeros(NS, T1, E, S, 3, dtype=torch.int32, device=dev),
            "action": zeros(NS, T1, E, S, 7, dtype=torch.uint8, device=dev),
            "logp": zeros(NS, T1, E, dtype=torch.float32, device=dev),
            "value": zeros(NS, T1, E, dtype=torch.float32, device=dev),
            "reward": zeros(NS, T1, E, dtype=torch.float32, device=dev),
            "done": zeros(NS, T1, E, dtype=torch.uint8, device=dev),
        }
        if S % 32 == 0:
            self.rb["abits"] = zeros(NS, T1, E, S // 32, dtype=torch.int32, device=dev)
        self.reference_keys = reference_keys or policy_logits
        self.emit_logits = policy_logits
        if self.reference_keys:
            self.rb["ep_return"] = zeros(NS, T1, E, dtype=torch.float32, device=dev)
            self.rb["ep_step"] = zeros(NS, T1, E, dtype=torch.int32, device=dev)
            self.rb["last_action0"] = zeros(NS, E, S, 7, dtype=torch.uint8, device=dev)
        if policy_logits:
            self.rb["policy_logits"] = zeros(NS, T1, E, S * 78, dtype=torch.float32,
                                                   device=dev)
        self.n_lanes = max(1, min(n_groups, n_lanes if n_lanes is not None else 1))
        self.fp8_policy = fp8_policy
        self.greedy = bool(greedy)
        self.selfplay_groups = int(selfplay_groups)
        self.lanes = []
        for ln in range(self.n_lanes):
            lane = {"io": self._make_io(),
                    "rng": torch.tensor([seed * 7919 + env_index_base + 15485863 * ln, 0],
                                        dtype=torch.int64, device=dev),
                    "model": make_model().to(dev)}
            lane["model"].eval()
            if fp8_policy:
                lane["model"].fp8_inference = True
            lane["flat"] = FlatParams(lane["model"], dev)
            lane["pack_graph"] = self._capture_pack(lane["model"])
            lane["graph"] = self._capture(lane["io"], lane["model"], lane["rng"], self.greedy)
            if self.selfplay_groups > 0:
                lane["io_p1"] = self._make_io()
                lane["rng_p1"] = torch.tensor(
                    [seed * 7919 + env_index_base + 104729 + 15485863 * ln, 0],
                    dtype=torch.int64, device=dev)
                lane["opp_model"] = make_model().to(dev)
                lane["opp_model"].eval()
                lane["opp_model"].fp8_inference = fp8_policy
                lane["opp_flat"] = FlatParams(lane["opp_model"], dev)
                lane["opp_pack_graph"] = self._capture_pack(lane["opp_model"])
                lane["opp_graph"] = self._capture(lane["io_p1"], lane["opp_model"],
                                                  lane["rng_p1"])
            self.lanes.append(lane)
        l0 = self.lanes[0]
        self.io, self.rng, self.infer_model = l0["io"], l0["rng"], l0["model"]
        self.infer_flat, self.pack_graph, self.graph = l0["flat"], l0["pack_graph"], l0["graph"]
        self.opp_graph = l0.get("opp_graph")
        if self.selfplay_groups > 0:
            self.opp_flat, self.opp_model = l0["opp_flat"], l0["opp_model"]
        if n_threads is None:
            n_threads = max(1, min(32, available_cpus() - 1))
        self.n_threads = n_threads
        cfg = dict(size=size, n_groups=n_groups, envs_per_group=E, unroll=self.T, n_slots=NS,
                   n_threads=n_threads, max_steps=max_steps, seed=seed,
                   bots=[BOT_IDS[b] if isinstance(b, str) else int(b) for b in bots],
                   reward_weight=list(reward_weight), env_index_base=env_index_base,
                   device=dev.index if dev.index is not None else torch.cuda.current_device(),
                   selfplay_groups=self.selfplay_groups, n_lanes=self.n_lanes,
                   preroll=int(preroll))
        bufs = {k: v.data_ptr() for k, v in self.rb.items()}
        bufs["lanes"] = []
        for lane in self.lanes:
            d = {k: v.data_ptr() for k, v in lane["io"].items()}
            if self.selfplay_groups > 0:
                d.update({"in_codes_p1": lane["io_p1"]["in_codes"].data_ptr(),
                          "in_res_p1": lane["io_p1"]["in_res"].data_ptr(),
                          "out_act16_p1": lane["io_p1"]["out_act16"].data_ptr()})
            bufs["lanes"].append(d)
        torch.cuda.synchronize()
        self.engine = rt.GpuEngine(cfg, bufs)
        self.engine.set_greedy(self.greedy)
        self.fused_act = (fused_act is not False and not self.reference_keys
                          and all(act_ops.supported(ln["model"], size, fp8_policy)
                                  for ln in self.lanes))
        if fused_act and not self.fused_act:
            raise ValueError("fused_act=True: the fused acting step does not cover this model "
                             "/ map size / dtype or the reference buffer keys")
        if self.fused_act:
            for lane in self.lanes:
                lane["act"] = act_ops.ActWorkspace(lane["model"], E, lane["rng"], dev)
                if self.selfplay_groups > 0:
                    lane["opp_act"] = act_ops.ActWorkspace(lane["opp_model"], E,
                                                           lane["rng_p1"], dev)
            torch.cuda.synchronize()
            self.engine.set_act_models([ln["act"].block() for ln in self.lanes],
                                       [ln["opp_act"].block() for ln in self.lanes
                                        if "opp_act" in ln])
        self.sparse_io = not self.fused_act and not self.reference_keys
        if self.sparse_io:
            self.engine.set_sparse_io(True)
        if not self.fused_act and "abits" in self.rb:
            self._abits_unwritten = self.rb.pop("abits")
        self.started = False
        self.frames_per_slot = E * self.T

    def _make_io(self):
        return make_io(self.E, self.S, self.device, getattr(self, "emit_logits", False))

    def _policy_step(self, io, m, rng, greedy: bool = False):
        graph_policy_step(io, m, rng, self.E, self.size, self.device, greedy)

    def _capture_pack(self, model):
        if not hasattr(model, "pack_inference"):
            return None
        s = torch.cuda.Stream(device=self.device)
        s.wait_stream(torch.cuda.current_stream())
        with torch.cuda.stream(s):
            model.pack_inference(self.device)
        torch.cuda.current_stream().wait_stream(s)
        torch.cuda.synchronize()
        g = torch.cuda.CUDAGraph()
        with torch.cuda.graph(g, stream=s):
            model.pack_inference(self.device)
        torch.cuda.synchronize()
        return g

    def _capture(self, io, model, rng, greedy: bool = False):
        s = torch.cuda.Stream(device=self.device)
        s.wait_stream(torch.cuda.current_stream())
        with torch.cuda.stream(s):
            for _ in range(3):
                self._policy_step(io, model, rng, greedy)
        torch.cuda.current_stream().wait_stream(s)
        torch.cuda.synchronize()
        g = torch.cuda.CUDAGraph()
        with torch.cuda.graph(g, stream=s):
            self._policy_step(io, model, rng, greedy)
        torch.cuda.synchronize()
        rng[1] = 0
        return g

    def start(self, learner_flat: FlatParams | None = None, opponent_version: int = -1,
              version: int = 0):
        self.engine.set_policy_version(int(version))
        if self.selfplay_groups > 0:
            self.engine.set_initial_opponent(int(opponent_version))
        for lane in self.lanes:
            if learner_flat is not None:
                lane["flat"].data.copy_(learner_flat.data)
                if self.selfplay_groups > 0:
                    lane["opp_flat"].data.copy_(learner_flat.data)
            for pg in (lane["pack_graph"], lane.get("opp_pack_graph")):
                if pg is not None:
                    pg.replay()
        torch.cuda.synchronize()
        ex = lambda g: int(g.raw_cuda_graph_exec()) if g is not None else 0
        self.engine.start([[ex(ln["graph"]), ex(ln.get("opp_graph")), ex(ln["pack_graph"]),
                            ex(ln.get("opp_pack_graph"))]
                           for ln in self.lanes])
        self.started = True

    def stop(self):
        if self.started:
            self.engine.stop()
            self.started = False

    def close(self):
        self.stop()
        self.engine = None
        self.lanes = []
        self.rb = {}
        for k in ("io", "rng", "infer_model", "infer_flat", "pack_graph", "graph", "opp_graph",
                  "opp_flat", "opp_model"):
            if hasattr(self, k):
                setattr(self, k, None)

    def check(self):
        if self.engine.failed():
            raise EngineFailure(f"GPU actor engine failed: {self.engine.error()}")

    def inject_fault(self):
        self.engine.inject_fault()

    def get_batch(self, n_slots: int | None = None, timeout: float = 600.0):
        n = n_slots or self.batch_slots
        self.check()
        slots = self.engine.get_full(n, timeout)
        self.check()
        if len(slots) < n:
            raise TimeoutError(f"no full rollout slot within {timeout}s (engine stats "
                               f"{self.engine.stats()})")
        sp = N.stream_ptr()
        for s in slots:
            self.engine.stream_wait_full(sp, s)
        keys = [k for k in self.rb if k != "last_action0"]
        if n == 1:
            s = slots[0]
            batch = {k: self.rb[k][s] for k in keys}
        else:
            batch = {k: torch.cat([self.rb[k][s] for s in slots], dim=1) for k in keys}
        if self.reference_keys:
            la = [torch.cat([self.rb["last_action0"][s][None], self.rb["action"][s][:-1]])
                  for s in slots]
            batch["last_action"] = la[0] if n == 1 else torch.cat(la, dim=1)
        return batch, slots

    def release(self, slots):
        self.engine.release(list(slots), N.stream_ptr())

    def publish(self, learner_flat: FlatParams, version: int = -1) -> bool:
        return self.engine.publish(learner_flat.data.data_ptr(),
                                   [ln["flat"].data.data_ptr() for ln in self.lanes],
                                   learner_flat.numel * 4, N.stream_ptr(), int(version))

    def policy_lag(self, slots, learner_version: int) -> int:
        return int(learner_version) - min(self.engine.slot_version(int(s)) for s in slots)

    def set_opponent(self, flat: torch.Tensor, version: int) -> bool:
        if self.selfplay_groups <= 0:
            raise RuntimeError("set_opponent: runtime has no self-play groups")
        assert flat.numel() == self.opp_flat.numel and flat.dtype == torch.float32
        return self.engine.publish_opponent(flat.data_ptr(),
                                            [ln["opp_flat"].data.data_ptr() for ln in self.lanes],
                                            self.opp_flat.numel * 4, N.stream_ptr(), int(version))

    def drain_episodes(self):
        return self.engine.drain_episodes()

    def stats(self):
        return self.engine.stats()
```

Before: 21.19 million.

## Publish policy weights via double-buffered packed sets with one fused pack kernel

Adds a single fused kernel that packs conv weights, the fc gather, the head weights and the f32 bias copies straight from the learner's flat parameters into a compact policy set. The engine double-buffers these sets per channel. Publishing then packs into the inactive set instead of copying the full flat to every lane and replaying per-lane pack graphs. This removes per-lane full-parameter copies and several pack launches from the publish path, at the cost of new set-swap synchronisation logic in the engine and extra buffers. The head pack also gains an 8-wide vectorised store path.

```diff
diff --git a/microbeast_amd/_native.py b/microbeast_amd/_native.py
--- a/microbeast_amd/_native.py
+++ b/microbeast_amd/_native.py
@@ -186,6 +186,7 @@
     "mbk_act_trunk": [c_void_p, c_void_p, c_void_p],
     "mbk_act_head": [c_void_p, c_void_p, c_void_p],
     "mbk_act_set_stamps": [c_void_p],
+    "mbk_pack_policy": [c_void_p, c_void_p],
     "mbk_rows_to_codes": [c_void_p, c_int, c_int, c_int, c_void_p, c_void_p, c_void_p],
     "mbk_codes_to_rows": [c_void_p, c_int, c_int, c_void_p, c_int, c_void_p],
     "mbk_gemm_nt_mask": [c_void_p, c_void_p, c_void_p, c_void_p, c_int, c_int, c_int, c_int, c_int,
diff --git a/microbeast_amd/csrc/include/mbk_api.h b/microbeast_amd/csrc/include/mbk_api.h
--- a/microbeast_amd/csrc/include/mbk_api.h
+++ b/microbeast_amd/csrc/include/mbk_api.h
@@ -32,6 +32,26 @@
 } MbkPackJob8;
 
 int mbk_conv_pack_fp8(const MbkPackJob8* jobs, int n, hipStream_t stream);
+
+#define MBK_POLICY_CONVS 15
+#define MBK_POLICY_F32 18
+typedef struct {
+  MbkPackJob conv[MBK_POLICY_CONVS];
+  int n_conv;
+  const float* w5;
+  const int32_t* w5_map;
+  void* w5_dst;
+  int w5_n;
+  const float* head_w;
+  const float* head_b;
+  int S;
+  void* Wp;
+  float* bp;
+  MbkCopySeg f32[MBK_POLICY_F32];
+  int n_f32;
+} MbkPolicyPack;
+
+int mbk_pack_policy(const MbkPolicyPack* p, hipStream_t stream);
 
 typedef struct {
   const void* w0;
diff --git a/microbeast_amd/csrc/kernels/conv.hip b/microbeast_amd/csrc/kernels/conv.hip
--- a/microbeast_amd/csrc/kernels/conv.hip
+++ b/microbeast_amd/csrc/kernels/conv.hip
@@ -1,6 +1,7 @@
 #include "../include/mbk_api.h"
 #include "common.h"
 #include "launch.h"
+#include "pack.h"
 #include "tile.h"
 
 #include <algorithm>
@@ -1352,46 +1353,15 @@
   }
 }
 
-struct PackJob {
-  const float* w;
-  bf16* fwd;
-  bf16* bwd;
-  int cin, cin_real, cout;
-};
 struct PackJobs {
   PackJob j[16];
   int n;
 };
 
-__device__ __forceinline__ int nch_of(int c) { return c == 16 ? 5 : 9; }
-
 __global__ __launch_bounds__(256) void conv_pack_kernel(PackJobs jobs) {
   const PackJob& J = jobs.j[blockIdx.y];
   if (blockIdx.y >= jobs.n) return;
-  const int nf = J.cout * nch_of(J.cin) * 32;
-  const int nb = J.bwd ? J.cin * nch_of(J.cout) * 32 : 0;
-  for (int e = blockIdx.x * blockDim.x + threadIdx.x; e < nf + nb; e += gridDim.x * blockDim.x) {
-    if (e < nf) {
-      const int co = e / (nch_of(J.cin) * 32), r = e % (nch_of(J.cin) * 32);
-      const int c = r / 32, k = r % 32;
-      int tap, ci;
-      if (J.cin == 16) { tap = 2 * c + k / 16; ci = k % 16; }
-      else { tap = c; ci = k; }
-      float v = 0.f;
-      if (tap < 9 && ci < J.cin_real) v = J.w[((size_t)co * J.cin_real + ci) * 9 + tap];
-      J.fwd[e] = f2bf(v);
-    } else {
-      const int f = e - nf;
-      const int ci = f / (nch_of(J.cout) * 32), r = f % (nch_of(J.cout) * 32);
-      const int c = r / 32, k = r % 32;
-      int tap, co;
-      if (J.cout == 16) { tap = 2 * c + k / 16; co = k % 16; }
-      else { tap = c; co = k; }
-      float v = 0.f;
-      if (tap < 9 && ci < J.cin_real) v = J.w[((size_t)co * J.cin_real + ci) * 9 + (8 - tap)];
-      J.bwd[f] = f2bf(v);
-    }
-  }
+  conv_pack_elems(J, blockIdx.x * blockDim.x + threadIdx.x, gridDim.x * blockDim.x);
 }
 
 struct PackJob8 {
diff --git a/microbeast_amd/csrc/kernels/gridnet.hip b/microbeast_amd/csrc/kernels/gridnet.hip
--- a/microbeast_amd/csrc/kernels/gridnet.hip
+++ b/microbeast_amd/csrc/kernels/gridnet.hip
@@ -1,4 +1,5 @@
 #include "common.h"
+#include "pack.h"
 
 #include <algorithm>
 #include <climits>
@@ -105,24 +106,14 @@
 }
 
 constexpr int kMaxSeg = 24;
-struct MapSeg {
-  const float* src;
-  void* dst;
-  const int* map;
-  int n, dst_bf16;
-};
+using mbk::MapSeg;
 struct MapSegs {
   MapSeg s[kMaxSeg];
 };
 
 __global__ __launch_bounds__(kThreads) void map_gather_kernel(MapSegs a) {
   const MapSeg sg = a.s[blockIdx.y];
-  for (int i = blockIdx.x * kThreads + threadIdx.x; i < sg.n; i += gridDim.x * kThreads) {
-    const int m = sg.map[i];
-    const float v = m >= 0 ? sg.src[m] : 0.f;
-    if (sg.dst_bf16) ((bf16*)sg.dst)[i] = __float2bfloat16(v);
-    else ((float*)sg.dst)[i] = v;
-  }
+  mbk::map_gather_elems(sg, blockIdx.x * kThreads + threadIdx.x, gridDim.x * kThreads);
 }
 
 __global__ __launch_bounds__(kThreads) void value_bwd_kernel(const float* __restrict__ dv,
diff --git a/microbeast_amd/csrc/kernels/head.hip b/microbeast_amd/csrc/kernels/head.hip
--- a/microbeast_amd/csrc/kernels/head.hip
+++ b/microbeast_amd/csrc/kernels/head.hip
@@ -5,6 +5,7 @@
 #include "../include/microrts_rules.h"
 #include "common.h"
 #include "launch.h"
+#include "pack.h"
 #include "tile.h"
 
 #ifndef MBK_HA_MB
@@ -1324,22 +1325,9 @@
                                                         bf16* __restrict__ Wp,
                                                         float* __restrict__ bp,
                                                         bf16* __restrict__ WpT) {
-  const size_t nWp = (size_t)S * NP * KD;
-  const size_t nWt = WpT ? (size_t)S * KD * NPT : 0;
-  const size_t nb = (size_t)S * NP;
-  for (size_t e = (size_t)blockIdx.x * blockDim.x + threadIdx.x; e < nWp + nWt + nb;
-       e += (size_t)gridDim.x * blockDim.x) {
-    if (e < nWp) {
-      const size_t c = e / (NP * KD), r = e % (NP * KD), n = r / KD, k = r % KD;
-      Wp[e] = f2bf(n < (size_t)kCell ? W[(c * kCell + n) * KD + k] : 0.f);
-    } else if (e < nWp + nWt) {
-      const size_t q = e - nWp, c = q / (KD * NPT), r = q % (KD * NPT), d = r / NPT, n = r % NPT;
-      WpT[q] = f2bf(n < (size_t)kCell ? W[(c * kCell + n) * KD + d] : 0.f);
-    } else {
-      const size_t q = e - nWp - nWt, c = q / NP, n = q % NP;
-      bp[q] = n < (size_t)kCell ? b[c * kCell + n] : 0.f;
-    }
-  }
+  static_assert(KD == kHeadKD && NP == kHeadNP && NPT == kHeadNPT, "pack.h head geometry");
+  head_pack_elems(W, b, S, Wp, bp, WpT, (size_t)blockIdx.x * blockDim.x + threadIdx.x,
+                  (size_t)gridDim.x * blockDim.x);
 }
 
 }
@@ -1526,7 +1514,7 @@
 
 extern "C" int mbk_head_pack(const float* W, const float* b, int S, void* Wp, float* bp, void* WpT,
                              hipStream_t stream) {
-  size_t tot = (size_t)S * (NP * KD + (WpT ? KD * NPT : 0) + NP);
+  size_t tot = head_pack_total(S, WpT != nullptr);
   size_t blocks = (tot + 255) / 256;
   if (blocks > 4096) blocks = 4096;
   hipLaunchKernelGGL(head_pack_kernel, dim3((unsigned)blocks), dim3(256), 0, stream, W, b, S,
diff --git a/microbeast_amd/csrc/kernels/pack.h b/microbeast_amd/csrc/kernels/pack.h
--- /dev/null
+++ b/microbeast_amd/csrc/kernels/pack.h
@@ -0,0 +1,113 @@
+#pragma once
+#include "common.h"
+
+namespace mbk {
+
+struct PackJob {
+  const float* w;
+  bf16* fwd;
+  bf16* bwd;
+  int cin, cin_real, cout;
+};
+
+__host__ __device__ __forceinline__ int nch_of(int c) { return c == 16 ? 5 : 9; }
+
+__device__ __forceinline__ void conv_pack_elems(const PackJob& J, int first, int stride) {
+  const int nf = J.cout * nch_of(J.cin) * 32;
+  const int nb = J.bwd ? J.cin * nch_of(J.cout) * 32 : 0;
+  for (int e = first; e < nf + nb; e += stride) {
+    if (e < nf) {
+      const int co = e / (nch_of(J.cin) * 32), r = e % (nch_of(J.cin) * 32);
+      const int c = r / 32, k = r % 32;
+      int tap, ci;
+      if (J.cin == 16) { tap = 2 * c + k / 16; ci = k % 16; }
+      else { tap = c; ci = k; }
+      float v = 0.f;
+      if (tap < 9 && ci < J.cin_real) v = J.w[((size_t)co * J.cin_real + ci) * 9 + tap];
+      J.fwd[e] = f2bf(v);
+    } else {
+      const int f = e - nf;
+      const int ci = f / (nch_of(J.cout) * 32), r = f % (nch_of(J.cout) * 32);
+      const int c = r / 32, k = r % 32;
+      int tap, co;
+      if (J.cout == 16) { tap = 2 * c + k / 16; co = k % 16; }
+      else { tap = c; co = k; }
+      float v = 0.f;
+      if (tap < 9 && ci < J.cin_real) v = J.w[((size_t)co * J.cin_real + ci) * 9 + (8 - tap)];
+      J.bwd[f] = f2bf(v);
+    }
+  }
+}
+
+struct MapSeg {
+  const float* src;
+  void* dst;
+  const int* map;
+  int n, dst_bf16;
+};
+
+__device__ __forceinline__ void map_gather_elems(const MapSeg& sg, int first, int stride) {
+  for (int i = first; i < sg.n; i += stride) {
+    const int m = sg.map[i];
+    const float v = m >= 0 ? sg.src[m] : 0.f;
+    if (sg.dst_bf16) ((bf16*)sg.dst)[i] = __float2bfloat16(v);
+    else ((float*)sg.dst)[i] = v;
+  }
+}
+
+constexpr int kHeadKD = 256;
+constexpr int kHeadNP = 80;
+constexpr int kHeadNPT = 96;
+
+constexpr int kHeadVec = 8;
+__host__ __device__ __forceinline__ size_t head_pack_total(int S, bool with_t) {
+  return (size_t)S * (kHeadNP * kHeadKD / kHeadVec + (with_t ? kHeadKD * kHeadNPT : 0) + kHeadNP);
+}
+
+__device__ __forceinline__ void head_pack_elems(const float* __restrict__ W,
+                                                const float* __restrict__ b, int S,
+                                                bf16* __restrict__ Wp, float* __restrict__ bp,
+                                                bf16* __restrict__ WpT, size_t first,
+                                                size_t stride) {
+  constexpr int KD = kHeadKD, NP = kHeadNP, NPT = kHeadNPT, V = kHeadVec, KV = KD / V;
+  static_assert(KD % V == 0 && V == 8, "a Wp item is 8 features");
+  const size_t nWp = (size_t)S * NP * KV;
+  const size_t nWt = WpT ? (size_t)S * KD * NPT : 0;
+  const size_t nb = (size_t)S * NP;
+  const bool vec = ((((uintptr_t)W) | ((uintptr_t)Wp)) & 15) == 0;
+  for (size_t e = first; e < nWp + nWt + nb; e += stride) {
+    if (e < nWp) {
+      const size_t c = e / (NP * KV), r = e % (NP * KV), n = r / KV, k = (r % KV) * V;
+      float v[V];
+#pragma unroll
+      for (int j = 0; j < V; ++j) v[j] = 0.f;
+      if (n < (size_t)kCell) {
+        const float* src = W + (c * kCell + n) * KD + k;
+        if (vec) {
+          const float4 lo = *(const float4*)src, hi = *(const float4*)(src + 4);
+          v[0] = lo.x; v[1] = lo.y; v[2] = lo.z; v[3] = lo.w;
+          v[4] = hi.x; v[5] = hi.y; v[6] = hi.z; v[7] = hi.w;
+        } else {
+#pragma unroll
+          for (int j = 0; j < V; ++j) v[j] = src[j];
+        }
+      }
+      bf16* dst = Wp + e * V;
+      if (vec) {
+        *(uint4*)dst = make_uint4(pack2(v[0], v[1]), pack2(v[2], v[3]), pack2(v[4], v[5]),
+                                  pack2(v[6], v[7]));
+      } else {
+#pragma unroll
+        for (int j = 0; j < V; ++j) dst[j] = f2bf(v[j]);
+      }
+    } else if (e < nWp + nWt) {
+      const size_t q = e - nWp, c = q / (KD * NPT), r = q % (KD * NPT), d = r / NPT, n = r % NPT;
+      WpT[q] = f2bf(n < (size_t)kCell ? W[(c * kCell + n) * KD + d] : 0.f);
+    } else {
+      const size_t q = e - nWp - nWt, c = q / NP, n = q % NP;
+      bp[q] = n < (size_t)kCell ? b[c * kCell + n] : 0.f;
+    }
+  }
+}
+
+}
diff --git a/microbeast_amd/csrc/kernels/publish.hip b/microbeast_amd/csrc/kernels/publish.hip
--- /dev/null
+++ b/microbeast_amd/csrc/kernels/publish.hip
@@ -0,0 +1,104 @@
+#include "../include/mbk_api.h"
+#include "common.h"
+#include "pack.h"
+
+#include <algorithm>
+#include <climits>
+
+using namespace mbk;
+
+namespace {
+
+constexpr int kThreads = 256;
+constexpr int kConvBlocks = 16;
+constexpr int kHeadBlocks = 4096;
+constexpr int kGatherBlocks = 1024;
+
+struct F32Seg {
+  const float* src;
+  float* dst;
+  int n;
+};
+
+struct PolicyArgs {
+  PackJob conv[MBK_POLICY_CONVS];
+  MapSeg w5;
+  const float* head_w;
+  const float* head_b;
+  bf16* Wp;
+  float* bp;
+  F32Seg f32[MBK_POLICY_F32];
+  int S, n_conv, n_f32;
+  int nb_head, nb_w5;
+};
+
+__global__ __launch_bounds__(kThreads) void pack_policy_kernel(PolicyArgs a) {
+  int b = blockIdx.x;
+  const int tid = threadIdx.x;
+  if (b < a.nb_head) {
+    head_pack_elems(a.head_w, a.head_b, a.S, a.Wp, a.bp, nullptr,
+                    (size_t)b * kThreads + tid, (size_t)a.nb_head * kThreads);
+    return;
+  }
+  b -= a.nb_head;
+  if (b < kConvBlocks * a.n_conv) {
+    const PackJob& J = a.conv[b / kConvBlocks];
+    conv_pack_elems(J, (b % kConvBlocks) * kThreads + tid, kConvBlocks * kThreads);
+    return;
+  }
+  b -= kConvBlocks * a.n_conv;
+  if (b < a.nb_w5) {
+    map_gather_elems(a.w5, b * kThreads + tid, a.nb_w5 * kThreads);
+    return;
+  }
+  b -= a.nb_w5;
+  if (b < a.n_f32) {
+    const F32Seg sg = a.f32[b];
+    for (int i = tid; i < sg.n; i += kThreads) sg.dst[i] = sg.src[i];
+  }
+}
+
+int blocks_for(size_t work, int cap) {
+  const size_t g = (work + kThreads - 1) / kThreads;
+  return (int)std::min<size_t>(g, (size_t)cap);
+}
+
+}
+
+extern "C" int mbk_pack_policy(const MbkPolicyPack* p, hipStream_t stream) {
+  if (!p || p->n_conv < 0 || p->n_conv > MBK_POLICY_CONVS || p->n_f32 < 0 ||
+      p->n_f32 > MBK_POLICY_F32 || p->w5_n < 0 || p->S < 0)
+    return (int)hipErrorInvalidValue;
+  PolicyArgs a{};
+  for (int i = 0; i < p->n_conv; ++i) {
+    const MbkPackJob& j = p->conv[i];
+    const bool c_ok = (j.cin == 16 || j.cin == 32) && (j.cout == 16 || j.cout == 32) &&
+                      j.cin_real >= 1 && j.cin_real <= j.cin;
+    if (!j.w || !j.fwd || j.bwd || !c_ok) return (int)hipErrorInvalidValue;
+    a.conv[i] = PackJob{j.w, (bf16*)j.fwd, nullptr, j.cin, j.cin_real, j.cout};
+  }
+  a.n_conv = p->n_conv;
+  if (p->w5_n > 0 && (!p->w5 || !p->w5_map || !p->w5_dst)) return (int)hipErrorInvalidValue;
+  a.w5 = MapSeg{p->w5, p->w5_dst, (const int*)p->w5_map, p->w5_n, 1};
+  if (p->S > 0 && (!p->head_w || !p->head_b || !p->Wp || !p->bp))
+    return (int)hipErrorInvalidValue;
+  a.head_w = p->head_w;
+  a.head_b = p->head_b;
+  a.Wp = (bf16*)p->Wp;
+  a.bp = p->bp;
+  a.S = p->S;
+  for (int i = 0; i < p->n_f32; ++i) {
+    const MbkCopySeg& s = p->f32[i];
+    if (!s.src || !s.dst || (s.bytes & 3) || s.bytes / 4 > (uint64_t)INT_MAX ||
+        (((uintptr_t)s.src | (uintptr_t)s.dst) & 3))
+      return (int)hipErrorInvalidValue;
+    a.f32[i] = F32Seg{(const float*)s.src, (float*)s.dst, (int)(s.bytes / 4)};
+  }
+  a.n_f32 = p->n_f32;
+  a.nb_head = p->S > 0 ? blocks_for(head_pack_total(p->S, false), kHeadBlocks) : 0;
+  a.nb_w5 = p->w5_n > 0 ? blocks_for((size_t)p->w5_n, kGatherBlocks) : 0;
+  const int grid = a.nb_head + kConvBlocks * a.n_conv + a.nb_w5 + a.n_f32;
+  if (grid == 0) return 0;
+  hipLaunchKernelGGL(pack_policy_kernel, dim3(grid), dim3(kThreads), 0, stream, a);
+  return (int)hipGetLastError();
+}
diff --git a/microbeast_amd/csrc/runtime/bindings.cpp b/microbeast_amd/csrc/runtime/bindings.cpp
--- a/microbeast_amd/csrc/runtime/bindings.cpp
+++ b/microbeast_amd/csrc/runtime/bindings.cpp
@@ -221,6 +221,19 @@
     return (int)hipMemcpy2DAsync(P<void>(dst), dpitch, P<const void>(src), spitch, width, height,
                                  hipMemcpyDefault, (hipStream_t)stream);
   });
+
+  py::class_<PubSets>(m, "PubSets")
+      .def(py::init<int>(), py::arg("n_lanes"))
+      .def("reset", &PubSets::reset)
+      .def("n_lanes", &PubSets::n_lanes)
+      .def("busy", &PubSets::busy)
+      .def("current", &PubSets::current)
+      .def("writable", &PubSets::writable)
+      .def("lane_set", &PubSets::lane_set)
+      .def("pending", &PubSets::pending)
+      .def("version", &PubSets::version)
+      .def("begin", &PubSets::begin)
+      .def("apply", &PubSets::apply);
 
   py::class_<GpuEngine>(m, "GpuEngine")
       .def(py::init([](py::dict c, py::dict b) {
@@ -330,6 +343,38 @@
            },
            py::arg("blocks"),
            py::arg("opp_blocks") = std::vector<py::bytes>{})
+      .def("set_policy_sets",
+           [](GpuEngine& e, int chan, std::vector<py::bytes> jobs,
+              std::vector<py::bytes> weights) {
+             std::vector<MbkPolicyPack> js;
+             std::vector<MbkActModel> ws;
+             for (const py::bytes& b : jobs) {
+               const std::string raw = b;
+               if (raw.size() != sizeof(MbkPolicyPack))
+                 throw std::runtime_error("set_policy_sets: job block size " +
+                                          std::to_string(raw.size()) +
+                                          " != sizeof(MbkPolicyPack) " +
+                                          std::to_string(sizeof(MbkPolicyPack)));
+               MbkPolicyPack j;
+               std::memcpy(&j, raw.data(), sizeof(j));
+               js.push_back(j);
+             }
+             for (const py::bytes& b : weights) {
+               const std::string raw = b;
+               if (raw.size() != sizeof(MbkActModel))
+                 throw std::runtime_error("set_policy_sets: weight block size " +
+                                          std::to_string(raw.size()) +
+                                          " != sizeof(MbkActModel) " +
+                                          std::to_string(sizeof(MbkActModel)));
+               MbkActModel m;
+               std::memcpy(&m, raw.data(), sizeof(m));
+               ws.push_back(m);
+             }
+             e.set_policy_sets(chan, js, ws);
+           },
+           py::arg("chan"), py::arg("jobs"), py::arg("weights"))
+      .def("current_set", &GpuEngine::current_set)
+      .def_static("policy_pack_size", [] { return (int)sizeof(MbkPolicyPack); })
       .def("act_mode", &GpuEngine::act_mode)
       .def("set_sparse_io", &GpuEngine::set_sparse_io)
       .def("set_greedy", &GpuEngine::set_greedy)
diff --git a/microbeast_amd/csrc/runtime/engine.cpp b/microbeast_amd/csrc/runtime/engine.cpp
--- a/microbeast_amd/csrc/runtime/engine.cpp
+++ b/microbeast_amd/csrc/runtime/engine.cpp
@@ -119,7 +119,7 @@
   }
   for (PubChan& c : pub_) {
     CTOR_CHECK(hipEventCreateWithFlags(&c.ready, hipEventDisableTiming));
-    c.pending.assign(cfg_.n_lanes, false);
+    c.sets.reset(cfg_.n_lanes);
     c.dst.assign(cfg_.n_lanes, 0);
     c.consumed.assign(cfg_.n_lanes, nullptr);
     for (auto& ev : c.consumed) CTOR_CHECK(hipEventCreateWithFlags(&ev, hipEventDisableTiming));
@@ -262,6 +262,66 @@
       if (!L.opp_scratch && hipMalloc((void**)&L.opp_scratch, sc) != hipSuccess)
         throw std::runtime_error("set_act_models: hipMalloc of the opponent scratch failed");
   }
+}
+
+namespace {
+void take_weights(MbkActModel& m, const MbkActModel& set) {
+  m.w0 = set.w0;
+  m.b0 = set.b0;
+  for (int i = 0; i < 14; ++i) {
+    m.w[i] = set.w[i];
+    m.b[i] = set.b[i];
+  }
+  m.w5 = set.w5;
+  m.b5 = set.b5;
+  m.wc = set.wc;
+  m.bc = set.bc;
+  m.Wp = set.Wp;
+  m.bp = set.bp;
+}
+
+MbkPolicyPack rebased(const MbkPolicyPack& job, uintptr_t base) {
+  MbkPolicyPack p = job;
+  auto at = [base](const void* off) { return (const float*)(base + (uintptr_t)off); };
+  for (int i = 0; i < p.n_conv; ++i) p.conv[i].w = at(p.conv[i].w);
+  p.w5 = at(p.w5);
+  p.head_w = at(p.head_w);
+  p.head_b = at(p.head_b);
+  for (int i = 0; i < p.n_f32; ++i) p.f32[i].src = at(p.f32[i].src);
+  return p;
+}
+}
+
+void GpuEngine::set_policy_sets(int chan, const std::vector<MbkPolicyPack>& jobs,
+                                const std::vector<MbkActModel>& weights) {
+  if (started_) throw std::runtime_error("set_policy_sets: before start() only");
+  if (chan < 0 || chan > 1) throw std::runtime_error("set_policy_sets: channel 0 or 1");
+  std::vector<MbkActModel>& models = chan == 0 ? act_models_ : opp_act_models_;
+  if (models.empty())
+    throw std::runtime_error("set_policy_sets: the channel has no fused acting step blocks");
+  if (jobs.size() != 2 || weights.size() != 2)
+    throw std::runtime_error("set_policy_sets: need two sets (a double buffer)");
+  for (const MbkPolicyPack& j : jobs)
+    if (j.n_conv != MBK_POLICY_CONVS || j.n_f32 < 0 || j.n_f32 > MBK_POLICY_F32 ||
+        j.S != cfg_.size * cfg_.size)
+      throw std::runtime_error("set_policy_sets: pack job shape mismatch");
+  for (const MbkActModel& w : weights)
+    if (!w.w0 || !w.b0 || !w.w5 || !w.b5 || !w.wc || !w.bc || !w.Wp || !w.bp)
+      throw std::runtime_error("set_policy_sets: a set is missing a weight pointer");
+  std::lock_guard<std::mutex> l(pub_m_);
+  PubChan& P = pub_[chan];
+  for (int s = 0; s < 2; ++s) {
+    P.job[s] = jobs[s];
+    P.weights[s] = weights[s];
+  }
+  P.packed = true;
+  P.sets.reset(cfg_.n_lanes);
+  for (MbkActModel& m : models) take_weights(m, P.weights[P.sets.current()]);
+}
+
+int GpuEngine::current_set(int chan) {
+  std::lock_guard<std::mutex> l(pub_m_);
+  return pub_[chan < 0 || chan > 1 ? 0 : chan].sets.current();
 }
 
 void GpuEngine::stop() {
@@ -387,22 +447,26 @@
     const int ln = G.lane;
     for (int c = 0; c < 2; ++c) {
       PubChan& P = pub_[c];
-      if (!P.pending[ln]) continue;
+      if (!P.sets.pending(ln)) continue;
       if (hipEventQuery(P.ready) == hipErrorNotReady) continue;
       ENG_CHECK(hipStreamWaitEvent(st, P.ready, 0));
-      ENG_CHECK(hipMemcpyAsync((void*)P.dst[ln], P.staging, P.n, hipMemcpyDeviceToDevice,
-                               st));
-      ENG_CHECK(hipEventRecord(P.consumed[ln], st));
-      if (L.pack_graph[c]) ENG_CHECK(hipGraphLaunch(L.pack_graph[c], st));
-      P.pending[ln] = false;
-      if (c == 1) L.opp_version = P.version;
-      else if (P.version >= 0) L.policy_version = P.version;
-      bool all = true;
-      for (bool pl : P.pending) all = all && !pl;
-      if (all) {
+      if (P.packed) {
+        ENG_CHECK(hipEventRecord(P.consumed[ln], st));
+        take_weights((c == 0 ? act_models_ : opp_act_models_)[ln],
+                     P.weights[P.sets.writable()]);
+      } else {
+        ENG_CHECK(hipMemcpyAsync((void*)P.dst[ln], P.staging, P.n, hipMemcpyDeviceToDevice,
+                                 st));
+        ENG_CHECK(hipEventRecord(P.consumed[ln], st));
+        if (L.pack_graph[c]) ENG_CHECK(hipGraphLaunch(L.pack_graph[c], st));
+      }
+      const int version = P.sets.version();
+      if (c == 1) L.opp_version = version;
+      else if (version >= 0) L.policy_version = version;
+      if (P.sets.apply(ln)) {
         if (c == 0) publishes_.fetch_add(1);
         else {
-          opp_version_pub_.store(P.version);
+          opp_version_pub_.store(version);
           opp_publishes_.fetch_add(1);
         }
       }
@@ -732,11 +796,23 @@
                              size_t nbytes, uintptr_t stream, int version) {
   std::lock_guard<std::mutex> l(pub_m_);
   PubChan& P = pub_[chan];
+  hipStream_t s = (hipStream_t)stream;
+  if (P.packed) {
+    if (P.sets.busy()) return false;
+    for (hipEvent_t ev : P.consumed)
+      if (hipStreamWaitEvent(s, ev, 0) != hipSuccess)
+        throw std::runtime_error("publish: hipStreamWaitEvent failed");
+    const MbkPolicyPack job = rebased(P.job[P.sets.writable()], src);
+    const hipError_t e = (hipError_t)mbk_pack_policy(&job, s);
+    if (e != hipSuccess || hipEventRecord(P.ready, s) != hipSuccess)
+      throw std::runtime_error(std::string("publish: policy pack failed: ") +
+                               hipGetErrorString(e));
+    P.sets.begin(version);
+    return true;
+  }
   if ((int)dsts.size() != cfg_.n_lanes)
     throw std::runtime_error("publish: need one destination per lane");
-  for (bool pl : P.pending)
-    if (pl) return false;
-  hipStream_t s = (hipStream_t)stream;
+  if (P.sets.busy()) return false;
   if (nbytes > P.staging_n) {
     if (P.staging) {
       for (Lane& L : lanes_) hipStreamSynchronize(L.stream);
@@ -751,8 +827,7 @@
   hipEventRecord(P.ready, s);
   P.dst = dsts;
   P.n = nbytes;
-  P.version = version;
-  P.pending.assign(cfg_.n_lanes, true);
+  P.sets.begin(version);
   return true;
 }
 
diff --git a/microbeast_amd/csrc/runtime/engine.h b/microbeast_amd/csrc/runtime/engine.h
--- a/microbeast_amd/csrc/runtime/engine.h
+++ b/microbeast_amd/csrc/runtime/engine.h
@@ -12,6 +12,7 @@
 #include <thread>
 #include <vector>
 
+#include "pub_sets.h"
 #include "vec_env.h"
 #include "../include/mbk_api.h"
 
@@ -120,6 +121,9 @@
   void set_act_models(const std::vector<MbkActModel>& models,
                       const std::vector<MbkActModel>& opp_models = {});
   bool act_mode() const { return !act_models_.empty(); }
+  void set_policy_sets(int chan, const std::vector<MbkPolicyPack>& jobs,
+                       const std::vector<MbkActModel>& weights);
+  int current_set(int chan);
   void set_sparse_io(bool on);
   bool sparse_io() const { return sparse_; }
   void set_greedy(bool on);
@@ -149,14 +153,16 @@
     std::atomic<int64_t> t_ready_ns{0};
   };
   struct PubChan {
-    std::vector<bool> pending;
+    PubSets sets;
     std::vector<uintptr_t> dst;
     size_t n = 0;
-    int version = -1;
     hipEvent_t ready = nullptr;
     std::vector<hipEvent_t> consumed;
     uint8_t* staging = nullptr;
     size_t staging_n = 0;
+    bool packed = false;
+    MbkPolicyPack job[2];
+    MbkActModel weights[2];
   };
   struct Lane {
     hipStream_t stream = nullptr;
diff --git a/microbeast_amd/csrc/runtime/pub_sets.h b/microbeast_amd/csrc/runtime/pub_sets.h
--- /dev/null
+++ b/microbeast_amd/csrc/runtime/pub_sets.h
@@ -0,0 +1,47 @@
+#pragma once
+#include <cstdint>
+#include <vector>
+
+namespace mb {
+
+class PubSets {
+ public:
+  explicit PubSets(int n_lanes = 0) { reset(n_lanes); }
+  void reset(int n_lanes) {
+    pending_.assign(n_lanes < 0 ? 0 : n_lanes, 0);
+    n_pending_ = 0;
+    cur_ = 0;
+    version_ = -1;
+  }
+  int n_lanes() const { return (int)pending_.size(); }
+  bool busy() const { return n_pending_ > 0; }
+  int current() const { return cur_; }
+  int writable() const { return cur_ ^ 1; }
+  int lane_set(int lane) const {
+    return (busy() && !pending_.at(lane)) ? writable() : cur_;
+  }
+  bool pending(int lane) const { return pending_.at(lane) != 0; }
+  int version() const { return version_; }
+  int begin(int version) {
+    if (busy() || pending_.empty()) return -1;
+    for (auto& p : pending_) p = 1;
+    n_pending_ = (int)pending_.size();
+    version_ = version;
+    return writable();
+  }
+  bool apply(int lane) {
+    if (!pending_.at(lane)) return false;
+    pending_[lane] = 0;
+    if (--n_pending_ > 0) return false;
+    cur_ ^= 1;
+    return true;
+  }
+
+ private:
+  std::vector<uint8_t> pending_;
+  int n_pending_ = 0;
+  int cur_ = 0;
+  int version_ = -1;
+};
+
+}
diff --git a/microbeast_amd/ops/policy_set.py b/microbeast_amd/ops/policy_set.py
--- /dev/null
+++ b/microbeast_amd/ops/policy_set.py
@@ -0,0 +1,117 @@
+from __future__ import annotations
+
+import ctypes
+
+import torch
+
+from .. import _native as N
+from .act import MbkActModel
+from .encoder import _Job, encoder_params
+
+c_void_p, c_int = ctypes.c_void_p, ctypes.c_int
+N_CONVS, N_F32 = 15, 18
+
+
+class MbkCopySeg(ctypes.Structure):
+    _fields_ = [("src", c_void_p), ("dst", c_void_p), ("bytes", ctypes.c_uint64)]
+
+
+class MbkPolicyPack(ctypes.Structure):
+    _fields_ = [("conv", _Job * N_CONVS), ("n_conv", c_int),
+                ("w5", c_void_p), ("w5_map", c_void_p), ("w5_dst", c_void_p), ("w5_n", c_int),
+                ("head_w", c_void_p), ("head_b", c_void_p), ("S", c_int),
+                ("Wp", c_void_p), ("bp", c_void_p),
+                ("f32", MbkCopySeg * N_F32), ("n_f32", c_int)]
+
+
+def _align(n: int, a: int = 256) -> int:
+    return (n + a - 1) // a * a
+
+
+class PolicySet:
+
+    def __init__(self, model, flat, device: torch.device):
+        assert model._prepacked and model._hip_enc is not None, "pack_inference first"
+        enc, head = model._hip_enc, model._head(device)
+        nseq = len(model.channels)
+        params = encoder_params(model.network, nseq)
+        assert len(params) == 2 * N_CONVS and len(enc.layers) == N_CONVS
+        fc = model.network[nseq + 2]
+        self._map = model._tail_maps.fwd
+        base = flat.data.data_ptr()
+
+        def off(p):
+            o = p.data_ptr() - base
+            assert 0 <= o and o + 4 * p.numel() <= 4 * flat.numel, "parameter outside its flat"
+            return o
+
+        f32 = [p for p in params[1::2]] + [fc.bias, model.critic.weight, model.critic.bias]
+        assert len(f32) == N_F32
+        sizes = ([("packed_fwd", 2 * enc.packed_fwd.numel()), ("w5", 2 * self._map.numel()),
+                  ("Wp", 2 * head.Wp.numel()), ("bp", 4 * head.bp.numel())]
+                 + [(f"f32_{i}", 4 * p.numel()) for i, p in enumerate(f32)])
+        offs, total = {}, 0
+        for name, nbytes in sizes:
+            offs[name] = total
+            total += _align(nbytes)
+        self.regions = {name: (offs[name], nbytes) for name, nbytes in sizes}
+        self.buf = torch.zeros(total, dtype=torch.uint8, device=device)
+
+        def view(name, like):
+            n = like.numel() * like.element_size()
+            return self.buf[offs[name]:offs[name] + n].view(like.dtype).view(like.shape)
+
+        self.packed_fwd = view("packed_fwd", enc.packed_fwd)
+        self.w5 = view("w5", model._fc_cache["w5"])
+        self.Wp, self.bp = view("Wp", head.Wp), view("bp", head.bp)
+        self.f32 = [view(f"f32_{i}", p) for i, p in enumerate(f32)]
+        self.biases, (self.b5, self.wc, self.bc) = self.f32[:N_CONVS], self.f32[N_CONVS:]
+        self.layers = enc.layers
+        self.flat_numel = flat.numel
+
+        j = MbkPolicyPack()
+        for i, (L, w) in enumerate(zip(enc.layers, params[0::2])):
+            assert w.dtype == torch.float32 and w.is_contiguous()
+            j.conv[i] = _Job(off(w), self.packed_fwd.data_ptr() + 2 * L.w_off, None,
+                             L.cin, L.cin_real, L.cout)
+        j.n_conv = N_CONVS
+        j.w5, j.w5_map, j.w5_dst = off(fc.weight), self._map.data_ptr(), self.w5.data_ptr()
+        j.w5_n = self._map.numel()
+        j.head_w, j.head_b, j.S = off(model.actor.weight), off(model.actor.bias), head.S
+        j.Wp, j.bp = self.Wp.data_ptr(), self.bp.data_ptr()
+        for i, (p, d) in enumerate(zip(f32, self.f32)):
+            j.f32[i] = MbkCopySeg(off(p), d.data_ptr(), 4 * p.numel())
+        j.n_f32 = N_F32
+        self._job = j
+
+        m = MbkActModel()
+        ws = [self.packed_fwd.data_ptr() + 2 * L.w_off for L in enc.layers]
+        m.w0, m.b0 = ws[0], self.biases[0].data_ptr()
+        for i in range(14):
+            m.w[i] = ws[i + 1]
+            m.b[i] = self.biases[i + 1].data_ptr()
+        m.w5, m.b5 = self.w5.data_ptr(), self.b5.data_ptr()
+        m.wc, m.bc = self.wc.data_ptr(), self.bc.data_ptr()
+        m.Wp, m.bp = self.Wp.data_ptr(), self.bp.data_ptr()
+        self._weights = m
+
+    def job_block(self) -> bytes:
+        return bytes(self._job)
+
+    def weights_block(self) -> bytes:
+        return bytes(self._weights)
+
+    def job(self, flat_ptr: int) -> MbkPolicyPack:
+        j = MbkPolicyPack.from_buffer_copy(self._job)
+        for i in range(j.n_conv):
+            j.conv[i].w = flat_ptr + (j.conv[i].w or 0)
+        j.w5 = flat_ptr + (j.w5 or 0)
+        j.head_w, j.head_b = flat_ptr + (j.head_w or 0), flat_ptr + (j.head_b or 0)
+        for i in range(j.n_f32):
+            j.f32[i].src = flat_ptr + (j.f32[i].src or 0)
+        return j
+
+    def pack(self, flat_data: torch.Tensor) -> None:
+        assert flat_data.dtype == torch.float32 and flat_data.numel() >= self.flat_numel
+        j = self.job(flat_data.data_ptr())
+        N.check(N.kernels().mbk_pack_policy(ctypes.addressof(j), N.stream_ptr()), "pack_policy")
diff --git a/microbeast_amd/runtime/gpu_actors.py b/microbeast_amd/runtime/gpu_actors.py
--- a/microbeast_amd/runtime/gpu_actors.py
+++ b/microbeast_amd/runtime/gpu_actors.py
@@ -10,6 +10,7 @@
 from ..ops import cell_head
 from ..ops.copy import zeros
 from ..ops.optim import FlatParams
+from ..ops.policy_set import PolicySet
 
 BOT_IDS = {"coac": 0, "random_biased": 1, "light_rush": 2, "worker_rush": 3, "passive": 4,
            "random": 5}
@@ -209,6 +210,15 @@
             self.engine.set_act_models([ln["act"].block() for ln in self.lanes],
                                        [ln["opp_act"].block() for ln in self.lanes
                                         if "opp_act" in ln])
+            l0 = self.lanes[0]
+            self.policy_sets = [PolicySet(l0["model"], l0["flat"], dev) for _ in range(2)]
+            self.engine.set_policy_sets(0, [s.job_block() for s in self.policy_sets],
+                                        [s.weights_block() for s in self.policy_sets])
+            if self.selfplay_groups > 0:
+                self.opp_sets = [PolicySet(l0["opp_model"], l0["opp_flat"], dev)
+                                 for _ in range(2)]
+                self.engine.set_policy_sets(1, [s.job_block() for s in self.opp_sets],
+                                            [s.weights_block() for s in self.opp_sets])
         self.sparse_io = not self.fused_act and not self.reference_keys
         if self.sparse_io:
             self.engine.set_sparse_io(True)
@@ -266,6 +276,11 @@
             for pg in (lane["pack_graph"], lane.get("opp_pack_graph")):
                 if pg is not None:
                     pg.replay()
+        if self.fused_act:
+            l0 = self.lanes[0]
+            self.policy_sets[self.engine.current_set(0)].pack(l0["flat"].data)
+            if self.selfplay_groups > 0:
+                self.opp_sets[self.engine.current_set(1)].pack(l0["opp_flat"].data)
         torch.cuda.synchronize()
         ex = lambda g: int(g.raw_cuda_graph_exec()) if g is not None else 0
         self.engine.start([[ex(ln["graph"]), ex(ln.get("opp_graph")), ex(ln["pack_graph"]),
@@ -284,7 +299,7 @@
         self.lanes = []
         self.rb = {}
         for k in ("io", "rng", "infer_model", "infer_flat", "pack_graph", "graph", "opp_graph",
-                  "opp_flat", "opp_model"):
+                  "opp_flat", "opp_model", "policy_sets", "opp_sets"):
             if hasattr(self, k):
                 setattr(self, k, None)
 
@@ -322,6 +337,9 @@
         self.engine.release(list(slots), N.stream_ptr())
 
     def publish(self, learner_flat: FlatParams, version: int = -1) -> bool:
+        if self.fused_act:
+            return self.engine.publish(learner_flat.data.data_ptr(), [], 0, N.stream_ptr(),
+                                       int(version))
         return self.engine.publish(learner_flat.data.data_ptr(),
                                    [ln["flat"].data.data_ptr() for ln in self.lanes],
                                    learner_flat.numel * 4, N.stream_ptr(), int(version))
@@ -333,6 +351,13 @@
         if self.selfplay_groups <= 0:
             raise RuntimeError("set_opponent: runtime has no self-play groups")
         assert flat.numel() == self.opp_flat.numel and flat.dtype == torch.float32
+        if self.fused_act:
+            ok = self.engine.publish_opponent(flat.data_ptr(), [], 0, N.stream_ptr(),
+                                              int(version))
+            if ok:
+                for ln in self.lanes:
+                    ln["opp_flat"].data.copy_(flat)
+            return ok
         return self.engine.publish_opponent(flat.data_ptr(),
                                             [ln["opp_flat"].data.data_ptr() for ln in self.lanes],
                                             self.opp_flat.numel * 4, N.stream_ptr(), int(version))
```

New measurement: 20.09 million. -5.2%, worse.
